# Sinica-SLAM/speechbrain

Measured on AMD Instinct MI355X. Metric: audio-sec/sec Fbank→Conformer fwd (16kHz, B=32×15s) at 1/2/4/8 GPU, higher is better.
Workload: dtype bf16; 1 GPU; Fbank(80)→ConvFrontEnd(64,32)→Conformer 12L d=256 H=4 ffn=1024 k=31 encode, B=32×15s per GPU; global_batch=32, seq_len=376, parallelism=replicas1, hip_graph=True

## Files before the change

include/sbk.h:

```cpp
#ifndef SBK_H
#define SBK_H

#include <stdint.h>

#ifdef __cplusplus
extern "C" {
#endif

#define SBK_ERR_ARG 1001


int sbk_fft_supported(int n_fft);

int sbk_spectrum(int mode, const float* wav, int Bo, int S, int C, int n_fft, int hop, int center, int pad_mode,
                 int T, const float* window, const float* twiddle_nc, const float* twiddle_nfft, int onesided,
                 float norm_scale, float power, float eps, int log_mag, const long long* out_strides,
                 const int* mel_start, const int* mel_len, const int* mel_off, const float* mel_w, int n_melw,
                 int M, int log_mel, float multiplier, float db_offset, float amin, float* out, float* slot_max,
                 void* stream);

int sbk_spectrum_slots(int n_fft, int hop, int T, int M, int n_melw);

int sbk_filterbank(const float* spec, int N, int T, int F, const int* mel_start, const int* mel_len,
                   const int* mel_off, const float* mel_w, const float* dense, int M, int log_mel, float multiplier,
                   float db_offset, float amin, float* out, float* slot_max, void* stream);

int sbk_filterbank_slots(int T, int F);

int sbk_topdb_clamp(float* x, const float* slot_max, int nslot, long long per_seq, int nseq, float top_db,
                    void* stream);

int sbk_filterbank_db_bwd(const float* x, const float* g, int N, long long per_seq, int log_mel, float multiplier,
                          float db_offset, float amin, float top_db, float* stats, float* dx, void* stream);

int sbk_filterbank_wgrad(const float* spec, const float* dx, long long rows, int F, int M, long long rows_per_chunk,
                         float* part, void* stream);

int sbk_magnitude(const float* x, float* y, long long n, int L, float power, float eps, int log_mag, void* stream);

int sbk_dct(const float* x, const float* D, float* y, long long rows, int n_in, int n_out, void* stream);

int sbk_deltas(const float* x, float* y, int N, int T, int F, int window_length, int concat, void* stream);
int sbk_deltas_floor(const float* x, float* y, int N, int T, int F, int window_length, const float* slot_max,
                     int nslot, float top_db, void* stream);

int sbk_context_window(const float* x, float* y, int N, int T, int F, int left, int right, void* stream);

int sbk_specaugment(float* x, int N, int T, int F, int c, int w, int warp_mode, float* tmp, const int* fmask,
                    int n_fmask, const int* tmask, int n_tmask, int use_mean, float* partial, long long n_fcells,
                    void* stream);
int sbk_specaugment_needs_scratch(int N, int T, int F, int c, int w, int n_fmask, int n_tmask, int x_aligned);


int sbk_rnnt_forward(const float* x, const int* labels, const int* Tl, const int* Ul, int B, int T, int U1, int V,
                     int blank, int is_logits, int loss_mode, int reduction, float* ws, float* out, void* stream);
long long sbk_rnnt_workspace_floats(int B, int T, int U1);

int sbk_rnnt_backward(const float* x, const int* labels, int B, int T, int U1, int V, int blank, int mode,
                      const float* ws, const float* scale, int scale_per_b, float* grad, void* stream);

int sbk_rnnt_lattice(const int* Tl, const int* Ul, int B, int T, int U1, int loss_mode, int reduction, float* ws,
                     float* out, void* stream);


int sbk_ctc_forward(const float* x, const int* targets, const int* in_len, const int* tg_len, int B, int T, int V,
                    int Lmax, int blank, int is_logits, float* ws, float* loss, void* stream);
long long sbk_ctc_workspace_floats(int B, int T, int Lmax);

int sbk_ctc_backward(const float* x, const int* targets, const int* in_len, const int* tg_len, int B, int T, int V,
                     int Lmax, int blank, int is_logits, const float* ws, const float* grad_out, float* grad,
                     void* stream);

int sbk_nll_rows_forward(const float* x, const int* targets, int B, int U, long long sb, int V, float* sel,
                         float* rsum, void* stream);
int sbk_nll_rows_backward(const int* targets, const float* a, const float* c, int B, int U, long long sb, int V,
                          float* grad, void* stream);


int sbk_thead_fwd(const float* tn, const float* pn, const void* w, const int* labels, int B, int T, int U1, int J,
                  int V, int blank, int act, float slope, float* lse, float* lpb, float* lpl, void* stream);
int sbk_thead_vpad(int V);
int sbk_thead_dlogits(const float* tn, const float* pn, const void* w, const int* labels, int B, int T, int U1,
                      int J, int V, int blank, int act, float slope, const float* lse, const float* gb,
                      const float* gl, const float* scale, int scale_per_b, void* ds, void* stream);
int sbk_thead_wgrad(const void* ds, const float* tn, const float* pn, const int* Tl, int B, int T, int U1, int J,
                    int V, int act, float slope, float* dw, void* stream);


int sbk_length_mask(const float* rel_len, int B, int T, uint8_t* out, void* stream);

int sbk_gemm_glu_group(int dtype_bf16);

int sbk_gemm(int dtype_bf16, const void* A, int lda, const void* W, int ldw, int M, int N, int K,
             const float* bias, int act, float slope, const float* res, int ldr, float alpha,
             const uint8_t* rowmask, void* out, int ldc, int out_bf16, int tile, void* stream);

int sbk_gemm_ln(int dtype_bf16, const void* A, int lda, const void* W, int ldw, int M, int N, int K,
                const float* bias, const float* res, int ldr, float alpha, const uint8_t* rowmask, float* out,
                int ldc, const float* ln_g, const float* ln_b, float ln_eps, void* u, int ldu, int u_bf16, int tile,
                void* stream);

int sbk_ffn_supported(int D, int H);

int sbk_gemm_batched(int dtype_bf16, const void* A, int lda, long long sA, const void* W, int ldw, long long sW, int M,
                     int N, int K, int batch, void* out, int ldc, long long sC, int zdiv, long long sCo, int out_bf16,
                     void* stream);

int sbk_gemm_tn(const void* A, long long lda, long long sA, const void* B, long long ldb, long long sB, int M, int N,
                int K, int batch, float* C, long long ldc, long long sC, void* stream);
int sbk_gemm_tn_cfg(const void* A, long long lda, long long sA, const void* B, long long ldb, long long sB, int M,
                    int N, int K, int batch, float* C, long long ldc, long long sC, int tile, int nsplit, void* stream);
int sbk_gemm_tn_f32(const float* A, long long lda, long long sA, const float* B, long long ldb, long long sB, int M,
                    int N, int K, int batch, float* C, long long ldc, long long sC, int nsplit, void* stream);

long long sbk_ffn_image_elems(int D, int H, int np, int chain);
int sbk_ffn_image(const void* w1, const void* w2, const void* w1b, const void* w2b, const void* wp, int D, int H,
                  int np, void* img, void* stream);

int sbk_ffn(const float* x, int M, int D, int d_eff, int H, const float* g0, const float* b0, float eps0, const void* img,
            long long img_elems, const float* b1, int act, float slope, const float* b2, float alpha, const float* gp, const float* bp,
            float epsp, float* out, const float* gn, const float* bn, float epsn, void* u, int u_bf16, void* stream);

int sbk_ffn_proj(const float* x, int M, int D, int d_eff, int H, const float* g0, const float* b0, float eps0, const void* img,
                 long long img_elems, const float* b1, int act, float slope, const float* b2, float alpha, const float* gp,
                 const float* bp, float epsp, float* out, const float* gn, const float* bn, float epsn, void* u,
                 int u_bf16, int np, void* yp, void* stream);

int sbk_ffn_chain(const float* x, int M, int D, int d_eff, int H, int act, float slope, const float* g0,
                  const float* b0,
                  float eps0, const float* b1, const float* b2, float alpha, const float* gp, const float* bp,
                  float epsp, const float* g0b, const float* b0b, float eps0b, const float* b1b, const float* b2b,
                  float alphab, float* out, const float* gn, const float* bn, float epsn, void* u, int u_bf16,
                  const void* img, long long img_elems, int np, void* yp, void* stream);

int sbk_layernorm(const float* x, int M, int D, const float* g1, const float* b1, float eps1, void* out1,
                  int out1_bf16, const float* g2, const float* b2, float eps2, void* out2, int out2_bf16,
                  void* stream);

int sbk_dwconv_ln_swish(int in_bf16, const void* x, int B, int T, int C, const float* w, const float* bias, int K,
                        int causal, const float* g, const float* beta, float eps, void* out, int out_bf16,
                        void* stream);

int sbk_conv_block_c1(const float* x, int B, int Tin, int Fin, int Cout, const float* w, const float* bias,
                      const float* g, const float* beta, float eps, float slope, void* out, int out_bf16, int* Tout,
                      int* Fout, void* stream);

int sbk_conv_block_mfma(int in_bf16, const void* x, int B, int Tin, int Fin, int Cin, int Cout, const void* wperm,
                        const float* bias, const float* g, const float* beta, float eps, float slope, void* out,
                        int out_bf16, int* Tout, int* Fout, void* stream);

int sbk_conv_frontend2(int dtype_bf16, const float* x, int B, int Tin, int Fin, const float* w1, const float* b1,
                       const float* g1, const float* be1, float eps1, float slope1, int C1, const void* wp2,
                       const float* b2, const float* g2, const float* be2, float eps2, float slope2, int C2, void* out,
                       int out_bf16, const float* slot_max, int nslot, float top_db, int* Tout, int* Fout,
                       void* stream);

int sbk_cast_bf16(const float* x, void* y, long long n, void* stream);

int sbk_swish(const float* x, float* y, long long n, float beta, void* stream);

int sbk_relpos_attention(int dtype_bf16, const void* qkv, const void* pk, const float* pbu, const float* pbv,
                         const uint8_t* kpm, int B, int T, int H, int dh, float scale, void* out, float* probs,
                         void* stream);

int sbk_relpos_attention_ld(int dtype_bf16, const void* qkv, const void* pk, int ldp, const float* pbu,
                            const float* pbv, const unsigned char* kpm, int B, int T, int H, int dh, float scale,
                            void* out, float* probs, void* stream);
int sbk_relpos_attention_mask(int dtype_bf16, const void* qkv, const void* pk, int ldp, const float* pbu,
                              const float* pbv, const unsigned char* kpm, const float* am, long long am_sb,
                              long long am_sh, int B, int T, int H, int dh, float scale, void* out, float* probs,
                              void* stream);
int sbk_mha_attention(const void* qkv, const unsigned char* kpm, int B, int T, int H, int dh, float scale, void* out,
                      void* stream);
long long sbk_relpos_attention_lds(int dtype_bf16, int T, int dh);

int sbk_relpos_xattn_fwd(int dtype_bf16, const void* q, int ldq, const void* k, int ldk, const void* v, int ldv,
                         const void* pk, int ldp, int P, const float* pbu, const float* pbv, const unsigned char* kpm,
                         const float* am, long long am_sb, long long am_sh, int B, int Lq, int Lk, int H, int dh,
                         float scale, int mask_pos_future, float p_drop, unsigned long long seed, void* out, int ldo,
                         float* probs, float* attn, void* stream);
int sbk_relpos_xattn_bwd(int dtype_bf16, const void* q, int ldq, const void* k, int ldk, const void* v, int ldv,
                         const void* pk, int ldp, int P, const float* pbu, const float* pbv, const float* probs,
                         const void* dO, int lddo, int B, int Lq, int Lk, int H, int dh, float scale,
                         int mask_pos_future, float p_drop, unsigned long long seed, float* G, float* dqu, float* dqv,
                         float* dq, float* dk, float* dv, float* dpk, void* stream);

int sbk_conv_module_supported(int D, int K);
int sbk_conv_module(const float* x, float* out, int B, int T, int D, int d_eff, const float* ln0_w, const float* ln0_b,
                    float eps0, const void* w1p, const float* b1p, const float* wc, const float* bc, int K, int causal,
                    const float* ln1_w, const float* ln1_b, float eps1, const void* w2, const float* b2,
                    const unsigned char* kpm, void* stream);
int sbk_conv_module_pre(const float* x, const void* o, const void* wo, const float* bo, float* out, int B, int T,
                        int D, int d_eff, const float* ln0_w, const float* ln0_b, float eps0, const void* w1p, const float* b1p,
                        const float* wc, const float* bc, int K, int causal, const float* ln1_w, const float* ln1_b,
                        float eps1, const void* w2, const float* b2, const unsigned char* kpm, void* stream);

int sbk_inorm_slices(int T);
int sbk_inorm_partials(const float* x, const float* len, int B, int T, int F, double* part, void* stream);
int sbk_inorm_stats(const double* part, int B, int T, int F, int mean_norm, int std_norm, float eps, float* mean,
                    float* std, float* cur_mean, float* cur_std, int upd, float keep, float wgt, float* glob_mean,
                    float* glob_std, void* stream);
int sbk_inorm_apply(const float* x, int B, int T, int F, const float* mean, const float* std, int per_utt, float* y,
                    void* stream);


int sbk_layernorm_bwd_blocks(int M);
int sbk_layernorm_bwd(const float* x, const void* dy, int dy_bf16, int M, int D, const float* g, float eps,
                      const float* dres, float* dx, float* part, void* stream);

int sbk_layernorm_wide(const float* x, int M, int D, const float* g, const float* b, float eps, void* y, int y_bf16,
                       void* stream);

int sbk_colsum(const float* part, int rows, int cols, float* out, int accumulate, void* stream);

int sbk_rowsum_chunks(long long rows);
int sbk_rowsum_batched(const void* x, int x_bf16, int batch, long long rows, int cols, float* part, float* out,
                       int accumulate, void* stream);
int sbk_rowsum(const void* x, int x_bf16, long long rows, int cols, float* part, float* out, int accumulate,
               void* stream);

int sbk_act_fwd(int mode, const void* x, int x_bf16, long long rows, int cols, void* y, int y_bf16, float slope,
                void* stream);
int sbk_act_bwd(int mode, const void* x, int x_bf16, const void* dy, int dy_bf16, long long rows, int cols, void* dx,
                int dx_bf16, float slope, void* stream);

int sbk_dwconv_fwd(const void* x, int x_bf16, int B, int T, int C, const float* w, const float* bias, int K,
                   int causal, void* y, int y_bf16, void* stream);
int sbk_dwconv_wgrad_chunks(int B, int T);
int sbk_dwconv_bwd(const void* x, int x_bf16, const float* dy, int B, int T, int C, const float* w, int K, int causal,
                   void* dx, int dx_bf16, float* part, void* stream);

int sbk_attn_prep(int dtype_bf16, const void* qkv, const void* dO, const void* pk, int ldp, const float* pbu,
                  const float* pbv, int B, int H, int T, int dh, int Tp, int dhp, int Wp, void* qu, void* qv, void* kT,
                  void* v, void* vT, void* doh, void* pkT, void* stream);
int sbk_attn_probs_pad(const float* P, int BH, int T, int Tp, float p, unsigned long long seed, float* attn, void* Pd,
                       int pd_bf16, void* stream);
int sbk_relpos_softmax_bwd_pad(int dtype_bf16, const float* P, const void* dP, int B, int H, int T, int Tp, int Wp,
                               float scale, float p, unsigned long long seed, void* dS, void* Pd, void* dBD,
                               void* stream);
int sbk_attn_dqkv(const float* dq_ac, const float* dq_bd, const float* dk, const float* dv, int B, int H, int T,
                  int dh, int Tp, int dhp, void* out, int out_bf16, void* stream);

int sbk_im2col(const void* x, int x_bf16, int B, int Ti, int Fi, int Ci, int kt, int kf, int st, int sf, int pt,
               int pf, int ldcol, void* col, int col_bf16, void* stream);
int sbk_col2im(const void* dcol, int dcol_bf16, int B, int Ti, int Fi, int Ci, int kt, int kf, int st, int sf, int pt,
               int pf, int ldcol, void* dx, int dx_bf16, void* stream);

int sbk_im2col_x(const void* x, int x_bf16, int B, int Ti, int Fi, int Ci, int kt, int kf, int st, int sf, int dt,
                 int df, int pt, int pf, int To, int Fo, int mode, int ldcol, void* col, int col_bf16, void* stream);
int sbk_col2im_x(const void* dcol, int dcol_bf16, int B, int Ti, int Fi, int Ci, int kt, int kf, int st, int sf,
                 int dt, int df, int pt, int pf, int To, int Fo, int mode, int ldcol, float* dxpad, void* dx,
                 int dx_bf16, void* stream);

long long sbk_joint_bwd_workspace_floats(int B, int T, int U1, int J);
int sbk_joint_fwd(const float* tn, const float* pn, int B, int T, int U1, int J, int act, float slope, void* z,
                  int z_bf16, void* stream);
int sbk_joint_bwd(const float* tn, const float* pn, const void* dz, int dz_bf16, int B, int T, int U1, int J, int act,
                  float slope, float* dtn, float* dpn, float* ws, void* stream);

int sbk_dropout_add(const void* x, int x_bf16, const float* res, long long rows, int cols,
                    const unsigned char* rowmask, float alpha, float p, unsigned long long seed, void* out,
                    int out_bf16, void* stream);

int sbk_logsoftmax_topk(const float* x, long long ldx, int R, int V, int k, float* vals, long long* idx,
                        void* stream);


int sbk_w2v_wav_stats(const float* wav, int B, long long S, float eps, float* stats, void* stream);

int sbk_w2v_conv0(const float* wav, const float* stats, int B, long long S, int T0, int C, int K, int stride,
                  const float* w, const float* g, const float* b, float eps, void* out, int out_mode,
                  uint8_t* scales, void* stream);

int sbk_ln_act(const void* x, int in_bf16, long long ldx, int M, int D, const float* g, const float* b, float eps,
               int act, void* out, long long ldo, int out_mode, uint8_t* scales, long long lds, void* stream);

int sbk_mx_gemm(const uint8_t* A, const uint8_t* SA, long long lda, long long ldsa, long long rpb, long long a_bs,
                long long s_bs, const uint8_t* W, const uint8_t* SW, long long ldw, long long ldsw, int M, int N,
                int K, const float* bias, int act, float alpha, const float* res, long long ldr, void* out,
                long long ldc, int out_mode, uint8_t* out_scales, long long ldso, void* stream);

long long sbk_mx_gemm_ws_floats(int M, int N, int K, int out_mode);
int sbk_mx_gemm_ws(const uint8_t* A, const uint8_t* SA, long long lda, long long ldsa, long long rpb, long long a_bs,
                   long long s_bs, const uint8_t* W, const uint8_t* SW, long long ldw, long long ldsw, int M, int N,
                   int K, const float* bias, int act, float alpha, const float* res, long long ldr, void* out,
                   long long ldc, int out_mode, uint8_t* out_scales, long long ldso, float* ws, long long ws_floats,
                   void* stream);

int sbk_mx_gemm256(const uint8_t* A, const uint8_t* SA, long long lda, long long ldsa, long long rpb, long long a_bs,
                   long long s_bs, const uint8_t* W, const uint8_t* SW, long long ldw, long long ldsw, int M, int N,
                   int K, const float* bias, int act, float alpha, const float* res, long long ldr, void* out,
                   long long ldc, int out_mode, uint8_t* out_scales, long long ldso, void* stream);

int sbk_add_rows_periodic(float* x, int M, int D, const float* pe, int T, void* stream);

int sbk_mx_quant(const void* x, int in_bf16, long long ldx, int M, int K, uint8_t* q, long long ldq,
                 uint8_t* scales, long long ldsq, void* stream);

int sbk_mx_dequant(const uint8_t* q, long long ldq, const uint8_t* scales, long long ldsq, int M, int K, float* out,
                   void* stream);

#ifdef __cplusplus
}
#endif

#endif
```

speechbrain_amd/_enc.py:

```python
import contextlib
import ctypes
import threading
import weakref
from typing import Optional

import torch

from ._lib import OPS, SbkError, check, custom_op, lib, ptr, require_device, stream_of

ACT = {None: 0, "none": 0, "swish": 1, "glu": 2, "leaky_relu": 3, "relu": 3, "gelu": 4}
_bf16 = torch.bfloat16
_f32 = torch.float32


def _is_bf16(t):
    return t.dtype == _bf16


@custom_op("sbk::gemm", mutates_args=())
def _gemm_op(a: torch.Tensor, w: torch.Tensor, bias: Optional[torch.Tensor], act: int, slope: float,
             res: Optional[torch.Tensor], alpha: float, rowmask: Optional[torch.Tensor], out_bf16: bool,
             tile: int) -> torch.Tensor:
    M, K = a.shape
    N = w.shape[0]
    n_out = N // 2 if act == 2 else N
    out = torch.empty(M, n_out, device=a.device, dtype=_bf16 if out_bf16 else _f32)
    rc = lib().sbk_gemm(int(_is_bf16(a)), ptr(a), a.stride(0), ptr(w), w.stride(0), M, N, K, ptr(bias), act,
                        float(slope), ptr(res), res.stride(0) if res is not None else 0, float(alpha),
                        ptr(rowmask), ptr(out), out.stride(0), int(out_bf16), int(tile), stream_of(a))
    check(rc, "sbk_gemm")
    return out


@_gemm_op.register_fake
def _(a, w, bias, act, slope, res, alpha, rowmask, out_bf16, tile):
    n = w.shape[0] // 2 if act == 2 else w.shape[0]
    return a.new_empty(a.shape[0], n, dtype=_bf16 if out_bf16 else _f32)


def gemm(a, w, bias=None, act=None, slope=0.0, res=None, alpha=1.0, rowmask=None, out=None,
         out_dtype=_f32, tile=0):
    require_device(a, w)
    if out is not None:
        raise ValueError("gemm allocates its output (out= is not supported)")
    if a.dtype != w.dtype:
        raise TypeError(f"gemm operand dtypes differ: {a.dtype} vs {w.dtype}")
    if (a.stride(-1) != 1 and a.shape[-1] > 1) or (w.stride(-1) != 1 and w.shape[-1] > 1):
        raise ValueError("gemm operands must be K-contiguous")
    if res is not None and (res.dtype != _f32 or res.stride(-1) != 1):
        raise ValueError("residual must be fp32, row-contiguous")
    vec = 8 if a.dtype == _bf16 else 4
    if (a.shape[1] % vec or a.stride(0) % vec or w.stride(0) % vec
            or (a.data_ptr() | w.data_ptr()) % 16):
        Kp = -(-a.shape[1] // vec) * vec
        a = torch.nn.functional.pad(a, (0, Kp - a.shape[1]))
        w = torch.nn.functional.pad(w, (0, Kp - w.shape[1]))
    return OPS.gemm(a, w, bias, ACT[act], float(slope), res, float(alpha), rowmask,
                              out_dtype == _bf16, int(tile))


@custom_op("sbk::gemm_tn", mutates_args=())
def _gemm_tn_op(a: torch.Tensor, b: torch.Tensor) -> torch.Tensor:
    K, M = a.shape[-2], a.shape[-1]
    N = b.shape[-1]
    batch = a.shape[0] if a.dim() == 3 else 1
    out = torch.zeros(*([batch] if a.dim() == 3 else []), M, N, device=a.device, dtype=_f32)
    sa = a.stride(0) if a.dim() == 3 else 0
    sb = b.stride(0) if b.dim() == 3 else 0
    _tn_call(a, a.stride(-2), sa, b, b.stride(-2), sb, M, N, K, batch, out, N, M * N if a.dim() == 3 else 0)
    return out


def _tn_call(a, lda, sa, b, ldb, sb, M, N, K, batch, out, ldc, sc):
    det = torch.are_deterministic_algorithms_enabled()
    L = lib()
    if a.dtype == _bf16:
        rc = (L.sbk_gemm_tn_cfg(ptr(a), lda, sa, ptr(b), ldb, sb, M, N, K, batch, ptr(out), ldc, sc, 0, 1, stream_of(a))
              if det else L.sbk_gemm_tn(ptr(a), lda, sa, ptr(b), ldb, sb, M, N, K, batch, ptr(out), ldc, sc, stream_of(a)))
    else:
        rc = L.sbk_gemm_tn_f32(ptr(a), lda, sa, ptr(b), ldb, sb, M, N, K, batch, ptr(out), ldc, sc, int(det),
                               stream_of(a))
    check(rc, "sbk_gemm_tn")


@_gemm_tn_op.register_fake
def _(a, b):
    return a.new_empty(*a.shape[:-2], a.shape[-1], b.shape[-1], dtype=_f32)


def gemm_tn(a, b):
    require_device(a, b)
    if a.dtype != b.dtype or a.dtype not in (_bf16, _f32):
        raise TypeError(f"gemm_tn takes two bf16 or two fp32 operands (got {a.dtype}, {b.dtype})")
    if a.stride(-1) != 1 or b.stride(-1) != 1:
        raise ValueError("gemm_tn operands must be column-contiguous")
    return OPS.gemm_tn(a, b)


def gemm_tn_into(a, b, out, ldc, sC):
    require_device(a, b, out)
    Bt, K, M = a.shape
    N = b.shape[-1]
    if a.dtype != b.dtype or out.dtype != _f32 or a.stride(-1) != 1 or b.stride(-1) != 1:
        raise ValueError("gemm_tn_into: same-dtype column-contiguous operands, fp32 out")
    if out.numel() < (Bt - 1) * sC + (M - 1) * ldc + N:
        raise ValueError("gemm_tn_into: output too small")
    _tn_call(a, a.stride(1), a.stride(0), b, b.stride(1), b.stride(0), M, N, K, Bt, out, ldc, sC)
    return out


@custom_op("sbk::gemm_batched", mutates_args=())
def _gemm_batched_op(a: torch.Tensor, w: torch.Tensor, out_bf16: bool, M: int, zdiv: int, ldc: int, sC: int,
                     sCo: int, rows: int) -> torch.Tensor:
    Bt, _, K = a.shape
    N = w.shape[1]
    if zdiv:
        out = torch.empty(rows, ldc, device=a.device, dtype=_bf16 if out_bf16 else _f32)
    else:
        out = torch.empty(Bt, M, N, device=a.device, dtype=_bf16 if out_bf16 else _f32)
        ldc, sC = N, M * N
    check(lib().sbk_gemm_batched(int(_is_bf16(a)), ptr(a), a.stride(1), a.stride(0), ptr(w), w.stride(1), w.stride(0),
                                 M, N, K, Bt, ptr(out), ldc, sC, zdiv, sCo, int(out_bf16), stream_of(a)),
          "sbk_gemm_batched")
    return out


@_gemm_batched_op.register_fake
def _(a, w, out_bf16, M, zdiv, ldc, sC, sCo, rows):
    dt = _bf16 if out_bf16 else _f32
    if zdiv:
        return a.new_empty(rows, ldc, dtype=dt)
    return a.new_empty(a.shape[0], M, w.shape[1], dtype=dt)


def gemm_batched(a, w, out_dtype=_f32, M=None, heads=None):
    require_device(a, w)
    if a.dtype != w.dtype or a.dtype not in (_bf16, _f32):
        raise TypeError(f"gemm_batched takes two bf16 or two fp32 operands (got {a.dtype}, {w.dtype})")
    if a.stride(-1) != 1 or w.stride(-1) != 1:
        raise ValueError("gemm_batched operands must be K-contiguous")
    Bt, Ma, _ = a.shape
    N = w.shape[1]
    M = Ma if M is None else int(M)
    if not 0 < M <= Ma:
        raise ValueError("gemm_batched: M out of range")
    if heads:
        H = int(heads)
        if Bt % H:
            raise ValueError("gemm_batched: batch not a multiple of heads")
        return OPS.gemm_batched(a, w, out_dtype == _bf16, M, H, H * N, N, M * H * N, Bt // H * M)
    return OPS.gemm_batched(a, w, out_dtype == _bf16, M, 0, 0, 0, 0, 0)


@custom_op("sbk::length_mask", mutates_args=())
def _length_mask_op(rel_len: torch.Tensor, T: int) -> torch.Tensor:
    B = rel_len.shape[0]
    out = torch.empty(B, T, device=rel_len.device, dtype=torch.uint8)
    check(lib().sbk_length_mask(ptr(rel_len), B, int(T), ptr(out), stream_of(rel_len)), "sbk_length_mask")
    return out


@_length_mask_op.register_fake
def _(rel_len, T):
    return rel_len.new_empty(rel_len.shape[0], T, dtype=torch.uint8)


def length_mask(rel_len, T):
    require_device(rel_len)
    rl = rel_len if (rel_len.dtype == _f32 and rel_len.is_contiguous()) else rel_len.float().contiguous()
    return OPS.length_mask(rl, int(T))


@custom_op("sbk::gemm_ln", mutates_args=())
def _gemm_ln_op(a: torch.Tensor, w: torch.Tensor, g: torch.Tensor, b: torch.Tensor, eps: float,
                bias: Optional[torch.Tensor], res: Optional[torch.Tensor], alpha: float,
                rowmask: Optional[torch.Tensor], u_bf16: bool, tile: int) -> tuple[torch.Tensor, torch.Tensor]:
    M, K = a.shape
    N = w.shape[0]
    out = torch.empty(M, N, device=a.device, dtype=_f32)
    u = torch.empty(M, N, device=a.device, dtype=_bf16 if u_bf16 else _f32)
    rc = lib().sbk_gemm_ln(int(_is_bf16(a)), ptr(a), a.stride(0), ptr(w), w.stride(0), M, N, K, ptr(bias), ptr(res),
                           res.stride(0) if res is not None else 0, float(alpha), ptr(rowmask), ptr(out),
                           out.stride(0), ptr(g), ptr(b), float(eps), ptr(u), u.stride(0), int(u_bf16),
                           int(tile), stream_of(a))
    check(rc, "sbk_gemm_ln")
    return out, u


@_gemm_ln_op.register_fake
def _(a, w, g, b, eps, bias, res, alpha, rowmask, u_bf16, tile):
    return (a.new_empty(a.shape[0], w.shape[0], dtype=_f32),
            a.new_empty(a.shape[0], w.shape[0], dtype=_bf16 if u_bf16 else _f32))


def gemm_ln(a, w, ln, bias=None, res=None, alpha=1.0, rowmask=None, out=None, u_dtype=_bf16, tile=0):
    require_device(a, w)
    if out is not None:
        raise ValueError("gemm_ln allocates its output (out= is not supported)")
    if a.dtype != w.dtype:
        raise TypeError(f"gemm operand dtypes differ: {a.dtype} vs {w.dtype}")
    if res is not None and (res.dtype != _f32 or res.stride(-1) != 1):
        raise ValueError("residual must be fp32, row-contiguous")
    g, b, eps = ln
    return OPS.gemm_ln(a, w, g, b, float(eps), bias, res, float(alpha), rowmask, u_dtype == _bf16,
                                 int(tile))


USE_GEMM_LN = False


def gemm_ln_supported(N):
    return int(N) == 256


@custom_op("sbk::layernorm", mutates_args=())
def _layernorm_op(x: torch.Tensor, w1: torch.Tensor, b1: torch.Tensor, eps1: float, out1_mode: int,
                  w2: Optional[torch.Tensor], b2: Optional[torch.Tensor], eps2: float,
                  out2_bf16: bool) -> tuple[torch.Tensor, torch.Tensor]:
    M, D = x.shape
    out1 = torch.empty(M, D, device=x.device, dtype=_bf16 if out1_mode == 2 else _f32) if out1_mode else None
    out2 = torch.empty(M, D, device=x.device, dtype=_bf16 if out2_bf16 else _f32) if w2 is not None else None
    rc = lib().sbk_layernorm(ptr(x), M, D, ptr(w1), ptr(b1), float(eps1), ptr(out1), int(out1_mode == 2),
                             ptr(w2), ptr(b2), float(eps2), ptr(out2), int(out2 is not None and out2_bf16),
                             stream_of(x))
    check(rc, "sbk_layernorm")
    e = x.new_empty(0)
    return (out1 if out1 is not None else e), (out2 if out2 is not None else e)


@_layernorm_op.register_fake
def _(x, w1, b1, eps1, out1_mode, w2, b2, eps2, out2_bf16):
    o1 = x.new_empty(x.shape, dtype=_bf16 if out1_mode == 2 else _f32) if out1_mode else x.new_empty(0)
    o2 = x.new_empty(x.shape, dtype=_bf16 if out2_bf16 else _f32) if w2 is not None else x.new_empty(0)
    return o1, o2


def layernorm(x, w1, b1, eps1, out1_dtype=_f32, w2=None, b2=None, eps2=1e-5, out2_dtype=_bf16, out1=None):
    require_device(x)
    if out1 is not None:
        raise ValueError("layernorm allocates its output (out1= is not supported)")
    mode = 0 if out1_dtype is None else (2 if out1_dtype == _bf16 else 1)
    y1, y2 = OPS.layernorm(x, w1, b1, float(eps1), mode, w2, b2, float(eps2), out2_dtype == _bf16)
    return (y1 if mode else None), (y2 if w2 is not None else None)


def ffn_supported(D, H):
    return bool(lib().sbk_ffn_supported(int(D), int(H)))


class _ImageCache:

    def __init__(self, cap=64):
        self.cap = cap
        self._d = {}

    def _drop(self, key):
        self._d.pop(key, None)

    def get(self, ws, np_, stream):
        key = tuple((w.data_ptr(), w._version) if w is not None else None for w in ws) + (np_,)
        hit = self._d.pop(key, None)
        if hit is None:
            w1, w2, w1b, w2b, wp = ws
            D, H = w1.shape[1], w1.shape[0]
            n = int(lib().sbk_ffn_image_elems(D, H, np_, int(w1b is not None)))
            if n <= 0:
                raise SbkError(f"sbk_ffn_image_elems: unsupported shape D={D} H={H} np={np_}")
            img = torch.empty(n, device=w1.device, dtype=_bf16)
            check(lib().sbk_ffn_image(ptr(w1), ptr(w2), ptr(w1b), ptr(w2b), ptr(wp), D, H, np_, ptr(img),
                                      ctypes.c_void_p(stream.cuda_stream)), "sbk_ffn_image")
            ev = torch.cuda.Event()
            ev.record(stream)
            refs = tuple(weakref.ref(w, lambda _r, k=key: self._drop(k)) for w in ws if w is not None)
            hit = (img, refs, ev, stream.cuda_stream)
            if len(self._d) >= self.cap:
                self._d.pop(next(iter(self._d)))
        elif hit[3] != stream.cuda_stream:
            stream.wait_event(hit[2])
        self._d[key] = hit
        return hit[0]


_FFN_IMAGES = _ImageCache()


def ffn_image(w1, w2, w1b=None, w2b=None, wp=None):
    for t in (w1, w2, w1b, w2b, wp):
        if t is not None and (t.dtype != _bf16 or not t.is_contiguous()):
            raise TypeError("ffn_image: contiguous bf16 weights")
    img = _FFN_IMAGES.get((w1, w2, w1b, w2b, wp), 0 if wp is None else wp.shape[0], torch.cuda.current_stream(w1.device))
    return img


@custom_op("sbk::ffn", mutates_args=())
def _ffn_op(x: torch.Tensor, g0: torch.Tensor, b0: torch.Tensor, e0: float, w1: torch.Tensor, b1: torch.Tensor,
            act: int, slope: float, w2: torch.Tensor, b2: torch.Tensor, alpha: float, gp: Optional[torch.Tensor],
            bp: Optional[torch.Tensor], ep: float, gn: Optional[torch.Tensor], bn: Optional[torch.Tensor], en: float,
            next_bf16: bool, deff: int) -> tuple[torch.Tensor, torch.Tensor]:
    M, D = x.shape
    H = w1.shape[0]
    img = ffn_image(w1, w2)
    out = torch.empty_like(x)
    u = torch.empty(M, D, device=x.device, dtype=_bf16 if next_bf16 else _f32) if gn is not None else None
    rc = lib().sbk_ffn(ptr(x), M, D, deff, H, ptr(g0), ptr(b0), float(e0), ptr(img), img.numel(), ptr(b1), act,
                       float(slope), ptr(b2), float(alpha), ptr(gp), ptr(bp), float(ep), ptr(out), ptr(gn), ptr(bn), float(en),
                       ptr(u), int(next_bf16), stream_of(x))
    check(rc, "sbk_ffn")
    return out, (u if u is not None else x.new_empty(0))


@_ffn_op.register_fake
def _(x, g0, b0, e0, w1, b1, act, slope, w2, b2, alpha, gp, bp, ep, gn, bn, en, next_bf16, deff):
    return (torch.empty_like(x),
            x.new_empty(x.shape, dtype=_bf16 if next_bf16 else _f32) if gn is not None else x.new_empty(0))


@custom_op("sbk::ffn_proj", mutates_args=())
def _ffn_proj_op(x: torch.Tensor, g0: torch.Tensor, b0: torch.Tensor, e0: float, w1: torch.Tensor,
                 b1: torch.Tensor, act: int, slope: float, w2: torch.Tensor, b2: torch.Tensor, alpha: float,
                 gp: Optional[torch.Tensor], bp: Optional[torch.Tensor], ep: float, gn: torch.Tensor,
                 bn: torch.Tensor, en: float, wp: torch.Tensor, deff: int) -> tuple[torch.Tensor, torch.Tensor]:
    M, D = x.shape
    H, NP = w1.shape[0], wp.shape[0]
    img = ffn_image(w1, w2, wp=wp)
    out = torch.empty_like(x)
    y = torch.empty(M, NP, device=x.device, dtype=_bf16)
    rc = lib().sbk_ffn_proj(ptr(x), M, D, deff, H, ptr(g0), ptr(b0), float(e0), ptr(img), img.numel(), ptr(b1), act,
                            float(slope), ptr(b2), float(alpha), ptr(gp), ptr(bp), float(ep), ptr(out), ptr(gn), ptr(bn),
                            float(en), None, 1, NP, ptr(y), stream_of(x))
    check(rc, "sbk_ffn_proj")
    return out, y


@_ffn_proj_op.register_fake
def _(x, g0, b0, e0, w1, b1, act, slope, w2, b2, alpha, gp, bp, ep, gn, bn, en, wp, deff):
    return torch.empty_like(x), x.new_empty((x.shape[0], wp.shape[0]), dtype=_bf16)


def ffn_proj_supported(D, H, NP):
    return ffn_supported(D, H) and NP > 0 and NP % 256 == 0


def ffn_proj(x, ln0, w1, b1, act, slope, w2, b2, alpha, next_ln, wp, post_ln=None, deff=None):
    require_device(x, w1, w2, wp)
    gp, bp, ep = post_ln if post_ln is not None else (None, None, 0.0)
    return OPS.ffn_proj(x, ln0[0], ln0[1], float(ln0[2]), w1, b1, ACT[act], float(slope), w2, b2,
                                  float(alpha), gp, bp, float(ep), next_ln[0], next_ln[1], float(next_ln[2]), wp,
                       int(deff or x.shape[1]))


@custom_op("sbk::ffn_chain", mutates_args=())
def _ffn_chain_op(x: torch.Tensor, act: int, slope: float, g0: torch.Tensor, b0: torch.Tensor, e0: float,
                  w1: torch.Tensor, b1: torch.Tensor, w2: torch.Tensor, b2: torch.Tensor, alpha: float,
                  gp: Optional[torch.Tensor], bp: Optional[torch.Tensor], ep: float, g0b: torch.Tensor,
                  b0b: torch.Tensor, e0b: float, w1b: torch.Tensor, b1b: torch.Tensor, w2b: torch.Tensor,
                  b2b: torch.Tensor, alphab: float, gn: torch.Tensor, bn: torch.Tensor, en: float,
                  wp: torch.Tensor, deff: int) -> tuple[torch.Tensor, torch.Tensor]:
    M, D = x.shape
    H, NP = w1.shape[0], wp.shape[0]
    img = ffn_image(w1, w2, w1b, w2b, wp)
    out = torch.empty_like(x)
    y = torch.empty(M, NP, device=x.device, dtype=_bf16)
    rc = lib().sbk_ffn_chain(ptr(x), M, D, deff, H, act, float(slope), ptr(g0), ptr(b0), float(e0), ptr(b1), ptr(b2),
                             float(alpha), ptr(gp), ptr(bp), float(ep), ptr(g0b), ptr(b0b), float(e0b), ptr(b1b),
                             ptr(b2b), float(alphab), ptr(out), ptr(gn), ptr(bn), float(en), None, 1, ptr(img), img.numel(), NP,
                             ptr(y), stream_of(x))
    check(rc, "sbk_ffn_chain")
    return out, y


@_ffn_chain_op.register_fake
def _(x, act, slope, g0, b0, e0, w1, b1, w2, b2, alpha, gp, bp, ep, g0b, b0b, e0b, w1b, b1b, w2b, b2b, alphab, gn,
      bn, en, wp, deff):
    return torch.empty_like(x), x.new_empty((x.shape[0], wp.shape[0]), dtype=_bf16)


def ffn_chain(x, a, b, act, slope, next_ln, wp, deff=None):
    require_device(x, a[1], b[1], wp)
    if b[1].shape != a[1].shape or b[3].shape != a[3].shape:
        raise ValueError(f"ffn_chain: block shapes differ ({tuple(a[1].shape)}/{tuple(a[3].shape)} vs "
                         f"{tuple(b[1].shape)}/{tuple(b[3].shape)})")
    gp, bp, ep = a[6] if a[6] is not None else (None, None, 0.0)
    return OPS.ffn_chain(x, ACT[act], float(slope), a[0][0], a[0][1], float(a[0][2]), a[1], a[2], a[3],
                                   a[4], float(a[5]), gp, bp, float(ep), b[0][0], b[0][1], float(b[0][2]), b[1], b[2],
                                   b[3], b[4], float(b[5]), next_ln[0], next_ln[1], float(next_ln[2]), wp,
                         int(deff or x.shape[1]))


def ffn(x, ln0, w1, b1, act, slope, w2, b2, alpha, post_ln=None, next_ln=None, next_dtype=_bf16, out=None, deff=None):
    require_device(x, w1, w2)
    gp, bp, ep = post_ln if post_ln is not None else (None, None, 0.0)
    gn, bn, en = next_ln if next_ln is not None else (None, None, 0.0)
    y, u = OPS.ffn(x, ln0[0], ln0[1], float(ln0[2]), w1, b1, ACT[act], float(slope), w2, b2, float(alpha),
                             gp, bp, float(ep), gn, bn, float(en), next_dtype == _bf16, int(deff or x.shape[1]))
    return y, (u if next_ln is not None else None)


@custom_op("sbk::dwconv_ln_swish", mutates_args=())
def _dwconv_op(x: torch.Tensor, B: int, T: int, w: torch.Tensor, bias: Optional[torch.Tensor], causal: bool,
               ln_w: torch.Tensor, ln_b: torch.Tensor, eps: float, out_bf16: bool) -> torch.Tensor:
    C = x.shape[-1]
    K = w.shape[-1]
    out = torch.empty(B * T, C, device=x.device, dtype=_bf16 if out_bf16 else _f32)
    rc = lib().sbk_dwconv_ln_swish(int(_is_bf16(x)), ptr(x), B, T, C, ptr(w), ptr(bias), K, int(causal), ptr(ln_w),
                                   ptr(ln_b), float(eps), ptr(out), int(out_bf16), stream_of(x))
    check(rc, "sbk_dwconv_ln_swish")
    return out


@_dwconv_op.register_fake
def _(x, B, T, w, bias, causal, ln_w, ln_b, eps, out_bf16):
    return x.new_empty(B * T, x.shape[-1], dtype=_bf16 if out_bf16 else _f32)


def dwconv_ln_swish(x, B, T, w, bias, causal, ln_w, ln_b, eps, out_dtype):
    return OPS.dwconv_ln_swish(x, int(B), int(T), w, bias, bool(causal), ln_w, ln_b, float(eps),
                                         out_dtype == _bf16)


def conv_module_supported(D, K):
    return bool(lib().sbk_conv_module_supported(int(D), int(K)))


@custom_op("sbk::conv_module", mutates_args=())
def _conv_module_op(x: torch.Tensor, B: int, T: int, g0: torch.Tensor, b0: torch.Tensor, e0: float,
                    w1p: torch.Tensor, b1p: torch.Tensor, wc: torch.Tensor, bc: Optional[torch.Tensor], causal: bool,
                    g1: torch.Tensor, b1: torch.Tensor, e1: float, w2: torch.Tensor, b2: Optional[torch.Tensor],
                    kpm: Optional[torch.Tensor], o: Optional[torch.Tensor], wo: Optional[torch.Tensor],
                    bo: Optional[torch.Tensor], deff: int) -> torch.Tensor:
    K = wc.shape[0]
    out = torch.empty_like(x)
    rc = lib().sbk_conv_module_pre(ptr(x), ptr(o), ptr(wo), ptr(bo), ptr(out), B, T, x.shape[1], deff, ptr(g0),
                                   ptr(b0),
                                   float(e0), ptr(w1p), ptr(b1p), ptr(wc), ptr(bc), K, int(causal), ptr(g1), ptr(b1),
                                   float(e1), ptr(w2), ptr(b2), ptr(kpm), stream_of(x))
    check(rc, "sbk_conv_module_pre")
    return out


@_conv_module_op.register_fake
def _(x, B, T, g0, b0, e0, w1p, b1p, wc, bc, causal, g1, b1, e1, w2, b2, kpm, o, wo, bo, deff):
    return torch.empty_like(x)


def conv_module(x, B, T, ln0, w1p, b1p, wc, bc, causal, ln1, w2, b2, kpm=None, pre=None, deff=None):
    require_device(x, w1p, w2)
    o, wo, bo = pre if pre is not None else (None, None, None)
    return OPS.conv_module(x, int(B), int(T), ln0[0], ln0[1], float(ln0[2]), w1p, b1p, wc, bc,
                                     bool(causal), ln1[0], ln1[1], float(ln1[2]), w2, b2, kpm, o, wo, bo,
                            int(deff or x.shape[1]))


@custom_op("sbk::conv_block_c1", mutates_args=())
def _conv_block_c1_op(x: torch.Tensor, w: torch.Tensor, bias: torch.Tensor, ln_w: torch.Tensor, ln_b: torch.Tensor,
                      eps: float, slope: float, out_bf16: bool) -> torch.Tensor:
    B, Tin, Fin = x.shape
    Cout = w.shape[0]
    Tout, Fout = (Tin - 1) // 2 + 1, (Fin - 1) // 2 + 1
    out = torch.empty(B, Tout, Fout, Cout, device=x.device, dtype=_bf16 if out_bf16 else _f32)
    rc = lib().sbk_conv_block_c1(ptr(x), B, Tin, Fin, Cout, ptr(w), ptr(bias), ptr(ln_w), ptr(ln_b), float(eps),
                                 float(slope), ptr(out), int(out_bf16), None, None, stream_of(x))
    check(rc, "sbk_conv_block_c1")
    return out


@_conv_block_c1_op.register_fake
def _(x, w, bias, ln_w, ln_b, eps, slope, out_bf16):
    B, Tin, Fin = x.shape
    return x.new_empty(B, (Tin - 1) // 2 + 1, (Fin - 1) // 2 + 1, w.shape[0], dtype=_bf16 if out_bf16 else _f32)


def conv_block_c1(x, w, bias, ln_w, ln_b, eps, slope, out_dtype):
    require_device(x)
    return OPS.conv_block_c1(x, w, bias, ln_w, ln_b, float(eps), float(slope), out_dtype == _bf16)


@custom_op("sbk::conv_block_mfma", mutates_args=())
def _conv_block_mfma_op(x: torch.Tensor, wperm: torch.Tensor, bias: torch.Tensor, ln_w: torch.Tensor,
                        ln_b: torch.Tensor, eps: float, slope: float, out_bf16: bool) -> torch.Tensor:
    B, Tin, Fin, Cin = x.shape
    Cout = wperm.shape[0]
    Tout, Fout = (Tin - 1) // 2 + 1, (Fin - 1) // 2 + 1
    out = torch.empty(B, Tout, Fout, Cout, device=x.device, dtype=_bf16 if out_bf16 else _f32)
    rc = lib().sbk_conv_block_mfma(int(_is_bf16(x)), ptr(x), B, Tin, Fin, Cin, Cout, ptr(wperm), ptr(bias),
                                   ptr(ln_w), ptr(ln_b), float(eps), float(slope), ptr(out), int(out_bf16), None,
                                   None, stream_of(x))
    check(rc, "sbk_conv_block_mfma")
    return out


@_conv_block_mfma_op.register_fake
def _(x, wperm, bias, ln_w, ln_b, eps, slope, out_bf16):
    B, Tin, Fin, _ = x.shape
    return x.new_empty(B, (Tin - 1) // 2 + 1, (Fin - 1) // 2 + 1, wperm.shape[0],
                       dtype=_bf16 if out_bf16 else _f32)


def conv_block_mfma(x, wperm, bias, ln_w, ln_b, eps, slope, out_dtype):
    require_device(x, wperm)
    return OPS.conv_block_mfma(x, wperm, bias, ln_w, ln_b, float(eps), float(slope), out_dtype == _bf16)


@custom_op("sbk::conv_frontend2", mutates_args=())
def _conv_frontend2_op(x: torch.Tensor, w1: torch.Tensor, b1: torch.Tensor, g1: torch.Tensor, be1: torch.Tensor,
                       e1: float, s1: float, wperm2: torch.Tensor, b2: torch.Tensor, g2: torch.Tensor,
                       be2: torch.Tensor, e2: float, s2: float, out_bf16: bool, slot_max: Optional[torch.Tensor],
                       top_db: float) -> torch.Tensor:
    B, Tin, Fin = x.shape
    C1, C2 = w1.shape[0], wperm2.shape[0]
    T1, F1 = (Tin - 1) // 2 + 1, (Fin - 1) // 2 + 1
    T2, F2 = (T1 - 1) // 2 + 1, (F1 - 1) // 2 + 1
    out = torch.empty(B, T2, F2, C2, device=x.device, dtype=_bf16 if out_bf16 else _f32)
    rc = lib().sbk_conv_frontend2(int(_is_bf16(wperm2)), ptr(x), B, Tin, Fin, ptr(w1), ptr(b1), ptr(g1), ptr(be1),
                                  float(e1), float(s1), C1, ptr(wperm2), ptr(b2), ptr(g2), ptr(be2), float(e2),
                                  float(s2), C2, ptr(out), int(out_bf16), ptr(slot_max),
                                  slot_max.shape[1] if slot_max is not None else 0, float(top_db), None, None,
                                  stream_of(x))
    check(rc, "sbk_conv_frontend2")
    return out


@_conv_frontend2_op.register_fake
def _(x, w1, b1, g1, be1, e1, s1, wperm2, b2, g2, be2, e2, s2, out_bf16, slot_max, top_db):
    B, Tin, Fin = x.shape
    T1, F1 = (Tin - 1) // 2 + 1, (Fin - 1) // 2 + 1
    return x.new_empty(B, (T1 - 1) // 2 + 1, (F1 - 1) // 2 + 1, wperm2.shape[0], dtype=_bf16 if out_bf16 else _f32)


def conv_frontend2(x, blk1, blk2, wperm2, out_dtype, topdb=None):
    require_device(x, wperm2)
    w1, b1, g1, be1, e1, s1 = blk1
    _, b2, g2, be2, e2, s2 = blk2
    sm, tdb = topdb if topdb is not None else (None, 0.0)
    return OPS.conv_frontend2(x, w1, b1, g1, be1, float(e1), float(s1), wperm2, b2, g2, be2, float(e2),
                                        float(s2), out_dtype == _bf16, sm, float(tdb))


@custom_op("sbk::relpos_attention", mutates_args=())
def _relpos_attention_op(qkv: torch.Tensor, pk: torch.Tensor, pbu: torch.Tensor, pbv: torch.Tensor,
                         kpm: Optional[torch.Tensor], B: int, T: int, H: int, dh: int, scale: float,
                         need_probs: bool, am: Optional[torch.Tensor], am_sb: int,
                         am_sh: int) -> tuple[torch.Tensor, torch.Tensor]:
    d = H * dh
    out = torch.empty(B * T, d, device=qkv.device, dtype=qkv.dtype)
    probs = torch.empty(B, H, T, T, device=qkv.device, dtype=_f32) if need_probs else qkv.new_empty(0, dtype=_f32)
    if am is None:
        rc = lib().sbk_relpos_attention_ld(int(_is_bf16(qkv)), ptr(qkv), ptr(pk), pk.stride(0), ptr(pbu), ptr(pbv),
                                           ptr(kpm), B, T, H, dh, float(scale), ptr(out),
                                           ptr(probs) if need_probs else None, stream_of(qkv))
    else:
        rc = lib().sbk_relpos_attention_mask(int(_is_bf16(qkv)), ptr(qkv), ptr(pk), pk.stride(0), ptr(pbu), ptr(pbv),
                                             ptr(kpm), ptr(am), am_sb, am_sh, B, T, H, dh, float(scale), ptr(out),
                                             ptr(probs) if need_probs else None, stream_of(qkv))
    check(rc, "sbk_relpos_attention")
    return out, probs


@_relpos_attention_op.register_fake
def _(qkv, pk, pbu, pbv, kpm, B, T, H, dh, scale, need_probs, am, am_sb, am_sh):
    return (qkv.new_empty(B * T, H * dh),
            qkv.new_empty(B, H, T, T, dtype=_f32) if need_probs else qkv.new_empty(0, dtype=_f32))


def attn_mask_arg(attn_mask, B, T, H, device, Lk=None):
    if attn_mask is None:
        return None
    Lk = T if Lk is None else Lk
    m = attn_mask.to(device)
    if m.dtype == torch.bool:
        m = torch.zeros(m.shape, device=device, dtype=_f32).masked_fill_(m, -float("inf"))
    else:
        m = m.to(_f32)
    if m.dim() == 2:
        if tuple(m.shape) != (T, Lk):
            raise ValueError(f"attn_mask {tuple(m.shape)} != ({T}, {Lk})")
        return m.contiguous(), 0, 0
    m = m.reshape(-1, H, T, Lk).contiguous()
    if m.shape[0] not in (1, B):
        raise ValueError(f"attn_mask batch {m.shape[0]} does not broadcast to {B}")
    return m, (H * T * Lk if m.shape[0] == B else 0), T * Lk


def relpos_attention(qkv, pk, pbu, pbv, kpm, B, T, H, dh, scale, need_probs=False, am=None):
    d = H * dh
    if pk.stride(-1) != 1 or pk.shape[-1] != d:
        raise ValueError("pk must be (2T-1, d) with unit column stride")
    m, sb, sh = am if am is not None else (None, 0, 0)
    out, probs = OPS.relpos_attention(qkv, pk, pbu, pbv, kpm, int(B), int(T), int(H), int(dh),
                                                float(scale), bool(need_probs), m, int(sb), int(sh))
    return out, (probs if need_probs else None)


@custom_op("sbk::relpos_xattn", mutates_args=())
def _relpos_xattn_op(q: torch.Tensor, k: torch.Tensor, v: torch.Tensor, pk: Optional[torch.Tensor],
                     pbu: Optional[torch.Tensor], pbv: Optional[torch.Tensor], kpm: Optional[torch.Tensor],
                     am: Optional[torch.Tensor], am_sb: int, am_sh: int, B: int, Lq: int, Lk: int, H: int, dh: int,
                     scale: float, mpf: bool, p: float, seed: int) -> tuple[torch.Tensor, torch.Tensor, torch.Tensor]:
    out = torch.empty(B * Lq, H * dh, device=q.device, dtype=q.dtype)
    probs = torch.empty(B, H, Lq, Lk, device=q.device, dtype=_f32)
    attn = torch.empty_like(probs) if p > 0 else probs.new_empty(0)
    P = pk.shape[0] if pk is not None else 2 * Lk - 1
    rc = lib().sbk_relpos_xattn_fwd(int(_is_bf16(q)), ptr(q), q.stride(0), ptr(k), k.stride(0), ptr(v), v.stride(0),
                                    ptr(pk), pk.stride(0) if pk is not None else 0, P, ptr(pbu), ptr(pbv), ptr(kpm),
                                    ptr(am), int(am_sb), int(am_sh), B, Lq, Lk, H, dh, float(scale), int(mpf),
                                    float(p), int(seed), ptr(out), out.stride(0), ptr(probs),
                                    ptr(attn) if p > 0 else None, stream_of(q))
    check(rc, "sbk_relpos_xattn_fwd")
    return out, probs, attn


@_relpos_xattn_op.register_fake
def _(q, k, v, pk, pbu, pbv, kpm, am, am_sb, am_sh, B, Lq, Lk, H, dh, scale, mpf, p, seed):
    probs = q.new_empty(B, H, Lq, Lk, dtype=_f32)
    return q.new_empty(B * Lq, H * dh), probs, (q.new_empty(B, H, Lq, Lk, dtype=_f32) if p > 0 else
                                                  q.new_empty(0, dtype=_f32))


def relpos_xattn(q, k, v, pk, pbu, pbv, kpm, B, Lq, Lk, H, dh, scale, mask_pos_future=False, am=None, p=0.0,
                 seed=0):
    for t in (q, k, v) + ((pk,) if pk is not None else ()):
        if t.stride(-1) != 1 or t.shape[-1] != H * dh or t.dtype != q.dtype:
            raise ValueError("relpos_xattn: q / k / v / pk must be (rows, H*dh), unit column stride, one dtype")
    if pk is not None and pk.shape[0] // 2 + 1 != Lk:
        raise ValueError(f"pos_embs has {pk.shape[0]} rows: rel_shift keeps {pk.shape[0] // 2 + 1} != k_len {Lk}")
    m, sb, sh = am if am is not None else (None, 0, 0)
    out, probs, attn = OPS.relpos_xattn(q, k, v, pk, pbu, pbv, kpm, m, int(sb), int(sh), int(B), int(Lq), int(Lk),
                                        int(H), int(dh), float(scale), bool(mask_pos_future), float(p), int(seed))
    return out, probs, (attn if p > 0 else probs)


@custom_op("sbk::mha_attention", mutates_args=())
def _mha_attention_op(qkv: torch.Tensor, kpm: Optional[torch.Tensor], B: int, T: int, H: int, dh: int,
                      scale: float) -> torch.Tensor:
    out = torch.empty(B * T, H * dh, device=qkv.device, dtype=qkv.dtype)
    check(lib().sbk_mha_attention(ptr(qkv), ptr(kpm), B, T, H, dh, float(scale), ptr(out), stream_of(qkv)),
          "sbk_mha_attention")
    return out


@_mha_attention_op.register_fake
def _(qkv, kpm, B, T, H, dh, scale):
    return qkv.new_empty(B * T, H * dh)


def mha_fast_ok(qkv, T, dh):
    return qkv.dtype == _bf16 and dh == 64 and T <= 4096 and qkv.is_contiguous() and qkv.data_ptr() % 16 == 0


def mha_attention(qkv, kpm, B, T, H, dh, scale):
    return OPS.mha_attention(qkv, kpm, int(B), int(T), int(H), int(dh), float(scale))


def glu_group():
    return int(lib().sbk_gemm_glu_group(1))


@custom_op("sbk::cast_bf16", mutates_args=())
def _cast_bf16_op(x: torch.Tensor) -> torch.Tensor:
    out = torch.empty(x.shape, device=x.device, dtype=_bf16)
    check(lib().sbk_cast_bf16(ptr(x), ptr(out), x.numel(), stream_of(x)), "sbk_cast_bf16")
    return out


@_cast_bf16_op.register_fake
def _(x):
    return x.new_empty(x.shape, dtype=_bf16)


def cast_bf16(x):
    return OPS.cast_bf16(x)


def to_compute(x, dtype):
    if dtype == _bf16:
        return x.contiguous() if x.dtype == _bf16 else cast_bf16(x.float().contiguous())
    if x.dtype in (torch.float16, _bf16):
        return x.float().contiguous()
    if x.dtype != _f32:
        raise TypeError(f"fp32 compute path got {x.dtype}")
    return x.contiguous()


def compute_dtype():
    if torch.is_autocast_enabled("cuda"):
        dt = torch.get_autocast_dtype("cuda")
        if dt == _bf16:
            return _bf16
        if dt != torch.float16:
            raise NotImplementedError(f"speechbrain_amd kernels compute in bf16 or fp32; torch.autocast(dtype={dt})")
    return _f32


_MX = threading.local()


@contextlib.contextmanager
def mxfp8(enabled=True):
    prev = getattr(_MX, "on", False)
    _MX.on = bool(enabled)
    try:
        yield
    finally:
        _MX.on = prev


def mx_enabled():
    return getattr(_MX, "on", False)


class WeightCache:

    def __init__(self):
        self._d = {}

    def get(self, key, params, make):
        sig = tuple((p.data_ptr(), p._version, p.device) for p in params)
        hit = self._d.get(key)
        if hit is not None and hit[0] == sig:
            return hit[1]
        v = make()
        self._d[key] = (sig, v)
        return v
```

speechbrain_amd/_lib.py:

```python
import ctypes
import os

import torch

_HERE = os.path.dirname(os.path.abspath(__file__))
LIB_PATH = os.path.join(_HERE, "libsbk.so")

_vp = ctypes.c_void_p
_i = ctypes.c_int
_ll = ctypes.c_longlong
_f = ctypes.c_float

SIGNATURES = {
    "sbk_fft_supported": [_i],
    "sbk_spectrum": [_i, _vp, _i, _i, _i, _i, _i, _i, _i, _i, _vp, _vp, _vp, _i, _f, _f, _f, _i, _vp,
                     _vp, _vp, _vp, _vp, _i, _i, _i, _f, _f, _f, _vp, _vp, _vp],
    "sbk_filterbank": [_vp, _i, _i, _i, _vp, _vp, _vp, _vp, _vp, _i, _i, _f, _f, _f, _vp, _vp, _vp],
    "sbk_spectrum_slots": [_i, _i, _i, _i, _i],
    "sbk_filterbank_slots": [_i, _i],
    "sbk_topdb_clamp": [_vp, _vp, _i, _ll, _i, _f, _vp],
    "sbk_filterbank_db_bwd": [_vp, _vp, _i, _ll, _i, _f, _f, _f, _f, _vp, _vp, _vp],
    "sbk_filterbank_wgrad": [_vp, _vp, _ll, _i, _i, _ll, _vp, _vp],
    "sbk_magnitude": [_vp, _vp, _ll, _i, _f, _f, _i, _vp],
    "sbk_dct": [_vp, _vp, _vp, _ll, _i, _i, _vp],
    "sbk_deltas": [_vp, _vp, _i, _i, _i, _i, _i, _vp],
    "sbk_deltas_floor": [_vp, _vp, _i, _i, _i, _i, _vp, _i, _f, _vp],
    "sbk_context_window": [_vp, _vp, _i, _i, _i, _i, _i, _vp],
    "sbk_gemm_glu_group": [_i],
    "sbk_length_mask": [_vp, _i, _i, _vp, _vp],
    "sbk_gemm": [_i, _vp, _i, _vp, _i, _i, _i, _i, _vp, _i, _f, _vp, _i, _f, _vp, _vp, _i, _i, _i, _vp],
    "sbk_gemm_ln": [_i, _vp, _i, _vp, _i, _i, _i, _i, _vp, _vp, _i, _f, _vp, _vp, _i, _vp, _vp, _f, _vp, _i, _i, _i,
                    _vp],
    "sbk_thead_vpad": [_i],
    "sbk_thead_fwd": [_vp, _vp, _vp, _vp, _i, _i, _i, _i, _i, _i, _i, _f, _vp, _vp, _vp, _vp],
    "sbk_thead_dlogits": [_vp, _vp, _vp, _vp, _i, _i, _i, _i, _i, _i, _i, _f, _vp, _vp, _vp, _vp, _i, _vp, _vp],
    "sbk_thead_wgrad": [_vp, _vp, _vp, _vp, _i, _i, _i, _i, _i, _i, _f, _vp, _vp],
    "sbk_rnnt_lattice": [_vp, _vp, _i, _i, _i, _i, _i, _vp, _vp, _vp],
    "sbk_gemm_tn": [_vp, _ll, _ll, _vp, _ll, _ll, _i, _i, _i, _i, _vp, _ll, _ll, _vp],
    "sbk_gemm_tn_cfg": [_vp, _ll, _ll, _vp, _ll, _ll, _i, _i, _i, _i, _vp, _ll, _ll, _i, _i, _vp],
    "sbk_gemm_tn_f32": [_vp, _ll, _ll, _vp, _ll, _ll, _i, _i, _i, _i, _vp, _ll, _ll, _i, _vp],
    "sbk_gemm_batched": [_i, _vp, _i, _ll, _vp, _i, _ll, _i, _i, _i, _i, _vp, _i, _ll, _i, _ll, _i, _vp],
    "sbk_attn_prep": [_i, _vp, _vp, _vp, _i, _vp, _vp, _i, _i, _i, _i, _i, _i, _i, _vp, _vp, _vp, _vp, _vp, _vp,
                      _vp, _vp],
    "sbk_attn_dqkv": [_vp, _vp, _vp, _vp, _i, _i, _i, _i, _i, _i, _vp, _i, _vp],
    "sbk_attn_probs_pad": [_vp, _i, _i, _i, _f, ctypes.c_ulonglong, _vp, _vp, _i, _vp],
    "sbk_relpos_softmax_bwd_pad": [_i, _vp, _vp, _i, _i, _i, _i, _i, _f, _f, ctypes.c_ulonglong, _vp, _vp, _vp,
                                   _vp],
    "sbk_ffn_supported": [_i, _i],
    "sbk_ffn": [_vp, _i, _i, _i, _i, _vp, _vp, _f, _vp, _ll, _vp, _i, _f, _vp, _f, _vp, _vp, _f, _vp, _vp, _vp, _f, _vp,
                _i, _vp],
    "sbk_ffn_chain": [_vp, _i, _i, _i, _i, _i, _f, _vp, _vp, _f, _vp, _vp, _f, _vp, _vp, _f, _vp, _vp, _f, _vp, _vp, _f,
                      _vp, _vp, _vp, _f, _vp, _i, _vp, _ll, _i, _vp, _vp],
    "sbk_ffn_proj": [_vp, _i, _i, _i, _i, _vp, _vp, _f, _vp, _ll, _vp, _i, _f, _vp, _f, _vp, _vp, _f, _vp, _vp, _vp, _f,
                     _vp, _i, _i, _vp, _vp],
    "sbk_ffn_image_elems": [_i, _i, _i, _i],
    "sbk_ffn_image": [_vp, _vp, _vp, _vp, _vp, _i, _i, _i, _vp, _vp],
    "sbk_layernorm": [_vp, _i, _i, _vp, _vp, _f, _vp, _i, _vp, _vp, _f, _vp, _i, _vp],
    "sbk_dwconv_ln_swish": [_i, _vp, _i, _i, _i, _vp, _vp, _i, _i, _vp, _vp, _f, _vp, _i, _vp],
    "sbk_conv_block_c1": [_vp, _i, _i, _i, _i, _vp, _vp, _vp, _vp, _f, _f, _vp, _i, _vp, _vp, _vp],
    "sbk_conv_block_mfma": [_i, _vp, _i, _i, _i, _i, _i, _vp, _vp, _vp, _vp, _f, _f, _vp, _i, _vp, _vp, _vp],
    "sbk_conv_frontend2": [_i, _vp, _i, _i, _i, _vp, _vp, _vp, _vp, _f, _f, _i, _vp, _vp, _vp, _vp, _f, _f, _i,
                           _vp, _i, _vp, _i, _f, _vp, _vp, _vp],
    "sbk_cast_bf16": [_vp, _vp, _ll, _vp],
    "sbk_swish": [_vp, _vp, _ll, _f, _vp],
    "sbk_w2v_wav_stats": [_vp, _i, _ll, _f, _vp, _vp],
    "sbk_w2v_conv0": [_vp, _vp, _i, _ll, _i, _i, _i, _i, _vp, _vp, _vp, _f, _vp, _i, _vp, _vp],
    "sbk_add_rows_periodic": [_vp, _i, _i, _vp, _i, _vp],
    "sbk_ln_act": [_vp, _i, _ll, _i, _i, _vp, _vp, _f, _i, _vp, _ll, _i, _vp, _ll, _vp],
    "sbk_mx_gemm": [_vp, _vp, _ll, _ll, _ll, _ll, _ll, _vp, _vp, _ll, _ll, _i, _i, _i, _vp, _i, _f, _vp, _ll, _vp,
                    _ll, _i, _vp, _ll, _vp],
    "sbk_mx_gemm_ws": [_vp, _vp, _ll, _ll, _ll, _ll, _ll, _vp, _vp, _ll, _ll, _i, _i, _i, _vp, _i, _f, _vp, _ll, _vp,
                       _ll, _i, _vp, _ll, _vp, _ll, _vp],
    "sbk_mx_gemm_ws_floats": [_i, _i, _i, _i],
    "sbk_mx_gemm256": [_vp, _vp, _ll, _ll, _ll, _ll, _ll, _vp, _vp, _ll, _ll, _i, _i, _i, _vp, _i, _f, _vp, _ll,
                       _vp, _ll, _i, _vp, _ll, _vp],
    "sbk_mx_quant": [_vp, _i, _ll, _i, _i, _vp, _ll, _vp, _ll, _vp],
    "sbk_mx_dequant": [_vp, _ll, _vp, _ll, _i, _i, _vp, _vp],
    "sbk_specaugment": [_vp, _i, _i, _i, _i, _i, _i, _vp, _vp, _i, _vp, _i, _i, _vp, _ll, _vp],
    "sbk_specaugment_needs_scratch": [_i, _i, _i, _i, _i, _i, _i, _i],
    "sbk_rnnt_forward": [_vp, _vp, _vp, _vp, _i, _i, _i, _i, _i, _i, _i, _i, _vp, _vp, _vp],
    "sbk_rnnt_workspace_floats": [_i, _i, _i],
    "sbk_logsoftmax_topk": [_vp, _ll, _i, _i, _i, _vp, _vp, _vp],
    "sbk_rnnt_backward": [_vp, _vp, _i, _i, _i, _i, _i, _i, _vp, _vp, _i, _vp, _vp],
    "sbk_ctc_forward": [_vp, _vp, _vp, _vp, _i, _i, _i, _i, _i, _i, _vp, _vp, _vp],
    "sbk_ctc_workspace_floats": [_i, _i, _i],
    "sbk_ctc_backward": [_vp, _vp, _vp, _vp, _i, _i, _i, _i, _i, _i, _vp, _vp, _vp, _vp],
    "sbk_nll_rows_forward": [_vp, _vp, _i, _i, _ll, _i, _vp, _vp, _vp],
    "sbk_nll_rows_backward": [_vp, _vp, _vp, _i, _i, _ll, _i, _vp, _vp],
    "sbk_relpos_attention": [_i, _vp, _vp, _vp, _vp, _vp, _i, _i, _i, _i, _f, _vp, _vp, _vp],
    "sbk_relpos_attention_lds": [_i, _i, _i],
    "sbk_relpos_attention_mask": [_i, _vp, _vp, _i, _vp, _vp, _vp, _vp, _ll, _ll, _i, _i, _i, _i, _f, _vp, _vp, _vp],
    "sbk_relpos_attention_ld": [_i, _vp, _vp, _i, _vp, _vp, _vp, _i, _i, _i, _i, _f, _vp, _vp, _vp],
    "sbk_mha_attention": [_vp, _vp, _i, _i, _i, _i, _f, _vp, _vp],
    "sbk_relpos_xattn_fwd": [_i, _vp, _i, _vp, _i, _vp, _i, _vp, _i, _i, _vp, _vp, _vp, _vp, _ll, _ll, _i, _i, _i, _i,
                             _i, _f, _i, _f, ctypes.c_ulonglong, _vp, _i, _vp, _vp, _vp],
    "sbk_relpos_xattn_bwd": [_i, _vp, _i, _vp, _i, _vp, _i, _vp, _i, _i, _vp, _vp, _vp, _vp, _i, _i, _i, _i, _i, _i,
                             _f, _i, _f, ctypes.c_ulonglong, _vp, _vp, _vp, _vp, _vp, _vp, _vp, _vp],
    "sbk_inorm_slices": [_i],
    "sbk_inorm_partials": [_vp, _vp, _i, _i, _i, _vp, _vp],
    "sbk_inorm_stats": [_vp, _i, _i, _i, _i, _i, _f, _vp, _vp, _vp, _vp, _i, _f, _f, _vp, _vp, _vp],
    "sbk_inorm_apply": [_vp, _i, _i, _i, _vp, _vp, _i, _vp, _vp],
    "sbk_conv_module_supported": [_i, _i],
    "sbk_conv_module_pre": [_vp, _vp, _vp, _vp, _vp, _i, _i, _i, _i, _vp, _vp, _f, _vp, _vp, _vp, _vp, _i, _i, _vp,
                            _vp, _f, _vp, _vp, _vp, _vp],
    "sbk_conv_module": [_vp, _vp, _i, _i, _i, _i, _vp, _vp, _f, _vp, _vp, _vp, _vp, _i, _i, _vp, _vp, _f, _vp, _vp, _vp,
                        _vp],
    "sbk_layernorm_bwd_blocks": [_i],
    "sbk_layernorm_bwd": [_vp, _vp, _i, _i, _i, _vp, _f, _vp, _vp, _vp, _vp],
    "sbk_layernorm_wide": [_vp, _i, _i, _vp, _vp, _f, _vp, _i, _vp],
    "sbk_colsum": [_vp, _i, _i, _vp, _i, _vp],
    "sbk_rowsum_chunks": [_ll],
    "sbk_rowsum": [_vp, _i, _ll, _i, _vp, _vp, _i, _vp],
    "sbk_rowsum_batched": [_vp, _i, _i, _ll, _i, _vp, _vp, _i, _vp],
    "sbk_act_fwd": [_i, _vp, _i, _ll, _i, _vp, _i, _f, _vp],
    "sbk_act_bwd": [_i, _vp, _i, _vp, _i, _ll, _i, _vp, _i, _f, _vp],
    "sbk_dwconv_fwd": [_vp, _i, _i, _i, _i, _vp, _vp, _i, _i, _vp, _i, _vp],
    "sbk_dwconv_wgrad_chunks": [_i, _i],
    "sbk_dwconv_bwd": [_vp, _i, _vp, _i, _i, _i, _vp, _i, _i, _vp, _i, _vp, _vp],
    "sbk_im2col": [_vp, _i, _i, _i, _i, _i, _i, _i, _i, _i, _i, _i, _i, _vp, _i, _vp],
    "sbk_col2im": [_vp, _i, _i, _i, _i, _i, _i, _i, _i, _i, _i, _i, _i, _vp, _i, _vp],
    "sbk_im2col_x": [_vp, _i, _i, _i, _i, _i, _i, _i, _i, _i, _i, _i, _i, _i, _i, _i, _i, _i, _vp, _i, _vp],
    "sbk_col2im_x": [_vp, _i, _i, _i, _i, _i, _i, _i, _i, _i, _i, _i, _i, _i, _i, _i, _i, _i, _vp, _vp, _i, _vp],
    "sbk_joint_fwd": [_vp, _vp, _i, _i, _i, _i, _i, _f, _vp, _i, _vp],
    "sbk_dropout_add": [_vp, _i, _vp, _ll, _i, _vp, _f, _f, ctypes.c_ulonglong, _vp, _i, _vp],
    "sbk_joint_bwd": [_vp, _vp, _vp, _i, _i, _i, _i, _i, _i, _f, _vp, _vp, _vp, _vp],
    "sbk_joint_bwd_workspace_floats": [_i, _i, _i, _i],
}
RESTYPES = {"sbk_relpos_attention_lds": ctypes.c_longlong, "sbk_mx_gemm_ws_floats": ctypes.c_longlong, "sbk_ffn_image_elems": ctypes.c_longlong, "sbk_joint_bwd_workspace_floats": ctypes.c_longlong, "sbk_rnnt_workspace_floats": ctypes.c_longlong, "sbk_ctc_workspace_floats": ctypes.c_longlong}

_lib = None
_load_error = None


class SbkError(RuntimeError):
    pass


def lib():
    global _lib, _load_error
    if _lib is not None:
        return _lib
    if not os.path.exists(LIB_PATH):
        raise SbkError(
            f"speechbrain_amd HIP library not found at {LIB_PATH}; build it with "
            "`python -c 'import __graft_entry__ as g; g.build()'` (hipcc --offload-arch=gfx950). "
            "There is no CPU fallback.")
    try:
        l = ctypes.CDLL(LIB_PATH)
    except OSError as e:
        _load_error = e
        raise SbkError(f"failed to load {LIB_PATH}: {e}") from e
    for name, argt in SIGNATURES.items():
        fn = getattr(l, name)
        fn.argtypes = argt
        fn.restype = RESTYPES.get(name, ctypes.c_int)
    _lib = l
    return l


def exported_symbols():
    return list(SIGNATURES)


def check(rc, what):
    if rc != 0:
        raise SbkError(f"{what} failed with code {rc}" + (" (invalid argument)" if rc == 1001 else ""))


def ptr(t):
    if t is None:
        return None
    return ctypes.c_void_p(t.data_ptr())


def stream_of(t):
    return ctypes.c_void_p(torch.cuda.current_stream(t.device).cuda_stream)


def require_device(*tensors):
    for t in tensors:
        if t is not None and (not isinstance(t, torch.Tensor) or t.device.type != "cuda"):
            raise SbkError("speechbrain_amd kernels need ROCm device tensors (got "
                           f"{getattr(t, 'device', type(t))}); there is no CPU fallback")


class _FastOp:

    def __init__(self, opdef, mutates_args=()):
        import inspect
        self._def = opdef
        self._body = opdef._init_fn
        self._op = None
        names = list(inspect.signature(opdef._init_fn).parameters)
        self._mut = tuple((names.index(m), m) for m in mutates_args)

    def __call__(self, *args, **kw):
        diff = (torch.is_grad_enabled()
                and any(isinstance(t, torch.Tensor) and t.requires_grad for t in (*args, *kw.values())))
        if diff and self._def._backward_fn is None and not torch.jit.is_tracing():
            raise RuntimeError(f"sbk::{self._def._name} has no backward; an input requires grad — call it under "
                               "torch.no_grad() or on detached tensors (the differentiable path is _autograd)")
        if (torch.compiler.is_compiling() or torch.jit.is_tracing()
                or torch._C._get_dispatch_mode(torch._C._TorchDispatchModeKey.FAKE) is not None
                or torch._C._len_torch_dispatch_stack() > 0 or torch._C._are_functorch_transforms_active()
                or diff):
            if self._op is None:
                self._op = getattr(torch.ops.sbk, self._def._name)
            return self._op(*args, **kw)
        out = self._body(*args, **kw)
        for i, m in self._mut:
            t = args[i] if i < len(args) else kw.get(m)
            if isinstance(t, torch.Tensor):
                torch.autograd.graph.increment_version(t)
        return out

    def __getattr__(self, name):
        return getattr(self._def, name)


_OPS = {}


def custom_op(qualname, mutates_args):
    def deco(fn):
        op = _FastOp(torch.library.custom_op(qualname, mutates_args=mutates_args)(fn), mutates_args)
        _OPS[qualname.split("::", 1)[1]] = op
        return op
    return deco


class _Ops:

    def __getattr__(self, name):
        return _OPS[name]


OPS = _Ops()
```

speechbrain_amd/csrc/ffn.hip:

```cpp
#include "mfma.h"

using namespace sbk;

namespace {

enum Act { ACT_NONE = 0, ACT_SWISH = 1, ACT_GLU = 2, ACT_LRELU = 3, ACT_GELU = 4 };

struct FfnArgs {
  const float* x;
  int M, H;
  const float *g0, *b0;
  float eps0;
  const bf16_t* img;
  const float* b1;
  int act;
  float slope;
  const float* b2;
  float alpha;
  const float *gp, *bp;
  float epsp;
  float* out;
  const float *gn, *bn;
  float epsn;
  void* u;
  int u_bf16;
  int np;
  bf16_t* yp;
  const float *g0b, *b0b;
  float eps0b;
  const float *b1b, *b2b;
  float alphab;
  float inv_n, npad;
};

__device__ __forceinline__ bf16x8 ld8(const bf16_t* p) { return *reinterpret_cast<const bf16x8*>(p); }

template <int V>
struct IntC {
  static constexpr int value = V;
};

constexpr int FFN_BM = 48;
constexpr int FFN_PAD = 16;
constexpr int FFN_NW = 8, FFN_NT = FFN_NW * 64;
__device__ __forceinline__ constexpr int ffn_sw(int row) { return ((row >> 2) & 1) << 3; }
static_assert(FFN_NW % 8 == 0, "rows w + FFN_NW * i share bit 2 with w (their swizzle is ffn_sw(w))");
constexpr int FFN_RS = 12;

#define FFN_MFMA(A, B, C) __builtin_amdgcn_mfma_f32_16x16x32_bf16((A), (B), (C), 0, 0, 0)

template <int ACT>
__device__ __forceinline__ float act_fn(float v, float slope) {
  if (ACT == ACT_SWISH) return v * __builtin_amdgcn_rcpf(1.0f + __expf(-v));
  if (ACT == ACT_LRELU) return v >= 0.f ? v : v * slope;
  if (ACT == ACT_GELU) return 0.5f * v * (1.0f + erff(v * 0.70710678118654752f));
  return v;
}

__device__ __forceinline__ f32x4 lds_f4(const float* p) {
  f32x4 v;
  const uint32_t la = (uint32_t)(uintptr_t)((const __attribute__((address_space(3))) float*)p);
  asm volatile("ds_read_b128 %0, %1" : "=v"(v) : "v"(la) : "memory");
  return v;
}

__device__ __forceinline__ uint32_t lds_addr(const void* p) {
  return (uint32_t)(uintptr_t)((const __attribute__((address_space(3))) char*)p);
}
__device__ __forceinline__ float lds_f1(const float* p) {
  float v;
  asm volatile("ds_read_b32 %0, %1" : "=v"(v) : "v"(lds_addr(p)) : "memory");
  return v;
}
__device__ __forceinline__ void lds_st1(float* p, float v) {
  asm volatile("ds_write_b32 %0, %1" ::"v"(lds_addr(p)), "v"(v) : "memory");
}
__device__ __forceinline__ void lds_st4(float* p, f32x4 v) {
  asm volatile("ds_write_b128 %0, %1" ::"v"(lds_addr(p)), "v"(v) : "memory");
}
__device__ __forceinline__ void lds_st2(void* p, uint2 v) {
  const unsigned long long u = (unsigned long long)v.x | ((unsigned long long)v.y << 32);
  asm volatile("ds_write_b64 %0, %1" ::"v"(lds_addr(p)), "v"(u) : "memory");
}
template <typename V>
__device__ __forceinline__ void tie(V& v) {
  asm volatile("s_waitcnt lgkmcnt(0)" : "+v"(v));
}
__device__ __forceinline__ void lds_barrier() {
  asm volatile("s_waitcnt lgkmcnt(0)" ::: "memory");
  __builtin_amdgcn_s_barrier();
}

__device__ __forceinline__ f32x4 gld4(const float* p) {
  f32x4 v;
  asm volatile("global_load_dwordx4 %0, %1, off" : "=v"(v) : "v"(p) : "memory");
  return v;
}
__device__ __forceinline__ void vtie(f32x4& v) { asm volatile("" : "+v"(v)); }

__device__ __forceinline__ void vm_wait(int n) {
  switch (n) {
    case 0: asm volatile("s_waitcnt vmcnt(0)" ::: "memory"); break;
    case 1: asm volatile("s_waitcnt vmcnt(1)" ::: "memory"); break;
    case 2: asm volatile("s_waitcnt vmcnt(2)" ::: "memory"); break;
    case 3: asm volatile("s_waitcnt vmcnt(3)" ::: "memory"); break;
    case 4: asm volatile("s_waitcnt vmcnt(4)" ::: "memory"); break;
    case 5: asm volatile("s_waitcnt vmcnt(5)" ::: "memory"); break;
    case 6: asm volatile("s_waitcnt vmcnt(6)" ::: "memory"); break;
    case 7: asm volatile("s_waitcnt vmcnt(7)" ::: "memory"); break;
    default: asm volatile("s_waitcnt vmcnt(8)" ::: "memory"); break;
  }
}

template <int D, int T2, int MT, int NW>
__device__ __forceinline__ void row_ln(float (&z)[T2][MT][4], float* red, const float* gam, const float* bet, float eps,
                                       int w, int g, int fr, float inv_n, float npad) {
  static_assert(NW == 8, "two b128 reads per row");
  float mean[MT], rstd[MT];
#pragma unroll
  for (int pass = 0; pass < 2; ++pass) {
    float part[MT];
#pragma unroll
    for (int mt = 0; mt < MT; ++mt) {
      float s = 0.f;
#pragma unroll
      for (int j = 0; j < T2; ++j)
#pragma unroll
        for (int e = 0; e < 4; ++e) {
          const float dv = pass ? z[j][mt][e] - mean[mt] : z[j][mt][e];
          s += pass ? dv * dv : dv;
        }
      part[mt] = col4_sum(s);
    }
    lds_barrier();
    if (g == 0) {
#pragma unroll
      for (int mt = 0; mt < MT; ++mt) lds_st1(red + (mt * 16 + fr) * FFN_RS + w, part[mt]);
    }
    lds_barrier();
    f32x4 rv[MT][2];
#pragma unroll
    for (int mt = 0; mt < MT; ++mt) {
      rv[mt][0] = lds_f4(red + (mt * 16 + fr) * FFN_RS);
      rv[mt][1] = lds_f4(red + (mt * 16 + fr) * FFN_RS + 4);
    }
#pragma unroll
    for (int mt = 0; mt < MT; ++mt) {
      tie(rv[mt][0]);
      tie(rv[mt][1]);
      const float t = (rv[mt][0][0] + rv[mt][0][1]) + (rv[mt][0][2] + rv[mt][0][3]) + (rv[mt][1][0] + rv[mt][1][1]) +
                      (rv[mt][1][2] + rv[mt][1][3]);
      if (pass)
        rstd[mt] = 1.0f / sqrtf((t - npad * mean[mt] * mean[mt]) * inv_n + eps);
      else
        mean[mt] = t * inv_n;
    }
  }
  f32x4 gv[T2], bv[T2];
#pragma unroll
  for (int j = 0; j < T2; ++j) {
    const int d = (w * T2 + j) * 16 + 4 * g;
    gv[j] = lds_f4(gam + d);
    bv[j] = lds_f4(bet + d);
  }
#pragma unroll
  for (int j = 0; j < T2; ++j) {
    tie(gv[j]);
    tie(bv[j]);
#pragma unroll
    for (int e = 0; e < 4; ++e)
#pragma unroll
      for (int mt = 0; mt < MT; ++mt) z[j][mt][e] = (z[j][mt][e] - mean[mt]) * rstd[mt] * gv[j][e] + bv[j][e];
  }
}

template <int K1, int KS, int MT, int XS, int BK>
__device__ __forceinline__ void load_frags(bf16x8 (&xa)[K1][KS][MT], const bf16_t* Xn, int fr, int fk) {
#pragma unroll
  for (int r = 0; r < K1; ++r)
#pragma unroll
    for (int ks = 0; ks < KS; ++ks)
#pragma unroll
      for (int mt = 0; mt < MT; ++mt)
        asm volatile("ds_read_b128 %0, %1"
                     : "=v"(xa[r][ks][mt])
                     : "v"(lds_addr(Xn + (mt * 16 + fr) * XS + r * BK + ks * 32 + fk))
                     : "memory");
#pragma unroll
  for (int r = 0; r < K1; ++r)
#pragma unroll
    for (int ks = 0; ks < KS; ++ks)
#pragma unroll
      for (int mt = 0; mt < MT; ++mt) tie(xa[r][ks][mt]);
}


SBK_PROBE_BUFFER(g_ffn_tl, 16, 256)
#define FFN_TL(i) SBK_PROBE(if (tl_rec >= 0 && lane == 0) g_ffn_tl[tl_rec][i] = __builtin_amdgcn_s_memtime();)

template <int D, int ACT, bool PROJ, bool CHAIN>
__global__ void __launch_bounds__(FFN_NT) ffn_kernel(FfnArgs a) {
  constexpr int BM = FFN_BM, HC = 256, NW = FFN_NW, NT = FFN_NT;
  constexpr int XS = D + FFN_PAD, HS = HC + FFN_PAD;
  constexpr int MT = BM / 16;
  constexpr int T = 256 / 16 / FFN_NW;
  constexpr int BK = 64;
  constexpr int K1 = D / BK, K2 = HC / BK, SPC = K1 + K2;
  constexpr int NB = 2;
  constexpr int TROWS = 256;
  constexpr int GL = TROWS * BK * 2 / 16 / NT;
  static_assert(GL * 8 == T * 16, "each wave stages exactly the weight rows it multiplies");
  constexpr int PER = D / 64;
  static_assert(PER == 4 && D == 256 && HC / 16 / NW == T && D / 16 / NW == T, "shape");

  extern __shared__ __attribute__((aligned(16))) unsigned char smem[];
  bf16_t* ring = reinterpret_cast<bf16_t*>(smem);
  bf16_t* Xn = ring + NB * TROWS * BK;
  bf16_t* Hs = Xn + BM * XS;
  float* b1s = reinterpret_cast<float*>(Hs + 2 * BM * HS);
  float* red = b1s + (CHAIN ? 2 : 1) * a.H;
  float* prm = red + BM * FFN_RS;
  enum { P_B2 = 0, P_GP, P_BP, P_G0B, P_B0B, P_B2B, P_GN, P_BN, P_N };
  static_assert(P_N == NW, "one parameter row per wave");

  const int tid = threadIdx.x, lane = tid & 63, w = tid >> 6;
  const int fr = lane & 15, g = lane >> 4, fk = (8 * g) ^ ffn_sw(fr);
  const int m0 = blockIdx.x * BM;
  const int NCH = a.H / HC;
  const int S = NCH * SPC;
  const int SF = CHAIN ? 2 * S : S;
  const int SP = PROJ ? (a.np / TROWS) * K1 : 0;
  const int ST = SF + SP;
  SBK_PROBE(const int tl_rec = blockIdx.x == 128 ? w : -1;)
  FFN_TL(0);

  auto issue = [&](int s, int slot) __attribute__((always_inline)) {
    const bf16_t* src = a.img + (long long)s * (TROWS * BK) + w * (GL * 512) + lane * 8;
    bf16_t* dst = ring + slot * (TROWS * BK) + w * (GL * 512);
    const auto gs = (const __attribute__((address_space(1))) void*)src;
    const auto ls = (__attribute__((address_space(3))) void*)dst;
    static_assert(GL == 4, "four 1-KB pieces per wave and tile");
    __builtin_amdgcn_global_load_lds(gs, ls, 16, 0, 0);
    __builtin_amdgcn_global_load_lds(gs, ls, 16, 1024, 0);
    __builtin_amdgcn_global_load_lds(gs, ls, 16, 2048, 0);
    __builtin_amdgcn_global_load_lds(gs, ls, 16, 3072, 0);
  };
  constexpr int NRW = (BM + NW - 1) / NW;
  f32x4 xres[T][MT];
#pragma unroll
  for (int j = 0; j < T; ++j)
#pragma unroll
    for (int mt = 0; mt < MT; ++mt) {
      const int row = min(m0 + mt * 16 + fr, a.M - 1);
      xres[j][mt] = gld4(a.x + (long long)row * D + (w * T + j) * 16 + 4 * g);
    }
  f32x4 xv[NRW];
#pragma unroll
  for (int i = 0; i < NRW; ++i) {
    const int rr = w + i * NW, row = min(m0 + rr, a.M - 1);
    xv[i] = gld4(a.x + (long long)row * D + lane * PER);
  }
  f32x4 g04 = gld4(a.g0 + lane * PER), b04 = gld4(a.b0 + lane * PER);
  const float* psrc = w == P_B2 ? a.b2 : w == P_GP ? a.gp : w == P_BP ? a.bp : w == P_G0B ? a.g0b
                    : w == P_B0B ? a.b0b : w == P_B2B ? a.b2b : w == P_GN ? a.gn : a.bn;
  f32x4 pv = f32x4{0.f, 0.f, 0.f, 0.f}, b1v = pv, b1bv = pv;
  if (psrc) pv = gld4(psrc + lane * PER);
  const bool b1t = tid * 4 < a.H;
  if (b1t) b1v = gld4(a.b1 + tid * 4);
  if (CHAIN && b1t) b1bv = gld4(a.b1b + tid * 4);
  issue(0, 0);
  issue(1, 1);
  asm volatile("s_waitcnt vmcnt(%0)" ::"n"(NB * GL) : "memory");
#pragma unroll
  for (int j = 0; j < T; ++j)
#pragma unroll
    for (int mt = 0; mt < MT; ++mt) vtie(xres[j][mt]);
#pragma unroll
  for (int i = 0; i < NRW; ++i) vtie(xv[i]);
  vtie(g04);
  vtie(b04);
  vtie(pv);
  vtie(b1v);
  vtie(b1bv);

#pragma unroll
  for (int i = 0; i < NRW; ++i) {
    const int rr = w + i * NW;
    if (rr >= BM) break;
    const bool live = m0 + rr < a.M;
    const float v[4] = {live ? xv[i][0] : 0.f, live ? xv[i][1] : 0.f, live ? xv[i][2] : 0.f, live ? xv[i][3] : 0.f};
    const float mean = wave_sum_v(v[0] + v[1] + v[2] + v[3]) * a.inv_n;
    float q = 0.f;
#pragma unroll
    for (int e = 0; e < 4; ++e) q += (v[e] - mean) * (v[e] - mean);
    const float rstd = 1.0f / sqrtf((wave_sum_v(q) - a.npad * mean * mean) * a.inv_n + a.eps0);
    uint2 pk;
    pk.x = pack_bf16x2((v[0] - mean) * rstd * g04[0] + b04[0], (v[1] - mean) * rstd * g04[1] + b04[1]);
    pk.y = pack_bf16x2((v[2] - mean) * rstd * g04[2] + b04[2], (v[3] - mean) * rstd * g04[3] + b04[3]);
    lds_st2(Xn + rr * XS + ((lane * PER) ^ ffn_sw(w)), pk);
  }
  static_assert(2048 <= NT * 4, "b1 in one float4 per thread");
  if (psrc) lds_st4(prm + w * D + lane * PER, pv);
  if (b1t) lds_st4(b1s + tid * 4, b1v);
  if (CHAIN && b1t) lds_st4(b1s + a.H + tid * 4, b1bv);

  f32x4 acc1[T][MT], acc2[T][MT];
#pragma unroll
  for (int t = 0; t < T; ++t)
#pragma unroll
    for (int mt = 0; mt < MT; ++mt) {
      acc1[t][mt] = f32x4{0.f, 0.f, 0.f, 0.f};
      acc2[t][mt] = f32x4{0.f, 0.f, 0.f, 0.f};
    }

  FFN_TL(1);
  lds_barrier();
  bf16x8 xa[K1][BK / 32][MT];
  load_frags<K1, BK / 32, MT, XS, BK>(xa, Xn, fr, fk);
  auto step = [&](int s, int r, bool ph2, const bf16_t* Hc, bool bar, auto&& post) __attribute__((always_inline)) {
    asm volatile("s_waitcnt vmcnt(%0)" ::"n"(GL * (NB - 1)) : "memory");
    asm volatile("s_waitcnt lgkmcnt(0)" ::: "memory");
    if (bar) __builtin_amdgcn_s_barrier();
    if (s < 96) FFN_TL(2 + 2 * s);
    const bf16_t* tile = ring + (s % NB) * TROWS * BK;
    bf16x8 fw[BK / 32][T], fa[BK / 32][MT];
#pragma unroll
    for (int ks = 0; ks < BK / 32; ++ks) {
#pragma unroll
      for (int t = 0; t < T; ++t) {
        const int row = w * (T * 16) + t * 16 + fr;
        fw[ks][t] = ld8(tile + row * BK + (((ks * 4 + g) ^ ((row >> 1) & 7)) << 3));
      }
#pragma unroll
      for (int mt = 0; mt < MT; ++mt)
        fa[ks][mt] = ph2 ? ld8(Hc + (mt * 16 + fr) * HS + r * BK + ks * 32 + fk) : xa[ph2 ? 0 : r][ks][mt];
    }
    asm volatile("s_waitcnt lgkmcnt(0)" ::: "memory");
    issue(min(s + NB, ST - 1), s % NB);
#pragma unroll
    for (int ks = 0; ks < BK / 32; ++ks)
#pragma unroll
      for (int t = 0; t < T; ++t)
#pragma unroll
        for (int mt = 0; mt < MT; ++mt) {
          if (ph2)
            acc2[t][mt] = FFN_MFMA(fw[ks][t], fa[ks][mt], acc2[t][mt]);
          else
            acc1[t][mt] = FFN_MFMA(fw[ks][t], fa[ks][mt], acc1[t][mt]);
        }
    post();
    if (s < 96) FFN_TL(3 + 2 * s);
  };
  auto none = []() __attribute__((always_inline)) {};
  auto act_tiles = [&](int i0, int i1, const float* b1c, bf16_t* Hn) __attribute__((always_inline)) {
#pragma unroll
    for (int t = 0; t < T; ++t) {
      if ((t + 1) * MT <= i0 || t * MT >= i1) continue;
      const int n = w * (T * 16) + t * 16 + 4 * g;
      f32x4 bb;
      asm volatile("ds_read_b128 %0, %1\n\ts_waitcnt lgkmcnt(0)" : "=v"(bb) : "v"(lds_addr(b1c + n)) : "memory");
#pragma unroll
      for (int mt = 0; mt < MT; ++mt) {
        const int i = t * MT + mt;
        if (i < i0 || i >= i1) continue;
        const f32x4 v = acc1[t][mt];
        uint2 pk;
        pk.x = pack_bf16x2(act_fn<ACT>(v[0] + bb[0], a.slope), act_fn<ACT>(v[1] + bb[1], a.slope));
        pk.y = pack_bf16x2(act_fn<ACT>(v[2] + bb[2], a.slope), act_fn<ACT>(v[3] + bb[3], a.slope));
        const unsigned long long pv = (unsigned long long)pk.x | ((unsigned long long)pk.y << 32);
        asm volatile("ds_write_b64 %0, %1" ::"v"(lds_addr(Hn + (mt * 16 + fr) * HS + (n ^ ffn_sw(fr)))), "v"(pv) : "memory");
        acc1[t][mt] = f32x4{0.f, 0.f, 0.f, 0.f};
      }
    }
  };
  for (int stage = 0; stage < (CHAIN ? 2 : 1); ++stage) {
  if (CHAIN && stage == 1) {
    FFN_TL(197);
    float z[T][MT][4];
#pragma unroll
    for (int j = 0; j < T; ++j) {
      const int d = (w * T + j) * 16 + 4 * g;
      f32x4 bb = lds_f4(prm + P_B2 * D + d);
      tie(bb);
#pragma unroll
      for (int mt = 0; mt < MT; ++mt) {
        const f32x4 xr = xres[j][mt];
        z[j][mt][0] = xr[0] + a.alpha * (acc2[j][mt][0] + bb[0]);
        z[j][mt][1] = xr[1] + a.alpha * (acc2[j][mt][1] + bb[1]);
        z[j][mt][2] = xr[2] + a.alpha * (acc2[j][mt][2] + bb[2]);
        z[j][mt][3] = xr[3] + a.alpha * (acc2[j][mt][3] + bb[3]);
        acc1[j][mt] = f32x4{0.f, 0.f, 0.f, 0.f};
        acc2[j][mt] = f32x4{0.f, 0.f, 0.f, 0.f};
      }
    }
    FFN_TL(200);
    if (a.gp) row_ln<D, T, MT, NW>(z, red, prm + P_GP * D, prm + P_BP * D, a.epsp, w, g, fr, a.inv_n, a.npad);
    FFN_TL(201);
#pragma unroll
    for (int j = 0; j < T; ++j)
#pragma unroll
      for (int mt = 0; mt < MT; ++mt) xres[j][mt] = f32x4{z[j][mt][0], z[j][mt][1], z[j][mt][2], z[j][mt][3]};
    row_ln<D, T, MT, NW>(z, red, prm + P_G0B * D, prm + P_B0B * D, a.eps0b, w, g, fr, a.inv_n, a.npad);
    FFN_TL(202);
#pragma unroll
    for (int j = 0; j < T; ++j) {
      const int d = (w * T + j) * 16 + 4 * g;
#pragma unroll
      for (int mt = 0; mt < MT; ++mt) {
        uint2 pk;
        pk.x = pack_bf16x2(z[j][mt][0], z[j][mt][1]);
        pk.y = pack_bf16x2(z[j][mt][2], z[j][mt][3]);
        lds_st2(Xn + (mt * 16 + fr) * XS + (d ^ ffn_sw(fr)), pk);
      }
    }
    lds_barrier();
    FFN_TL(203);
    load_frags<K1, BK / 32, MT, XS, BK>(xa, Xn, fr, fk);
    FFN_TL(198);
  }
  const float* b1st = b1s + stage * a.H;
  for (int c = 0; c < NCH; ++c) {
    const int s0 = stage * S + c * SPC;
#pragma unroll
    for (int r = 0; r < K1; ++r) step(s0 + r, r, false, nullptr, false, none);
    bf16_t* Hc = Hs + (c & 1) * BM * HS;
    act_tiles(0, T * MT, b1st + c * HC, Hc);
#pragma unroll
    for (int p = 0; p < K2; ++p) step(s0 + K1 + p, p, true, Hc, p == 0, none);
  }
  }
  if (!PROJ) asm volatile("s_waitcnt vmcnt(0)" ::: "memory");
  FFN_TL(194);

  const float* b2f = prm + (CHAIN ? P_B2B : P_B2) * D;
  const float alphaf = CHAIN ? a.alphab : a.alpha;
  const bool postln = !CHAIN && a.gp;
  float z[T][MT][4];
#pragma unroll
  for (int j = 0; j < T; ++j) {
    const int d = (w * T + j) * 16 + 4 * g;
    f32x4 bb = lds_f4(b2f + d);
    tie(bb);
#pragma unroll
    for (int mt = 0; mt < MT; ++mt) {
      const f32x4 xr = xres[j][mt];
      z[j][mt][0] = xr[0] + alphaf * (acc2[j][mt][0] + bb[0]);
      z[j][mt][1] = xr[1] + alphaf * (acc2[j][mt][1] + bb[1]);
      z[j][mt][2] = xr[2] + alphaf * (acc2[j][mt][2] + bb[2]);
      z[j][mt][3] = xr[3] + alphaf * (acc2[j][mt][3] + bb[3]);
    }
  }
  FFN_TL(195);
  if (postln) row_ln<D, T, MT, NW>(z, red, prm + P_GP * D, prm + P_BP * D, a.epsp, w, g, fr, a.inv_n, a.npad);
  if (PROJ) {
    float* Zo = reinterpret_cast<float*>(Hs);
    constexpr int ZS = D + 4;
    static_assert(BM * ZS * 4 <= 2 * BM * HS * 2, "out rows fit over Hs");
#pragma unroll
    for (int j = 0; j < T; ++j)
#pragma unroll
      for (int mt = 0; mt < MT; ++mt) xres[j][mt] = f32x4{z[j][mt][0], z[j][mt][1], z[j][mt][2], z[j][mt][3]};
    row_ln<D, T, MT, NW>(z, red, prm + P_GN * D, prm + P_BN * D, a.epsn, w, g, fr, a.inv_n, a.npad);
    FFN_TL(204);
#pragma unroll
    for (int j = 0; j < T; ++j) {
      const int d = (w * T + j) * 16 + 4 * g;
#pragma unroll
      for (int mt = 0; mt < MT; ++mt) {
        lds_st4(Zo + (mt * 16 + fr) * ZS + d, xres[j][mt]);
        uint2 pk;
        pk.x = pack_bf16x2(z[j][mt][0], z[j][mt][1]);
        pk.y = pack_bf16x2(z[j][mt][2], z[j][mt][3]);
        lds_st2(Xn + (mt * 16 + fr) * XS + (d ^ ffn_sw(fr)), pk);
      }
    }
    lds_barrier();
    FFN_TL(205);
    static_assert(MT <= K1, "stores of a column block fit in its steps");
    const int ncp = a.np / TROWS;
    const bool full = m0 + BM <= a.M;
    uint2 yq[T][MT];
    for (int nc = 0; nc < ncp; ++nc) {
#pragma unroll
      for (int r = 0; r < K1; ++r) {
        const int s = SF + nc * K1 + r;
        const int kprev1 = (r >= 1 ? (r - 1 < MT) : (K1 - 1 < MT)) ? T : 0;
        const int kprev2 = (r >= 2 ? (r - 2 < MT) : (K1 + r - 2 < MT)) ? T : 0;
        const int k1 = (r >= 1 || nc > 0) ? kprev1 : 0, k2 = (r >= 2 || nc > 0) ? kprev2 : 0;
        vm_wait((s + 1 < ST ? GL : 0) + (full ? k1 + k2 : 0));
        const bf16_t* tile = ring + (s % NB) * TROWS * BK;
        int ln;
        asm volatile("v_mbcnt_lo_u32_b32 %0, -1, 0\n\tv_mbcnt_hi_u32_b32 %0, -1, %0" : "=v"(ln));
        const int lfr = ln & 15, lg = ln >> 4;
        bf16x8 fw[BK / 32][T];
#pragma unroll
        for (int ks = 0; ks < BK / 32; ++ks)
#pragma unroll
          for (int t = 0; t < T; ++t) {
            const int row = w * (T * 16) + t * 16 + lfr;
            fw[ks][t] = ld8(tile + row * BK + (((ks * 4 + lg) ^ ((row >> 1) & 7)) << 3));
          }
        bf16x8 fx[BK / 32][MT];
#pragma unroll
        for (int ks = 0; ks < BK / 32; ++ks)
#pragma unroll
          for (int mt = 0; mt < MT; ++mt) {
            const uint32_t la = (uint32_t)(uintptr_t)((const __attribute__((address_space(3))) bf16_t*)(
                Xn + (mt * 16 + fr) * XS + r * BK + ks * 32 + fk));
            asm volatile("ds_read_b128 %0, %1" : "=v"(fx[ks][mt]) : "v"(la) : "memory");
          }
        f32x4 ov[T];
        if (r < MT && full && nc == 0) {
#pragma unroll
          for (int j = 0; j < T; ++j) ov[j] = lds_f4(Zo + (r * 16 + lfr) * ZS + (w * T + j) * 16 + 4 * lg);
        }
        asm volatile("s_waitcnt lgkmcnt(0)" ::: "memory");
        if (s + NB < ST) issue(s + NB, s % NB);
        asm volatile("" ::: "memory");
        if (r < MT && full) {
          const long long row = m0 + r * 16 + lfr;
          if (nc == 0) {
#pragma unroll
            for (int j = 0; j < T; ++j)
              *reinterpret_cast<f32x4*>(a.out + row * D + (w * T + j) * 16 + 4 * lg) = ov[j];
          } else {
#pragma unroll
            for (int t = 0; t < T; ++t)
              *reinterpret_cast<uint2*>(a.yp + row * a.np + (nc - 1) * TROWS + w * (T * 16) + t * 16 + 4 * lg) = yq[t][r];
          }
        }
#pragma unroll
        for (int ks = 0; ks < BK / 32; ++ks)
#pragma unroll
          for (int t = 0; t < T; ++t)
#pragma unroll
            for (int mt = 0; mt < MT; ++mt)
              acc1[t][mt] = __builtin_amdgcn_mfma_f32_16x16x32_bf16(fw[ks][t], fx[ks][mt], acc1[t][mt], 0, 0, 0);
      }
      int ln;
      asm volatile("v_mbcnt_lo_u32_b32 %0, -1, 0\n\tv_mbcnt_hi_u32_b32 %0, -1, %0" : "=v"(ln));
#pragma unroll
      for (int t = 0; t < T; ++t)
#pragma unroll
        for (int mt = 0; mt < MT; ++mt) {
          const f32x4 v = acc1[t][mt];
          yq[t][mt].x = pack_bf16x2(v[0], v[1]);
          yq[t][mt].y = pack_bf16x2(v[2], v[3]);
          acc1[t][mt] = f32x4{0.f, 0.f, 0.f, 0.f};
          const int row = m0 + mt * 16 + (ln & 15);
          if ((!full || nc == ncp - 1) && row < a.M)
            *reinterpret_cast<uint2*>(a.yp + (long long)row * a.np + nc * TROWS + w * (T * 16) + t * 16 + 4 * (ln >> 4)) =
                yq[t][mt];
        }
    }
    FFN_TL(206);
    if (!full) {
      f32x4 ov[T][MT];
#pragma unroll
      for (int j = 0; j < T; ++j)
#pragma unroll
        for (int mt = 0; mt < MT; ++mt) ov[j][mt] = lds_f4(Zo + (mt * 16 + fr) * ZS + (w * T + j) * 16 + 4 * g);
      asm volatile("s_waitcnt lgkmcnt(0)" ::: "memory");
#pragma unroll
      for (int j = 0; j < T; ++j)
#pragma unroll
        for (int mt = 0; mt < MT; ++mt) {
          const int row = m0 + mt * 16 + fr;
          if (row < a.M) *reinterpret_cast<f32x4*>(a.out + (long long)row * D + (w * T + j) * 16 + 4 * g) = ov[j][mt];
        }
    }
    SBK_PROBE(asm volatile("s_waitcnt vmcnt(0)" ::: "memory");)
    FFN_TL(196);
    return;
  }
#pragma unroll
  for (int j = 0; j < T; ++j) {
    const int d = (w * T + j) * 16 + 4 * g;
#pragma unroll
    for (int mt = 0; mt < MT; ++mt) {
      const int row = m0 + mt * 16 + fr;
      if (row < a.M)
        *reinterpret_cast<float4*>(a.out + (long long)row * D + d) =
            make_float4(z[j][mt][0], z[j][mt][1], z[j][mt][2], z[j][mt][3]);
    }
  }
  if (a.gn) {
    row_ln<D, T, MT, NW>(z, red, prm + P_GN * D, prm + P_BN * D, a.epsn, w, g, fr, a.inv_n, a.npad);
#pragma unroll
    for (int j = 0; j < T; ++j) {
      const int d = (w * T + j) * 16 + 4 * g;
#pragma unroll
      for (int mt = 0; mt < MT; ++mt) {
        const int row = m0 + mt * 16 + fr;
        if (row >= a.M) continue;
        if (a.u_bf16) {
          uint2 pk;
          pk.x = pack_bf16x2(z[j][mt][0], z[j][mt][1]);
          pk.y = pack_bf16x2(z[j][mt][2], z[j][mt][3]);
          *reinterpret_cast<uint2*>(reinterpret_cast<bf16_t*>(a.u) + (long long)row * D + d) = pk;
        } else {
          *reinterpret_cast<float4*>(reinterpret_cast<float*>(a.u) + (long long)row * D + d) =
              make_float4(z[j][mt][0], z[j][mt][1], z[j][mt][2], z[j][mt][3]);
        }
      }
    }
  }
  FFN_TL(196);
}

template <int D>
size_t ffn_lds(int H, bool chain) {
  return ((size_t)2 * 256 * 64 + (size_t)FFN_BM * (D + FFN_PAD) + (size_t)2 * FFN_BM * (256 + FFN_PAD)) *
             sizeof(bf16_t) +
         (size_t)(chain ? 2 : 1) * H * 4 + (size_t)FFN_RS * FFN_BM * 4 + (size_t)FFN_NW * D * 4;
}

template <int D, int ACT, bool PROJ, bool CHAIN>
int launch_ffn_act(const FfnArgs& a, size_t lds, hipStream_t s) {
  if (hipError_t e = sbk::lds_optin(reinterpret_cast<const void*>(&ffn_kernel<D, ACT, PROJ, CHAIN>), lds))
    return (int)e;
  hipLaunchKernelGGL((ffn_kernel<D, ACT, PROJ, CHAIN>), dim3((a.M + FFN_BM - 1) / FFN_BM), dim3(FFN_NT), lds, s, a);
  return 0;
}

template <int D, bool PROJ, bool CHAIN>
int launch_ffn(const FfnArgs& a, hipStream_t s) {
  const size_t lds = ffn_lds<D>(a.H, CHAIN);
  if (lds > 160 * 1024) return SBK_ERR_ARG;
  switch (a.act) {
    case ACT_SWISH: return launch_ffn_act<D, ACT_SWISH, PROJ, CHAIN>(a, lds, s);
    case ACT_LRELU: return launch_ffn_act<D, ACT_LRELU, PROJ, CHAIN>(a, lds, s);
    case ACT_GELU: return launch_ffn_act<D, ACT_GELU, PROJ, CHAIN>(a, lds, s);
    case ACT_NONE: return launch_ffn_act<D, ACT_NONE, PROJ, CHAIN>(a, lds, s);
    default: return SBK_ERR_ARG;
  }
}

int ffn_dispatch(const FfnArgs& a, hipStream_t s) {
  const bool proj = a.np > 0, chain = a.g0b != nullptr;
  if (chain) return proj ? launch_ffn<256, true, true>(a, s) : launch_ffn<256, false, true>(a, s);
  return proj ? launch_ffn<256, true, false>(a, s) : launch_ffn<256, false, false>(a, s);
}

struct ImgSrc {
  const bf16_t *w1, *w2, *w1b, *w2b, *wp;
  int D, H, ntile_blk, ntile_ffn, chain;
};

__device__ __forceinline__ void img_tile_src(const ImgSrc& q, int s, const bf16_t** mat, int* ld, int* row0,
                                             int* k0) {
  const int K1 = q.D / 64, SPC = K1 + 4;
  if (s >= q.ntile_ffn) {
    const int pj = s - q.ntile_ffn, nc = pj / K1, r = pj - nc * K1;
    *mat = q.wp; *ld = q.D; *row0 = nc * 256; *k0 = r * 64;
    return;
  }
  const bool sb = s >= q.ntile_blk;
  const int sl = sb ? s - q.ntile_blk : s, c = sl / SPC, r = sl - c * SPC;
  if (r < K1) {
    *mat = sb ? q.w1b : q.w1; *ld = q.D; *row0 = c * 256; *k0 = r * 64;
  } else {
    *mat = sb ? q.w2b : q.w2; *ld = q.H; *row0 = 0; *k0 = c * 256 + (r - K1) * 64;
  }
}

__global__ void __launch_bounds__(256) ffn_image_kernel(ImgSrc q, int ntile, bf16_t* __restrict__ img) {
  const long long n = (long long)ntile * 256 * 8;
  for (long long i = (long long)blockIdx.x * blockDim.x + threadIdx.x; i < n; i += (long long)gridDim.x * blockDim.x) {
    const int s = (int)(i >> 11), rem = (int)(i & 2047), r = rem >> 3, jp = rem & 7;
    const bf16_t* mat;
    int ld, row0, k0;
    img_tile_src(q, s, &mat, &ld, &row0, &k0);
    const int j = jp ^ ((r >> 1) & 7);
    *reinterpret_cast<uint4*>(img + i * 8) =
        *reinterpret_cast<const uint4*>(mat + (long long)(row0 + r) * ld + k0 + 8 * j);
  }
}

int ffn_tiles(int D, int H, int np, int chain) {
  const int per_blk = (H / 256) * (D / 64 + 4);
  return (chain ? 2 : 1) * per_blk + (np / 256) * (D / 64);
}

}

SBK_PROBE_EXPORT(sbk_probe_ffn_tl, g_ffn_tl)

SBK_API int sbk_ffn_supported(int D, int H) { return D == 256 && H > 0 && H % 256 == 0 && H <= 2048; }

SBK_API long long sbk_ffn_image_elems(int D, int H, int np, int chain) {
  if (!sbk_ffn_supported(D, H) || np < 0 || np % 256) return -1;
  return (long long)ffn_tiles(D, H, np, chain) * 256 * 64;
}

SBK_API int sbk_ffn_image(const void* w1, const void* w2, const void* w1b, const void* w2b, const void* wp, int D,
                          int H, int np, void* img, void* stream) {
  const int chain = w1b != nullptr;
  if (!sbk_ffn_supported(D, H) || !w1 || !w2 || !img || (chain && !w2b) || np < 0 || np % 256 || (np > 0) != (wp != nullptr))
    return SBK_ERR_ARG;
  if ((reinterpret_cast<uintptr_t>(w1) | reinterpret_cast<uintptr_t>(w2) | reinterpret_cast<uintptr_t>(w1b) |
       reinterpret_cast<uintptr_t>(w2b) | reinterpret_cast<uintptr_t>(wp) | reinterpret_cast<uintptr_t>(img)) & 15)
    return SBK_ERR_ARG;
  ImgSrc q;
  q.w1 = reinterpret_cast<const bf16_t*>(w1); q.w2 = reinterpret_cast<const bf16_t*>(w2);
  q.w1b = reinterpret_cast<const bf16_t*>(w1b); q.w2b = reinterpret_cast<const bf16_t*>(w2b);
  q.wp = reinterpret_cast<const bf16_t*>(wp);
  q.D = D; q.H = H; q.chain = chain;
  q.ntile_blk = (H / 256) * (D / 64 + 4);
  q.ntile_ffn = (chain ? 2 : 1) * q.ntile_blk;
  const int nt = ffn_tiles(D, H, np, chain);
  const long long chunks = (long long)nt * 2048;
  hipLaunchKernelGGL(ffn_image_kernel, dim3((unsigned)std::min<long long>((chunks + 255) / 256, 4096)), dim3(256), 0,
                     (hipStream_t)stream, q, nt, reinterpret_cast<bf16_t*>(img));
  SBK_CHECK_LAUNCH();
  return 0;
}

namespace {
int ffn_check(const float* x, int M, int D, int H, const float* g0, const float* b0, const void* img,
              long long img_elems, int chain, const float* b1, int act, const float* b2, const float* gp,
              const float* bp, float* out, const float* gn, const float* bn, void* u, int np, void* yp) {
  if (M <= 0 || !sbk_ffn_supported(D, H) || !g0 || !b0 || !img || !b1 || !b2 || !out) return SBK_ERR_ARG;
  if (np < 0 || np % 256 || img_elems != sbk_ffn_image_elems(D, H, np, chain)) return SBK_ERR_ARG;
  if (act == ACT_GLU || act < 0 || act > ACT_GELU || (gn && !u && np == 0)) return SBK_ERR_ARG;
  if (np < 0 || np % 256 || (np > 0 && (!gn || !bn || u || !yp))) return SBK_ERR_ARG;
  const uintptr_t al = reinterpret_cast<uintptr_t>(x) | reinterpret_cast<uintptr_t>(g0) |
                       reinterpret_cast<uintptr_t>(b0) | reinterpret_cast<uintptr_t>(b1) |
                       reinterpret_cast<uintptr_t>(b2) | reinterpret_cast<uintptr_t>(gp) |
                       reinterpret_cast<uintptr_t>(bp) | reinterpret_cast<uintptr_t>(out) |
                       reinterpret_cast<uintptr_t>(gn) | reinterpret_cast<uintptr_t>(bn) |
                       reinterpret_cast<uintptr_t>(u) | reinterpret_cast<uintptr_t>(img) | reinterpret_cast<uintptr_t>(yp);
  return (al & 15) ? SBK_ERR_ARG : 0;
}
}

SBK_API int sbk_ffn_proj(const float* x, int M, int D, int d_eff, int H, const float* g0, const float* b0, float eps0,
                         const void* img, long long img_elems, const float* b1, int act, float slope, const float* b2,
                         float alpha, const float* gp, const float* bp, float epsp, float* out, const float* gn,
                         const float* bn, float epsn, void* u, int u_bf16, int np, void* yp, void* stream) {
  if (ffn_check(x, M, D, H, g0, b0, img, img_elems, 0, b1, act, b2, gp, bp, out, gn, bn, u, np, yp) || d_eff <= 0 ||
      d_eff > D)
    return SBK_ERR_ARG;
  FfnArgs a;
  a.inv_n = 1.0f / (float)d_eff; a.npad = (float)(D - d_eff);
  a.x = x; a.M = M; a.H = H;
  a.g0 = g0; a.b0 = b0; a.eps0 = eps0;
  a.img = reinterpret_cast<const bf16_t*>(img); a.b1 = b1; a.act = act; a.slope = slope;
  a.b2 = b2; a.alpha = alpha;
  a.gp = gp; a.bp = bp; a.epsp = epsp;
  a.out = out;
  a.gn = gn; a.bn = bn; a.epsn = epsn; a.u = u; a.u_bf16 = u_bf16;
  a.np = np; a.yp = reinterpret_cast<bf16_t*>(yp);
  a.g0b = nullptr; a.b0b = nullptr; a.eps0b = 0.f; a.b1b = nullptr; a.b2b = nullptr; a.alphab = 0.f;
  const int rc = ffn_dispatch(a, (hipStream_t)stream);
  if (rc) return rc;
  SBK_CHECK_LAUNCH();
  return 0;
}

SBK_API int sbk_ffn_chain(const float* x, int M, int D, int d_eff, int H, int act, float slope, const float* g0,
                          const float* b0,
                          float eps0, const float* b1, const float* b2, float alpha, const float* gp, const float* bp,
                          float epsp, const float* g0b, const float* b0b, float eps0b, const float* b1b,
                          const float* b2b, float alphab, float* out, const float* gn, const float* bn, float epsn,
                          void* u, int u_bf16, const void* img, long long img_elems, int np, void* yp,
                          void* stream) {
  if (!g0b || !b0b || !b1b || !b2b) return SBK_ERR_ARG;
  if ((reinterpret_cast<uintptr_t>(g0b) | reinterpret_cast<uintptr_t>(b0b) | reinterpret_cast<uintptr_t>(b1b) |
       reinterpret_cast<uintptr_t>(b2b)) & 15)
    return SBK_ERR_ARG;
  if (ffn_check(x, M, D, H, g0, b0, img, img_elems, 1, b1, act, b2, gp, bp, out, gn, bn, u, np, yp) || d_eff <= 0 ||
      d_eff > D)
    return SBK_ERR_ARG;
  FfnArgs a;
  a.inv_n = 1.0f / (float)d_eff; a.npad = (float)(D - d_eff);
  a.x = x; a.M = M; a.H = H;
  a.g0 = g0; a.b0 = b0; a.eps0 = eps0;
  a.img = reinterpret_cast<const bf16_t*>(img); a.b1 = b1; a.act = act; a.slope = slope;
  a.b2 = b2; a.alpha = alpha;
  a.gp = gp; a.bp = bp; a.epsp = epsp;
  a.out = out;
  a.gn = gn; a.bn = bn; a.epsn = epsn; a.u = u; a.u_bf16 = u_bf16;
  a.np = np; a.yp = reinterpret_cast<bf16_t*>(yp);
  a.g0b = g0b; a.b0b = b0b; a.eps0b = eps0b;
  a.b1b = b1b; a.b2b = b2b; a.alphab = alphab;
  const int rc = ffn_dispatch(a, (hipStream_t)stream);
  if (rc) return rc;
  SBK_CHECK_LAUNCH();
  return 0;
}

SBK_API int sbk_ffn(const float* x, int M, int D, int d_eff, int H, const float* g0, const float* b0, float eps0,
                    const void* img, long long img_elems, const float* b1, int act, float slope, const float* b2,
                    float alpha, const float* gp, const float* bp, float epsp, float* out, const float* gn,
                    const float* bn, float epsn, void* u, int u_bf16, void* stream) {
  return sbk_ffn_proj(x, M, D, d_eff, H, g0, b0, eps0, img, img_elems, b1, act, slope, b2, alpha, gp, bp, epsp, out, gn, bn,
                      epsn, u, u_bf16, 0, nullptr, stream);
}
```

speechbrain_amd/lobes/models/transformer/Conformer.py:

```python
from typing import Optional

import torch
import torch.nn as nn

from .... import _autograd as A
from .... import _enc
from ....nnet.activations import Swish
from ....nnet.attention import FUSED_DH_MAX, MultiheadAttention, PositionalwiseFeedForward, RelPosMHAXL
from ....nnet.normalization import LayerNorm

__all__ = ["ConvolutionModule", "ConformerEncoderLayer", "ConformerEncoder"]

_f32 = torch.float32
_bf16 = torch.bfloat16

USE_CONV_MODULE_KERNEL = True
USE_LAYER_CHAIN = True
USE_PADDED_SHADOW = True
PAD_D = 256


def _check_swish(act_module):
    if not (isinstance(act_module, Swish) or type(act_module).__name__ == "Swish"):
        raise NotImplementedError("fused conv module supports the Swish activation only")
    if getattr(act_module, "beta", 1) != 1:
        raise NotImplementedError("Swish(beta != 1) is not fused")


class ConvolutionModule(nn.Module):

    _deff = None

    def __init__(self, input_size, kernel_size=31, bias=True, activation=Swish, dropout=0.0, causal=False,
                 dilation=1):
        super().__init__()
        self.causal = causal
        if dilation != 1:
            raise NotImplementedError("dilated depthwise conv is not on the hot path")
        if self.causal:
            self.padding = (kernel_size - 1) * 2 ** (dilation - 1)
        else:
            self.padding = (kernel_size - 1) * 2 ** (dilation - 1) // 2
        self.layer_norm = nn.LayerNorm(input_size)
        self.bottleneck = nn.Sequential(
            nn.Conv1d(input_size, 2 * input_size, kernel_size=1, stride=1, bias=bias), nn.GLU(dim=1))
        self.conv = nn.Conv1d(input_size, input_size, kernel_size=kernel_size, stride=1, padding=self.padding,
                              dilation=dilation, groups=input_size, bias=bias)
        self.after_conv = nn.Sequential(nn.LayerNorm(input_size), activation(), nn.Linear(input_size, input_size,
                                                                                          bias=bias),
                                        nn.Dropout(dropout))
        self._wc = _enc.WeightCache()

    def kernel_weights(self, dtype):
        w1 = self.bottleneck[0].weight
        b1 = self.bottleneck[0].bias
        w2 = self.after_conv[2].weight

        def make():
            d = w2.shape[0]
            grp = _enc.glu_group()
            perm = []
            for q in range(d // grp):
                perm += list(range(q * grp, (q + 1) * grp))
                perm += list(range(d + q * grp, d + (q + 1) * grp))
            idx = torch.tensor(perm, device=w1.device)
            w1p = w1.detach().reshape(2 * d, d).index_select(0, idx).contiguous()
            b1p = b1.detach().index_select(0, idx).contiguous() if b1 is not None else None
            w2d = w2.detach().contiguous()
            if dtype == _bf16:
                w1p, w2d = _enc.cast_bf16(w1p), _enc.cast_bf16(w2d)
            return w1p, b1p, w2d
        ps = [w1, w2] + ([b1] if b1 is not None else [])
        return self._wc.get(str(dtype), ps, make)

    def ln_params(self):
        return (self.layer_norm.weight.detach(), self.layer_norm.bias.detach(), self.layer_norm.eps)

    def run(self, x2d, B, T, dtype, pad_mask_u8=None, residual=None, u=None):
        d = x2d.shape[1]
        if d % _enc.glu_group():
            raise NotImplementedError("fused GLU needs d_model % 16 == 0")
        _check_swish(self.after_conv[1])
        w1p, b1p, w2 = self.kernel_weights(dtype)
        if u is None:
            u, _ = _enc.layernorm(x2d, *self.ln_params(), out1_dtype=dtype)
        g = _enc.gemm(u, w1p, bias=b1p, act="glu", out_dtype=dtype)
        ln = self.after_conv[0]
        v = _enc.dwconv_ln_swish(g, B, T, self.conv.weight.detach(), self.conv.bias.detach() if self.conv.bias is not None
                                 else None, self.causal, ln.weight.detach(), ln.bias.detach(), ln.eps, dtype)
        lin = self.after_conv[2]
        return _enc.gemm(v, w2, bias=lin.bias.detach() if lin.bias is not None else None, rowmask=pad_mask_u8,
                         res=residual, out_dtype=_f32)

    def fusable(self, dtype, d):
        return (dtype == _bf16 and _enc.conv_module_supported(d, self.conv.weight.shape[-1])
                and self.bottleneck[0].bias is not None and isinstance(self.after_conv[1], Swish)
                and getattr(self.after_conv[1], "beta", 1) == 1)

    def run_fused(self, x2d, B, T, pad_mask_u8=None, pre=None):
        w1p, b1p, w2 = self.kernel_weights(_bf16)
        ln = self.after_conv[0]
        lin = self.after_conv[2]
        wc = self._wc.get("taps", [self.conv.weight], lambda: self.conv.weight.detach().reshape(
            self.conv.weight.shape[0], -1).t().contiguous())
        return _enc.conv_module(x2d, B, T, self.ln_params(), w1p, b1p, wc,
                                self.conv.bias.detach() if self.conv.bias is not None else None, self.causal,
                                (ln.weight.detach(), ln.bias.detach(), ln.eps), w2,
                                lin.bias.detach() if lin.bias is not None else None, pad_mask_u8, pre=pre,
                                deff=self._deff)

    def train_run(self, x2d, B, T, dtype, pad_mask_u8=None, residual=None):
        _check_swish(self.after_conv[1])
        d = x2d.shape[1]
        u = A.layer_norm(x2d, self.layer_norm, out_dtype=dtype)
        pw = self.bottleneck[0]
        h = A.linear(u, pw.weight, pw.bias, dtype, self._wc, "t_pw", out_dtype=dtype)
        g = A.act(h, "glu")
        c = A.DwConvFn.apply(g, self.conv.weight, self.conv.bias, B, T, self.causal)
        n = A.layer_norm(c, self.after_conv[0], out_dtype=_f32)
        s = A.act(n, "swish", out_dtype=dtype)
        lin = self.after_conv[2]
        p = self.after_conv[3].p if self.training else 0.0
        if p == 0:
            return A.linear(s, lin.weight, lin.bias, dtype, self._wc, "t_lin", res=residual, rowmask=pad_mask_u8)
        y = A.linear(s, lin.weight, lin.bias, dtype, self._wc, "t_lin")
        return A.DropAddFn.apply(y, residual, 1.0, pad_mask_u8, float(p), _f32)

    def forward(self, x, mask=None):
        B, T, d = x.shape
        m = mask.reshape(B * T).to(torch.uint8).contiguous() if mask is not None else None
        x2d = x.float().reshape(B * T, d).contiguous()
        if A.needs_grad(self, x) or (self.training and self.after_conv[3].p > 0):
            return self.train_run(x2d, B, T, _enc.compute_dtype(), m).view(B, T, d)
        return self.run(x2d, B, T, _enc.compute_dtype(), m).view(B, T, d)


class ConformerEncoderLayer(nn.Module):

    def __init__(self, d_model, d_ffn, nhead, kernel_size=31, kdim=None, vdim=None, activation=Swish, bias=True,
                 dropout=0.0, causal=False, attention_type="RelPosMHAXL"):
        super().__init__()
        if attention_type == "regularMHA":
            self.mha_layer = MultiheadAttention(nhead=nhead, d_model=d_model, dropout=dropout, kdim=kdim, vdim=vdim)
        elif attention_type == "RelPosMHAXL":
            self.mha_layer = RelPosMHAXL(num_heads=nhead, embed_dim=d_model, dropout=dropout,
                                         mask_pos_future=causal)
        else:
            raise ValueError(f"attention_type {attention_type!r}: 'regularMHA' or 'RelPosMHAXL'")
        self.attention_type = attention_type
        self.module_layer = attention_type == "regularMHA" or d_model // nhead > FUSED_DH_MAX
        self.convolution_module = ConvolutionModule(d_model, kernel_size, bias, activation, dropout, causal=causal)
        self.ffn_module1 = nn.Sequential(
            nn.LayerNorm(d_model),
            PositionalwiseFeedForward(d_ffn=d_ffn, input_size=d_model, dropout=dropout, activation=activation),
            nn.Dropout(dropout))
        self.ffn_module2 = nn.Sequential(
            nn.LayerNorm(d_model),
            PositionalwiseFeedForward(d_ffn=d_ffn, input_size=d_model, dropout=dropout, activation=activation),
            nn.Dropout(dropout))
        self.norm1 = LayerNorm(d_model)
        self.norm2 = LayerNorm(d_model)
        self.drop = nn.Dropout(dropout)

    def _ln(self, mod):
        return mod.weight.detach(), mod.bias.detach(), mod.eps

    def chainable(self, dtype, d):
        if self.training and self.drop.p > 0 or self.module_layer:
            return False
        f1, f2 = self.ffn_module1, self.ffn_module2
        mha = self.mha_layer
        return (f1[1].fusable(dtype) and f2[1].fusable(dtype) and f1[1].act_name() == f2[1].act_name()
                and f1[1].ffn[0].out_features == f2[1].ffn[0].out_features
                and hasattr(mha, "fused_in_proj") and mha.fused_in_proj(dtype) is not None
                and self.convolution_module.fusable(dtype, d))

    def fused(self, x, B, T, pos, kpm_u8, dtype, need_attn, u_in=None, next_ln=None, final_ln=None, pk=None,
              am=None):
        if self.training and self.drop.p > 0:
            raise NotImplementedError("dropout in training mode is not implemented in HIP yet")
        f1, f2 = self.ffn_module1, self.ffn_module2
        if f1[1].fusable(dtype) and f2[1].fusable(dtype):
            wq = self.mha_layer.fused_in_proj(dtype) if hasattr(self.mha_layer, "fused_in_proj") else None
            qkv = None
            if wq is not None:
                x, qkv = f1[1].run_fused_proj(x, self._ln(f1[0]), 0.5, self._ln(self.norm1.norm), wq)
                u = None
            else:
                x, u = f1[1].run_fused(x, self._ln(f1[0]), 0.5, next_ln=self._ln(self.norm1.norm),
                                       next_dtype=dtype)
            cm = self.convolution_module
            if USE_CONV_MODULE_KERNEL and cm.fusable(dtype, x.shape[1]):
                if hasattr(self.mha_layer, "attend_heads"):
                    o, attn, pre = self.mha_layer.attend_heads(u, B, T, pos, kpm_u8, dtype, need_attn, pk=pk,
                                                               qkv=qkv, am=am)
                    x = cm.run_fused(x, B, T, kpm_u8, pre=pre)
                else:
                    x, attn = self.mha_layer.attend(u, B, T, pos, kpm_u8, dtype, need_attn, residual=x, pk=pk,
                                                    qkv=qkv, am=am)
                    x = cm.run_fused(x, B, T, kpm_u8)
            else:
                x, attn, uc = self.mha_layer.attend(u, B, T, pos, kpm_u8, dtype, need_attn, residual=x,
                                                    post_ln=cm.ln_params(), pk=pk, qkv=qkv, am=am)
                x = cm.run(x, B, T, dtype, kpm_u8, residual=x, u=uc)
            x, y = f2[1].run_fused(x, self._ln(f2[0]), 0.5, post_ln=self._ln(self.norm2.norm), out=x,
                                   next_ln=final_ln, next_dtype=_f32)
            return (y, None, attn, True) if final_ln is not None else (x, None, attn, False)
        if u_in is None:
            u_in, _ = _enc.layernorm(x, *self._ln(f1[0]), out1_dtype=dtype)
        x = f1[1].run(u_in, dtype, residual=x, alpha=0.5)
        u, _ = _enc.layernorm(x, *self._ln(self.norm1.norm), out1_dtype=dtype)
        x, attn, uc = self.mha_layer.attend(u, B, T, pos, kpm_u8, dtype, need_attn, residual=x,
                                            post_ln=self.convolution_module.ln_params(), pk=pk, am=am)
        x = self.convolution_module.run(x, B, T, dtype, kpm_u8, residual=x, u=uc)
        u, _ = _enc.layernorm(x, *self._ln(f2[0]), out1_dtype=dtype)
        z = f2[1].run(u, dtype, residual=x, alpha=0.5)
        w2, b2, e2 = self._ln(self.norm2.norm)
        if next_ln is not None:
            x, u_next = _enc.layernorm(z, w2, b2, e2, out1_dtype=_f32, w2=next_ln[0], b2=next_ln[1],
                                       eps2=next_ln[2], out2_dtype=dtype)
            return x, u_next, attn, False
        x, _ = _enc.layernorm(z, w2, b2, e2, out1_dtype=_f32)
        return x, None, attn, False

    def train_layer(self, x, B, T, pos, kpm_u8, dtype, am=None):
        f1, f2 = self.ffn_module1, self.ffn_module2
        tr = self.training
        u = A.layer_norm(x, f1[0], out_dtype=dtype)
        x = f1[1].train_run(u, dtype, residual=x, alpha=0.5, out_p=f1[2].p if tr else 0.0)
        u = A.layer_norm(x, self.norm1.norm, out_dtype=dtype)
        x, attn = self.mha_layer.train_attend(u, B, T, pos, kpm_u8, dtype, residual=x, am=am)
        x = self.convolution_module.train_run(x, B, T, dtype, kpm_u8, residual=x)
        u = A.layer_norm(x, f2[0], out_dtype=dtype)
        z = f2[1].train_run(u, dtype, residual=x, alpha=0.5, out_p=f2[2].p if tr else 0.0)
        return A.layer_norm(z, self.norm2.norm, out_dtype=_f32), attn

    def mha_layer_forward(self, x, B, T, kpm_u8, src_mask, pos_embs, dtype):
        f1, f2 = self.ffn_module1, self.ffn_module2
        tr = self.training
        d = x.shape[1]
        u = A.layer_norm(x, f1[0], out_dtype=dtype)
        x = f1[1].train_run(u, dtype, residual=x, alpha=0.5, out_p=f1[2].p if tr else 0.0)
        u = A.layer_norm(x, self.norm1.norm, out_dtype=_f32).view(B, T, d)
        o, attn = self.mha_layer(u, u, u, attn_mask=src_mask, key_padding_mask=kpm_u8, pos_embs=pos_embs)
        x = A.DropAddFn.apply(o.reshape(B * T, d).float(), x, 1.0, None, 0.0, _f32)
        x = self.convolution_module.train_run(x, B, T, dtype, kpm_u8, residual=x)
        u = A.layer_norm(x, f2[0], out_dtype=dtype)
        z = f2[1].train_run(u, dtype, residual=x, alpha=0.5, out_p=f2[2].p if tr else 0.0)
        return A.layer_norm(z, self.norm2.norm, out_dtype=_f32), attn

    def wants_train_path(self, x):
        return A.needs_grad(self, x) or (self.training and self.ffn_module1[2].p > 0)

    def forward(self, x, src_mask: Optional[torch.Tensor] = None,
                src_key_padding_mask: Optional[torch.Tensor] = None, pos_embs: Optional[torch.Tensor] = None):
        B, T, d = x.shape
        dtype = _enc.compute_dtype()
        kpm = src_key_padding_mask.to(torch.uint8).contiguous() if src_key_padding_mask is not None else None
        if self.module_layer:
            y, attn = self.mha_layer_forward(x.float().reshape(B * T, d).contiguous(), B, T, kpm, src_mask,
                                             pos_embs, dtype)
            return y.view(B, T, d), attn
        am = _enc.attn_mask_arg(src_mask, B, T, self.mha_layer.num_heads, x.device)
        x2d = x.float().reshape(B * T, d).contiguous()
        if self.wants_train_path(x):
            y, attn = self.train_layer(x2d, B, T, pos_embs.reshape(-1, d).float(), kpm, dtype, am=am)
            return y.view(B, T, d), attn
        pos = _enc.to_compute(pos_embs.reshape(-1, d), dtype)
        y, _, attn, _ = self.fused(x2d, B, T, pos, kpm, dtype, True, am=am)
        return y.view(B, T, d), attn


class ConformerEncoder(nn.Module):

    def __init__(self, num_layers, d_model, d_ffn, nhead, kernel_size=31, kdim=None, vdim=None, activation=Swish,
                 bias=True, dropout=0.0, causal=False, attention_type="RelPosMHAXL"):
        super().__init__()
        self.layers = torch.nn.ModuleList([
            ConformerEncoderLayer(d_ffn=d_ffn, nhead=nhead, d_model=d_model, kdim=kdim, vdim=vdim, dropout=dropout,
                                  activation=activation, kernel_size=kernel_size, bias=bias, causal=causal,
                                  attention_type=attention_type) for i in range(num_layers)])
        self.norm = LayerNorm(d_model, eps=1e-6)
        self.attention_type = attention_type
        self._wc = _enc.WeightCache()

    def stacked_pos_weight(self, dtype):
        ws = [layer.mha_layer.linear_pos.weight for layer in self.layers]

        def make():
            w = torch.cat([p.detach() for p in ws], dim=0).contiguous()
            return _enc.cast_bf16(w) if dtype == _bf16 else w
        return self._wc.get(("pos", dtype), ws, make)

    def train_run(self, src2d, B, T, pos_embs, kpm_u8, dtype, am=None):
        d = src2d.shape[1]
        pos = pos_embs.reshape(-1, d).float()
        x = src2d
        attns = []
        for layer in self.layers:
            x, a = layer.train_layer(x, B, T, pos, kpm_u8, dtype, am=am)
            attns.append(a)
        return A.layer_norm(x, self.norm.norm, out_dtype=_f32), attns

    def wants_train_path(self, x):
        return any(layer.wants_train_path(x) for layer in self.layers) or A.needs_grad(self.norm, x)

    def _shadow(self, d, dtype, am=None):
        if USE_PADDED_SHADOW and am is None and dtype == _bf16 and d < PAD_D:
            return _PaddedEncoder.of(self)
        return None

    def run(self, src2d, B, T, pos_embs, kpm_u8, dtype, need_attn, am=None):
        if self.wants_train_path(src2d):
            return self.train_run(src2d, B, T, pos_embs, kpm_u8, dtype, am=am)
        d = src2d.shape[1]
        sh = self._shadow(d, dtype, am)
        if sh is not None:
            return sh.run(src2d, B, T, pos_embs, kpm_u8, dtype, need_attn)
        pos = _enc.to_compute(pos_embs.reshape(-1, d), dtype)
        pk_all = _enc.gemm(pos, self.stacked_pos_weight(dtype), out_dtype=dtype)
        x = src2d
        u = None
        attns = []
        n = len(self.layers)
        if (USE_LAYER_CHAIN and am is None and all(layer.chainable(dtype, d) for layer in self.layers)
                and self._uniform_ffns()):
            return self._run_chain(x, B, T, pos, kpm_u8, dtype, need_attn, pk_all)
        for i, layer in enumerate(self.layers):
            nxt = self.layers[i + 1].ffn_module1[0] if i + 1 < n else None
            next_ln = (nxt.weight.detach(), nxt.bias.detach(), nxt.eps) if nxt is not None else None
            fn = self.norm.norm
            final_ln = (fn.weight.detach(), fn.bias.detach(), fn.eps) if nxt is None else None
            x, u, a, done = layer.fused(x, B, T, pos, kpm_u8, dtype, need_attn, u_in=u, next_ln=next_ln,
                                        final_ln=final_ln, pk=pk_all[:, i * d:(i + 1) * d], am=am)
            attns.append(a)
            if done:
                return x, attns
        fn = self.norm.norm
        y, _ = _enc.layernorm(x, fn.weight.detach(), fn.bias.detach(), fn.eps, out1_dtype=_f32)
        return y, attns

    def _uniform_ffns(self):
        f = [m[1] for layer in self.layers for m in (layer.ffn_module1, layer.ffn_module2)]
        return all(x.act_name() == f[0].act_name() and x.ffn[0].out_features == f[0].ffn[0].out_features for x in f)

    def _run_chain(self, x, B, T, pos, kpm_u8, dtype, need_attn, pk_all):
        d = x.shape[1]
        ln = ConformerEncoderLayer._ln
        L = self.layers
        l0 = L[0]
        f1 = l0.ffn_module1
        x, qkv = f1[1].run_fused_proj(x, ln(l0, f1[0]), 0.5, ln(l0, l0.norm1.norm), l0.mha_layer.fused_in_proj(dtype))
        attns = []
        for i, layer in enumerate(L):
            _, attn, pre = layer.mha_layer.attend_heads(None, B, T, pos, kpm_u8, dtype, need_attn,
                                                        pk=pk_all[:, i * d:(i + 1) * d], qkv=qkv)
            attns.append(attn)
            x = layer.convolution_module.run_fused(x, B, T, kpm_u8, pre=pre)
            f2 = layer.ffn_module2
            if i + 1 < len(L):
                nl = L[i + 1]
                a = f2[1].chain_block(ln(layer, f2[0]), 0.5, post_ln=ln(layer, layer.norm2.norm))
                b = nl.ffn_module1[1].chain_block(ln(nl, nl.ffn_module1[0]), 0.5)
                act, slope = f2[1].act_name()
                x, qkv = _enc.ffn_chain(x, a, b, act, slope, ln(nl, nl.norm1.norm), nl.mha_layer.fused_in_proj(dtype),
                                        deff=f2[1]._deff)
            else:
                fn = self.norm.norm
                _, y = f2[1].run_fused(x, ln(layer, f2[0]), 0.5, post_ln=ln(layer, layer.norm2.norm),
                                       next_ln=(fn.weight.detach(), fn.bias.detach(), fn.eps), next_dtype=_f32)
                return y, attns

    def forward(self, src, src_mask: Optional[torch.Tensor] = None,
                src_key_padding_mask: Optional[torch.Tensor] = None, pos_embs: Optional[torch.Tensor] = None):
        if self.attention_type == "RelPosMHAXL" and pos_embs is None:
            raise ValueError("The chosen attention type for the Conformer is RelPosMHAXL. For this attention type, "
                             "the positional embeddings are mandatory")
        B, T, d = src.shape
        kpm = src_key_padding_mask.to(torch.uint8).contiguous() if src_key_padding_mask is not None else None
        if self.layers[0].module_layer:
            x = src.float().reshape(B * T, d).contiguous()
            attns = []
            for layer in self.layers:
                x, a = layer.mha_layer_forward(x, B, T, kpm, src_mask, pos_embs, _enc.compute_dtype())
                attns.append(a)
            return A.layer_norm(x, self.norm.norm, out_dtype=_f32).view(B, T, d), attns
        am = _enc.attn_mask_arg(src_mask, B, T, self.layers[0].mha_layer.num_heads, src.device)
        y, attns = self.run(src.float().reshape(B * T, d).contiguous(), B, T, pos_embs, kpm,
                            _enc.compute_dtype(), True, am=am)
        return y.view(B, T, d), attns


class _PaddedEncoder:

    def __init__(self, enc, dev):
        d = enc.norm.norm.weight.shape[0]
        l0 = enc.layers[0]
        H = l0.mha_layer.num_heads
        K = l0.convolution_module.conv.weight.shape[-1]
        F = l0.ffn_module1[1].ffn[0].out_features
        act = type(l0.ffn_module1[1].ffn[1])
        self.d = d
        with torch.random.fork_rng(devices=[]):
            sh = ConformerEncoder(len(enc.layers), PAD_D, F, H, kernel_size=K, activation=act,
                                  bias=l0.convolution_module.conv.bias is not None,
                                  causal=l0.convolution_module.causal)
        sh = sh.to(dev).eval()
        dh, dp = d // H, PAD_D // H
        hmap = torch.tensor([h * dp + i for h in range(H) for i in range(dh)], device=dev)
        qmap = torch.tensor([h * 3 * dp + p * dp + i for h in range(H) for p in range(3) for i in range(dh)],
                            device=dev)
        gmap = torch.cat([torch.arange(d, device=dev), PAD_D + torch.arange(d, device=dev)])

        def put(dst, src, rows=None, cols=None):
            src = src.detach().to(dev, torch.float32)
            dst.zero_()
            r = rows if rows is not None else torch.arange(src.shape[0], device=dev)
            if dst.dim() == 1:
                dst[r] = src
                return
            tmp = torch.zeros(src.shape[0], *dst.shape[1:], device=dev)
            if cols is None:
                tmp[:, :src.shape[1]] = src
            else:
                tmp[:, cols] = src
            dst[r] = tmp

        with torch.no_grad():
            for lr, ls in zip(enc.layers, sh.layers):
                for fr_, fs in ((lr.ffn_module1, ls.ffn_module1), (lr.ffn_module2, ls.ffn_module2)):
                    put(fs[0].weight, fr_[0].weight)
                    put(fs[0].bias, fr_[0].bias)
                    put(fs[1].ffn[0].weight, fr_[1].ffn[0].weight, rows=torch.arange(F, device=dev))
                    put(fs[1].ffn[0].bias, fr_[1].ffn[0].bias, rows=torch.arange(F, device=dev))
                    put(fs[1].ffn[3].weight, fr_[1].ffn[3].weight)
                    put(fs[1].ffn[3].bias, fr_[1].ffn[3].bias)
                    fs[1]._deff = d
                mr, ms = lr.mha_layer, ls.mha_layer
                put(ms.in_proj_weight, mr.in_proj_weight, rows=qmap)
                put(ms.pos_bias_u.view(-1), mr.pos_bias_u.reshape(-1), rows=hmap)
                put(ms.pos_bias_v.view(-1), mr.pos_bias_v.reshape(-1), rows=hmap)
                put(ms.linear_pos.weight, mr.linear_pos.weight, rows=hmap)
                put(ms.out_proj.weight, mr.out_proj.weight, cols=hmap)
                put(ms.out_proj.bias, mr.out_proj.bias)
                ms.scale = mr.scale
                cr, cs = lr.convolution_module, ls.convolution_module
                put(cs.layer_norm.weight, cr.layer_norm.weight)
                put(cs.layer_norm.bias, cr.layer_norm.bias)
                put(cs.bottleneck[0].weight.view(2 * PAD_D, PAD_D), cr.bottleneck[0].weight.view(2 * d, d), rows=gmap)
                if cr.bottleneck[0].bias is not None:
                    put(cs.bottleneck[0].bias, cr.bottleneck[0].bias, rows=gmap)
                put(cs.conv.weight.view(PAD_D, K), cr.conv.weight.view(d, K))
                if cr.conv.bias is not None:
                    put(cs.conv.bias, cr.conv.bias)
                put(cs.after_conv[0].weight, cr.after_conv[0].weight)
                put(cs.after_conv[0].bias, cr.after_conv[0].bias)
                put(cs.after_conv[2].weight, cr.after_conv[2].weight)
                if cr.after_conv[2].bias is not None:
                    put(cs.after_conv[2].bias, cr.after_conv[2].bias)
                cs._deff = d
                for nr, ns in ((lr.norm1.norm, ls.norm1.norm), (lr.norm2.norm, ls.norm2.norm)):
                    put(ns.weight, nr.weight)
                    put(ns.bias, nr.bias)
                    ns.eps = nr.eps
                for a, b in ((lr.ffn_module1[0], ls.ffn_module1[0]), (lr.ffn_module2[0], ls.ffn_module2[0]),
                             (cr.layer_norm, cs.layer_norm), (cr.after_conv[0], cs.after_conv[0])):
                    b.eps = a.eps
            put(sh.norm.norm.weight, enc.norm.norm.weight)
            put(sh.norm.norm.bias, enc.norm.norm.bias)
            sh.norm.norm.eps = enc.norm.norm.eps
        self.sh = sh
        self._pos = {}

    @staticmethod
    def of(enc):
        ps = list(enc.parameters())
        dev = ps[0].device
        sig = (str(dev),) + tuple((p.data_ptr(), p._version) for p in ps)
        hit = getattr(enc, "_padded_shadow", None)
        if hit is not None and hit[0] == sig:
            return hit[1]
        l0 = enc.layers[0]
        d = enc.norm.norm.weight.shape[0]
        ok = (l0.attention_type == "RelPosMHAXL" and not l0.module_layer and d % l0.mha_layer.num_heads == 0
              and PAD_D % l0.mha_layer.num_heads == 0 and l0.mha_layer.vbias is None
              and l0.mha_layer._qkv_same_embed_dim and enc._uniform_ffns())
        shadow = None
        if ok:
            shadow = _PaddedEncoder(enc, dev)
            if not (all(layer.chainable(_bf16, PAD_D) for layer in shadow.sh.layers) and shadow.sh._uniform_ffns()):
                shadow = None
        enc._padded_shadow = (sig, shadow)
        return shadow

    def padded_pos(self, pos_embs, dtype):
        d = self.d
        key = (pos_embs.data_ptr(), tuple(pos_embs.shape), dtype)
        pos = self._pos.get(key)
        if pos is None:
            p = pos_embs.reshape(-1, d)
            pos = torch.zeros(p.shape[0], PAD_D, device=p.device, dtype=dtype)
            pos[:, :d] = p.to(dtype)
            self._pos = {key: pos}
        return pos

    def run(self, src2d, B, T, pos_embs, kpm_u8, dtype, need_attn):
        d = self.d
        if src2d.shape[1] == PAD_D:
            x = src2d
        else:
            x = torch.zeros(src2d.shape[0], PAD_D, device=src2d.device, dtype=torch.float32)
            x[:, :d] = src2d
        y, attns = self.sh.run(x, B, T, self.padded_pos(pos_embs, dtype), kpm_u8, dtype, need_attn)
        return y[:, :d].contiguous(), attns
```

Measured before the change: 384,100 audio-sec/sec.

## Fuse conformer conv module into the FFN chain kernel per layer

Adds a conv_ffn_chain kernel that runs the attention output projection, the conv module (LN, pointwise GLU, depthwise conv, LN-swish, pointwise) and the following FFN chain with next-layer QKV projection in one launch. The conv weights are pre-packed into a swizzled bf16 image and cached. This removes a kernel launch and the global-memory round trip of the conv module output between stages. In exchange it recomputes halo rows for the depthwise conv, and LDS pressure is high, which may lower occupancy.

```diff
diff --git a/include/sbk.h b/include/sbk.h
--- a/include/sbk.h
+++ b/include/sbk.h
@@ -132,6 +132,19 @@
                   float epsp, const float* g0b, const float* b0b, float eps0b, const float* b1b, const float* b2b,
                   float alphab, float* out, const float* gn, const float* bn, float epsn, void* u, int u_bf16,
                   const void* img, long long img_elems, int np, void* yp, void* stream);
+
+long long sbk_conv_image_elems(int D);
+int sbk_conv_image(const void* w1p, const void* w2, int D, void* img, void* stream);
+
+int sbk_conv_ffn_chain(const float* x, const void* o, const void* wo, const float* bo, int B, int T, int D, int d_eff,
+                       const float* cln0_w, const float* cln0_b, float ceps0, const void* cimg, long long cimg_elems,
+                       const float* cb1p, const float* wc, const float* bc, int K, int causal, const float* cln1_w,
+                       const float* cln1_b, float ceps1, const float* cb2, const unsigned char* kpm, int H, int act,
+                       float slope, const float* g0, const float* b0, float eps0, const float* b1, const float* b2,
+                       float alpha, const float* gp, const float* bp, float epsp, const float* g0b, const float* b0b,
+                       float eps0b, const float* b1b, const float* b2b, float alphab, float* out, const float* gn,
+                       const float* bn, float epsn, const void* img, long long img_elems, int np, void* yp,
+                       void* stream);
 
 int sbk_layernorm(const float* x, int M, int D, const float* g1, const float* b1, float eps1, void* out1,
                   int out1_bf16, const float* g2, const float* b2, float eps2, void* out2, int out2_bf16,
diff --git a/speechbrain_amd/_enc.py b/speechbrain_amd/_enc.py
--- a/speechbrain_amd/_enc.py
+++ b/speechbrain_amd/_enc.py
@@ -257,18 +257,23 @@
     def _drop(self, key):
         self._d.pop(key, None)
 
-    def get(self, ws, np_, stream):
+    @staticmethod
+    def _build_ffn(ws, np_, stream):
+        w1, w2, w1b, w2b, wp = ws
+        D, H = w1.shape[1], w1.shape[0]
+        n = int(lib().sbk_ffn_image_elems(D, H, np_, int(w1b is not None)))
+        if n <= 0:
+            raise SbkError(f"sbk_ffn_image_elems: unsupported shape D={D} H={H} np={np_}")
+        img = torch.empty(n, device=w1.device, dtype=_bf16)
+        check(lib().sbk_ffn_image(ptr(w1), ptr(w2), ptr(w1b), ptr(w2b), ptr(wp), D, H, np_, ptr(img),
+                                  ctypes.c_void_p(stream.cuda_stream)), "sbk_ffn_image")
+        return img
+
+    def get(self, ws, np_, stream, build=None):
         key = tuple((w.data_ptr(), w._version) if w is not None else None for w in ws) + (np_,)
         hit = self._d.pop(key, None)
         if hit is None:
-            w1, w2, w1b, w2b, wp = ws
-            D, H = w1.shape[1], w1.shape[0]
-            n = int(lib().sbk_ffn_image_elems(D, H, np_, int(w1b is not None)))
-            if n <= 0:
-                raise SbkError(f"sbk_ffn_image_elems: unsupported shape D={D} H={H} np={np_}")
-            img = torch.empty(n, device=w1.device, dtype=_bf16)
-            check(lib().sbk_ffn_image(ptr(w1), ptr(w2), ptr(w1b), ptr(w2b), ptr(wp), D, H, np_, ptr(img),
-                                      ctypes.c_void_p(stream.cuda_stream)), "sbk_ffn_image")
+            img = (build or self._build_ffn)(ws, np_, stream)
             ev = torch.cuda.Event()
             ev.record(stream)
             refs = tuple(weakref.ref(w, lambda _r, k=key: self._drop(k)) for w in ws if w is not None)
@@ -290,6 +295,27 @@
             raise TypeError("ffn_image: contiguous bf16 weights")
     img = _FFN_IMAGES.get((w1, w2, w1b, w2b, wp), 0 if wp is None else wp.shape[0], torch.cuda.current_stream(w1.device))
     return img
+
+
+_CONV_IMAGES = _ImageCache()
+
+
+def _build_conv_image(ws, np_, stream):
+    w1p, w2 = ws
+    D = w2.shape[0]
+    n = int(lib().sbk_conv_image_elems(D))
+    if n <= 0 or tuple(w1p.shape) != (2 * D, D) or tuple(w2.shape) != (D, D):
+        raise SbkError(f"sbk_conv_image: unsupported shapes {tuple(w1p.shape)}, {tuple(w2.shape)}")
+    img = torch.empty(n, device=w1p.device, dtype=_bf16)
+    check(lib().sbk_conv_image(ptr(w1p), ptr(w2), D, ptr(img), ctypes.c_void_p(stream.cuda_stream)), "sbk_conv_image")
+    return img
+
+
+def conv_image(w1p, w2):
+    for t in (w1p, w2):
+        if t.dtype != _bf16 or not t.is_contiguous():
+            raise TypeError("conv_image: contiguous bf16 weights")
+    return _CONV_IMAGES.get((w1p, w2), 0, torch.cuda.current_stream(w1p.device), build=_build_conv_image)
 
 
 @custom_op("sbk::ffn", mutates_args=())
@@ -387,6 +413,69 @@
                          int(deff or x.shape[1]))
 
 
+@custom_op("sbk::conv_ffn_chain", mutates_args=())
+def _conv_ffn_chain_op(x: torch.Tensor, B: int, T: int, o: torch.Tensor, wo: torch.Tensor, bo: Optional[torch.Tensor],
+                       cg0: torch.Tensor, cb0: torch.Tensor, ce0: float, w1p: torch.Tensor, b1p: torch.Tensor,
+                       wc: torch.Tensor, bc: Optional[torch.Tensor], causal: bool, cg1: torch.Tensor,
+                       cb1: torch.Tensor, ce1: float, cw2: torch.Tensor, cb2: Optional[torch.Tensor],
+                       kpm: Optional[torch.Tensor], act: int, slope: float, g0: torch.Tensor, b0: torch.Tensor,
+                       e0: float, w1: torch.Tensor, b1: torch.Tensor, w2: torch.Tensor, b2: torch.Tensor, alpha: float,
+                       gp: Optional[torch.Tensor], bp: Optional[torch.Tensor], ep: float, g0b: torch.Tensor,
+                       b0b: torch.Tensor, e0b: float, w1b: torch.Tensor, b1b: torch.Tensor, w2b: torch.Tensor,
+                       b2b: torch.Tensor, alphab: float, gn: torch.Tensor, bn: torch.Tensor, en: float,
+                       wp: torch.Tensor, deff: int) -> tuple[torch.Tensor, torch.Tensor]:
+    M, NP = x.shape[0], wp.shape[0]
+    if M != B * T:
+        raise ValueError(f"conv_ffn_chain: x has {M} rows, B * T = {B * T}")
+    out = torch.empty_like(x)
+    y = torch.empty(M, NP, device=x.device, dtype=_bf16)
+    _conv_ffn_chain_into(out, y, x, B, T, o, wo, bo, cg0, cb0, ce0, w1p, b1p, wc, bc, causal, cg1, cb1, ce1, cw2, cb2,
+                         kpm, act, slope, g0, b0, e0, w1, b1, w2, b2, alpha, gp, bp, ep, g0b, b0b, e0b, w1b, b1b, w2b,
+                         b2b, alphab, gn, bn, en, wp, deff)
+    return out, y
+
+
+def _conv_ffn_chain_into(out, y, x, B, T, o, wo, bo, cg0, cb0, ce0, w1p, b1p, wc, bc, causal, cg1, cb1, ce1, cw2, cb2,
+                         kpm, act, slope, g0, b0, e0, w1, b1, w2, b2, alpha, gp, bp, ep, g0b, b0b, e0b, w1b, b1b, w2b,
+                         b2b, alphab, gn, bn, en, wp, deff):
+    D = x.shape[1]
+    H, NP = w1.shape[0], wp.shape[0]
+    cimg = conv_image(w1p, cw2)
+    img = ffn_image(w1, w2, w1b, w2b, wp)
+    rc = lib().sbk_conv_ffn_chain(ptr(x), ptr(o), ptr(wo), ptr(bo), B, T, D, deff, ptr(cg0), ptr(cb0), float(ce0),
+                                  ptr(cimg), cimg.numel(), ptr(b1p), ptr(wc), ptr(bc), wc.shape[0], int(causal),
+                                  ptr(cg1), ptr(cb1), float(ce1), ptr(cb2), ptr(kpm), H, act, float(slope), ptr(g0),
+                                  ptr(b0), float(e0), ptr(b1), ptr(b2), float(alpha), ptr(gp), ptr(bp), float(ep),
+                                  ptr(g0b), ptr(b0b), float(e0b), ptr(b1b), ptr(b2b), float(alphab), ptr(out), ptr(gn),
+                                  ptr(bn), float(en), ptr(img), img.numel(), NP, ptr(y), stream_of(x))
+    check(rc, "sbk_conv_ffn_chain")
+
+
+@_conv_ffn_chain_op.register_fake
+def _(x, B, T, o, wo, bo, cg0, cb0, ce0, w1p, b1p, wc, bc, causal, cg1, cb1, ce1, cw2, cb2, kpm, act, slope, g0, b0,
+      e0, w1, b1, w2, b2, alpha, gp, bp, ep, g0b, b0b, e0b, w1b, b1b, w2b, b2b, alphab, gn, bn, en, wp, deff):
+    return torch.empty_like(x), x.new_empty((x.shape[0], wp.shape[0]), dtype=_bf16)
+
+
+def conv_ffn_chain_supported(D, K, H, NP):
+    return conv_module_supported(D, K) and ffn_proj_supported(D, H, NP) and H <= 1024
+
+
+def conv_ffn_chain(x, B, T, pre, conv, kpm, a, b, act, slope, next_ln, wp, deff=None):
+    o, wo, bo = pre
+    cln0, w1p, b1p, wc, bc, causal, cln1, cw2, cb2 = conv
+    require_device(x, o, wo, w1p, cw2, a[1], b[1], wp)
+    if b[1].shape != a[1].shape or b[3].shape != a[3].shape:
+        raise ValueError(f"conv_ffn_chain: block shapes differ ({tuple(a[1].shape)}/{tuple(a[3].shape)} vs "
+                         f"{tuple(b[1].shape)}/{tuple(b[3].shape)})")
+    gp, bp, ep = a[6] if a[6] is not None else (None, None, 0.0)
+    return OPS.conv_ffn_chain(x, int(B), int(T), o, wo, bo, cln0[0], cln0[1], float(cln0[2]), w1p, b1p, wc, bc,
+                              bool(causal), cln1[0], cln1[1], float(cln1[2]), cw2, cb2, kpm, ACT[act], float(slope),
+                              a[0][0], a[0][1], float(a[0][2]), a[1], a[2], a[3], a[4], float(a[5]), gp, bp, float(ep),
+                              b[0][0], b[0][1], float(b[0][2]), b[1], b[2], b[3], b[4], float(b[5]), next_ln[0],
+                              next_ln[1], float(next_ln[2]), wp, int(deff or x.shape[1]))
+
+
 def ffn(x, ln0, w1, b1, act, slope, w2, b2, alpha, post_ln=None, next_ln=None, next_dtype=_bf16, out=None, deff=None):
     require_device(x, w1, w2)
     gp, bp, ep = post_ln if post_ln is not None else (None, None, 0.0)
diff --git a/speechbrain_amd/_lib.py b/speechbrain_amd/_lib.py
--- a/speechbrain_amd/_lib.py
+++ b/speechbrain_amd/_lib.py
@@ -55,6 +55,11 @@
                      _vp, _i, _i, _vp, _vp],
     "sbk_ffn_image_elems": [_i, _i, _i, _i],
     "sbk_ffn_image": [_vp, _vp, _vp, _vp, _vp, _i, _i, _i, _vp, _vp],
+    "sbk_conv_image_elems": [_i],
+    "sbk_conv_image": [_vp, _vp, _i, _vp, _vp],
+    "sbk_conv_ffn_chain": [_vp, _vp, _vp, _vp, _i, _i, _i, _i, _vp, _vp, _f, _vp, _ll, _vp, _vp, _vp, _i, _i, _vp, _vp,
+                           _f, _vp, _vp, _i, _i, _f, _vp, _vp, _f, _vp, _vp, _f, _vp, _vp, _f, _vp, _vp, _f, _vp, _vp,
+                           _f, _vp, _vp, _vp, _f, _vp, _ll, _i, _vp, _vp],
     "sbk_layernorm": [_vp, _i, _i, _vp, _vp, _f, _vp, _i, _vp, _vp, _f, _vp, _i, _vp],
     "sbk_dwconv_ln_swish": [_i, _vp, _i, _i, _i, _vp, _vp, _i, _i, _vp, _vp, _f, _vp, _i, _vp],
     "sbk_conv_block_c1": [_vp, _i, _i, _i, _i, _vp, _vp, _vp, _vp, _f, _f, _vp, _i, _vp, _vp, _vp],
@@ -126,7 +131,7 @@
     "sbk_joint_bwd": [_vp, _vp, _vp, _i, _i, _i, _i, _i, _i, _f, _vp, _vp, _vp, _vp],
     "sbk_joint_bwd_workspace_floats": [_i, _i, _i, _i],
 }
-RESTYPES = {"sbk_relpos_attention_lds": ctypes.c_longlong, "sbk_mx_gemm_ws_floats": ctypes.c_longlong, "sbk_ffn_image_elems": ctypes.c_longlong, "sbk_joint_bwd_workspace_floats": ctypes.c_longlong, "sbk_rnnt_workspace_floats": ctypes.c_longlong, "sbk_ctc_workspace_floats": ctypes.c_longlong}
+RESTYPES = {"sbk_relpos_attention_lds": ctypes.c_longlong, "sbk_mx_gemm_ws_floats": ctypes.c_longlong, "sbk_ffn_image_elems": ctypes.c_longlong, "sbk_conv_image_elems": ctypes.c_longlong, "sbk_joint_bwd_workspace_floats": ctypes.c_longlong, "sbk_rnnt_workspace_floats": ctypes.c_longlong, "sbk_ctc_workspace_floats": ctypes.c_longlong}
 
 _lib = None
 _load_error = None
diff --git a/speechbrain_amd/csrc/convstage.h b/speechbrain_amd/csrc/convstage.h
--- /dev/null
+++ b/speechbrain_amd/csrc/convstage.h
@@ -0,0 +1,427 @@
+#pragma once
+
+struct ConvStageArgs {
+  const float* x;
+  int B, T, K, padL;
+  const float *g0, *b0;
+  float eps0;
+  const bf16_t* img;
+  const float* b1;
+  const float* wc;
+  const float* bc;
+  const float *g1, *b1n;
+  float eps1;
+  const float* b2;
+  const uint8_t* kpm;
+  const bf16_t* o;
+  const bf16_t* wo;
+  const float* bo;
+};
+
+constexpr int CS_D = 256, CS_BM = FFN_BM, CS_KMAX = 31;
+constexpr int CS_ROWS = 80;
+constexpr int CS_MT1 = CS_ROWS / 16, CS_MT3 = CS_BM / 16;
+constexpr int CS_NW = FFN_NW, CS_NT = FFN_NT;
+constexpr int CS_S = CS_D + FFN_PAD;
+constexpr int CS_TILE = 256 * 64;
+constexpr int CS_P1T = 8, CS_P3T = 4;
+constexpr int CS_OFF_G = CS_ROWS * CS_S * 2, CS_OFF_CV = 2 * CS_OFF_G;
+constexpr int CS_LDS = CS_OFF_CV + CS_BM * CS_D * 4;
+static_assert(CS_TILE * 2 <= CS_OFF_G && CS_TILE * 2 <= CS_BM * CS_D * 4, "ring slots fit");
+
+#pragma clang diagnostic push
+#pragma clang diagnostic ignored "-Winline-asm"
+__device__ __forceinline__ void cs_issue(const bf16_t* img, int tile, bf16_t* slot, int w, int lane) {
+  const bf16_t* src = img + (long long)tile * CS_TILE + w * 2048 + lane * 8;
+  const uint32_t la = __builtin_amdgcn_readfirstlane(lds_addr(slot + w * 2048));
+  asm volatile(
+      "s_mov_b32 m0, %1\n\ts_nop 0\n\t"
+      "global_load_lds_dwordx4 %0, off\n\t"
+      "global_load_lds_dwordx4 %0, off offset:1024\n\t"
+      "global_load_lds_dwordx4 %0, off offset:2048\n\t"
+      "global_load_lds_dwordx4 %0, off offset:3072" ::"v"(src),
+      "s"(la)
+      : "memory", "m0");
+}
+#pragma clang diagnostic pop
+__device__ __forceinline__ bf16x8 cs_frag(const bf16_t* slot, int row, int c) {
+  return *reinterpret_cast<const bf16x8*>(slot + row * 64 + ((c ^ ((row >> 1) & 7)) << 3));
+}
+__device__ __forceinline__ int cs_gldu8(const uint8_t* p) {
+  int v;
+  asm volatile("global_load_ubyte %0, %1, off" : "=v"(v) : "v"(p) : "memory");
+  return v;
+}
+__device__ __forceinline__ void cs_barrier() {
+  asm volatile("s_waitcnt lgkmcnt(0)" ::: "memory");
+  __builtin_amdgcn_s_barrier();
+  asm volatile("" ::: "memory");
+}
+
+template <typename F>
+__device__ __forceinline__ void conv_stage(const ConvStageArgs& a, float inv_n, float npad, unsigned char* smem, int b,
+                                           int t0, f32x4 (&zres)[2][CS_MT3], F&& stage) {
+  bf16_t* Us = reinterpret_cast<bf16_t*>(smem);
+  bf16_t* Gs = reinterpret_cast<bf16_t*>(smem + CS_OFF_G);
+  float* Cv = reinterpret_cast<float*>(smem + CS_OFF_CV);
+  bf16_t* slot[2] = {Gs, reinterpret_cast<bf16_t*>(Cv)};
+
+  const int tid = threadIdx.x, lane = tid & 63, w = tid >> 6;
+  const int fr = lane & 15, g = lane >> 4, fk = 8 * g;
+  const int fks = fk ^ ffn_sw(fr);
+  const int f0 = t0 - a.padL;
+  const int nrows = CS_BM + a.K - 1;
+  const long long ubase = (long long)b * a.T;
+
+  float4 xres[2][CS_MT3];
+  {
+    constexpr int OC = CS_ROWS * (CS_D / 8) / CS_NT;
+    static_assert(OC * CS_NT == CS_ROWS * (CS_D / 8), "whole chunks");
+    uint4 ov[OC];
+#pragma unroll
+    for (int i = 0; i < OC; ++i) {
+      const int c = tid + i * CS_NT;
+      const int r = c / (CS_D / 8), ch = c - r * (CS_D / 8);
+      const int fc = min(max(f0 + r, 0), a.T - 1);
+      ov[i] = *reinterpret_cast<const uint4*>(a.o + (ubase + fc) * CS_D + ch * 8);
+    }
+    float* lnscr = Cv + CS_TILE / 2;
+    constexpr int RS = CS_NW + 4;
+    static_assert(CS_TILE / 2 + 2 * CS_ROWS * RS + 2 * CS_ROWS + 2 * CS_D <= CS_BM * CS_D, "LN0 scratch fits");
+    float* gb0s = lnscr + 2 * CS_ROWS * RS + 2 * CS_ROWS;
+    const float4 gbv = tid < CS_D / 2 ? *reinterpret_cast<const float4*>((tid < CS_D / 4 ? a.g0 : a.b0) +
+                                                                         4 * (tid % (CS_D / 4)))
+                                      : make_float4(0.f, 0.f, 0.f, 0.f);
+    float4 xv[2][CS_MT1], bo4[2];
+    bf16x8 fwo[2][CS_D / 32];
+#pragma unroll
+    for (int j = 0; j < 2; ++j) {
+      const int u0 = (w * 2 + j) * 16 + 4 * g;
+#pragma unroll
+      for (int mt = 0; mt < CS_MT1; ++mt) {
+        const int f = min(max(f0 + mt * 16 + fr, 0), a.T - 1);
+        xv[j][mt] = *reinterpret_cast<const float4*>(a.x + (ubase + f) * CS_D + u0);
+      }
+      bo4[j] = a.bo ? *reinterpret_cast<const float4*>(a.bo + u0) : make_float4(0.f, 0.f, 0.f, 0.f);
+      const bf16_t* wrowo = a.wo + (long long)((w * 2 + j) * 16 + fr) * CS_D + fk;
+#pragma unroll
+      for (int kk = 0; kk < CS_D / 32; ++kk) fwo[j][kk] = ld8(wrowo + kk * 32);
+    }
+#pragma unroll
+    for (int i = 0; i < OC; ++i) {
+      const int c = tid + i * CS_NT;
+      const int r = c / (CS_D / 8), ch = c - r * (CS_D / 8), f = f0 + r;
+      const bool live = r < nrows && f >= 0 && f < a.T;
+      *reinterpret_cast<uint4*>(Gs + r * CS_S + ((ch * 8) ^ ffn_sw(r))) = live ? ov[i] : uint4{0u, 0u, 0u, 0u};
+    }
+    if (tid < CS_D / 2) *reinterpret_cast<float4*>(gb0s + 4 * tid) = gbv;
+    stage();
+    cs_barrier();
+    f32x4 acc[2][CS_MT1];
+#pragma unroll
+    for (int j = 0; j < 2; ++j)
+#pragma unroll
+      for (int mt = 0; mt < CS_MT1; ++mt) acc[j][mt] = f32x4{0.f, 0.f, 0.f, 0.f};
+#pragma unroll
+    for (int kk = 0; kk < CS_D / 32; ++kk)
+#pragma unroll
+      for (int mt = 0; mt < CS_MT1; ++mt) {
+        const bf16x8 fo = *reinterpret_cast<const bf16x8*>(Gs + (mt * 16 + fr) * CS_S + kk * 32 + fks);
+#pragma unroll
+        for (int j = 0; j < 2; ++j) acc[j][mt] = FFN_MFMA(fwo[j][kk], fo, acc[j][mt]);
+      }
+    float xa[2][CS_MT1][4];
+#pragma unroll
+    for (int j = 0; j < 2; ++j)
+#pragma unroll
+      for (int mt = 0; mt < CS_MT1; ++mt) {
+        xa[j][mt][0] = xv[j][mt].x + (acc[j][mt][0] + bo4[j].x);
+        xa[j][mt][1] = xv[j][mt].y + (acc[j][mt][1] + bo4[j].y);
+        xa[j][mt][2] = xv[j][mt].z + (acc[j][mt][2] + bo4[j].z);
+        xa[j][mt][3] = xv[j][mt].w + (acc[j][mt][3] + bo4[j].w);
+      }
+    {
+      const int q = a.padL >> 4, rr = a.padL & 15;
+      const int src = ((lane & 0x30) + ((fr + rr) & 15)) << 2;
+      const bool hi = fr + rr >= 16;
+#pragma unroll
+      for (int j = 0; j < 2; ++j)
+#pragma unroll
+        for (int mt = 0; mt < CS_MT3; ++mt) {
+          float v[4];
+#pragma unroll
+          for (int e = 0; e < 4; ++e) {
+            const float lo_v = q == 0 ? xa[j][mt][e] : xa[j][mt + 1][e];
+            const float hi_v = q == 0 ? xa[j][mt + 1][e] : xa[j][mt + 2][e];
+            const float lo = __int_as_float(__builtin_amdgcn_ds_bpermute(src, __float_as_int(lo_v)));
+            const float hv = __int_as_float(__builtin_amdgcn_ds_bpermute(src, __float_as_int(hi_v)));
+            v[e] = hi ? hv : lo;
+          }
+          xres[j][mt] = make_float4(v[0], v[1], v[2], v[3]);
+        }
+    }
+    float* red = lnscr;
+#pragma unroll
+    for (int mt = 0; mt < CS_MT1; ++mt) {
+      float s = 0.f, q2 = 0.f;
+#pragma unroll
+      for (int j = 0; j < 2; ++j) {
+        s += (xa[j][mt][0] + xa[j][mt][1]) + (xa[j][mt][2] + xa[j][mt][3]);
+        q2 += (xa[j][mt][0] * xa[j][mt][0] + xa[j][mt][1] * xa[j][mt][1]) +
+              (xa[j][mt][2] * xa[j][mt][2] + xa[j][mt][3] * xa[j][mt][3]);
+      }
+      const float ps = col4_sum(s), pq = col4_sum(q2);
+      if (g == 0) {
+        red[(mt * 16 + fr) * RS + w] = ps;
+        red[CS_ROWS * RS + (mt * 16 + fr) * RS + w] = pq;
+      }
+    }
+    cs_barrier();
+    cs_issue(a.img, 0, slot[0], w, lane);
+    cs_issue(a.img, 1, slot[1], w, lane);
+    float* stat = red + 2 * CS_ROWS * RS;
+    if (w < (CS_ROWS + 63) / 64 && w * 64 + lane < CS_ROWS) {
+      const int row = w * 64 + lane;
+      float t = 0.f, t2 = 0.f;
+#pragma unroll
+      for (int k4 = 0; k4 < CS_NW / 4; ++k4) {
+        const float4 a4 = *reinterpret_cast<const float4*>(red + row * RS + 4 * k4);
+        const float4 q4 = *reinterpret_cast<const float4*>(red + CS_ROWS * RS + row * RS + 4 * k4);
+        t += a4.x; t += a4.y; t += a4.z; t += a4.w;
+        t2 += q4.x; t2 += q4.y; t2 += q4.z; t2 += q4.w;
+      }
+      const float mu = t * inv_n;
+      stat[row] = mu;
+      stat[CS_ROWS + row] = 1.0f / sqrtf(fmaxf(t2 * inv_n - mu * mu, 0.f) + a.eps0);
+    }
+    cs_barrier();
+#pragma unroll
+    for (int j = 0; j < 2; ++j) {
+      const int u0 = (w * 2 + j) * 16 + 4 * g;
+      const float4 g04 = *reinterpret_cast<const float4*>(gb0s + u0);
+      const float4 b04 = *reinterpret_cast<const float4*>(gb0s + CS_D + u0);
+#pragma unroll
+      for (int mt = 0; mt < CS_MT1; ++mt) {
+        const float mean = stat[mt * 16 + fr], rstd = stat[CS_ROWS + mt * 16 + fr];
+        const int r = mt * 16 + fr, f = f0 + r;
+        const bool live = r < nrows && f >= 0 && f < a.T;
+        uint2 pk = make_uint2(0u, 0u);
+        if (live) {
+          pk.x = pack_bf16x2((xa[j][mt][0] - mean) * rstd * g04.x + b04.x, (xa[j][mt][1] - mean) * rstd * g04.y + b04.y);
+          pk.y = pack_bf16x2((xa[j][mt][2] - mean) * rstd * g04.z + b04.z, (xa[j][mt][3] - mean) * rstd * g04.w + b04.w);
+        }
+        *reinterpret_cast<uint2*>(Us + r * CS_S + (u0 ^ ffn_sw(fr))) = pk;
+      }
+    }
+  }
+  cs_barrier();
+
+  {
+    f32x4 acc[2][2][CS_MT1];
+#pragma unroll
+    for (int h = 0; h < 2; ++h)
+#pragma unroll
+      for (int t = 0; t < 2; ++t)
+#pragma unroll
+        for (int mt = 0; mt < CS_MT1; ++mt) acc[h][t][mt] = f32x4{0.f, 0.f, 0.f, 0.f};
+    bf16x8 fa[2][CS_MT1];
+#pragma unroll
+    for (int q = 0; q < CS_P1T; ++q) {
+      const int kt = q >> 1, h = q & 1;
+      if (q + 1 < CS_P1T)
+        asm volatile("s_waitcnt vmcnt(4)" ::: "memory");
+      else
+        asm volatile("s_waitcnt vmcnt(0)" ::: "memory");
+      bf16x8 fw[2][2];
+#pragma unroll
+      for (int ks = 0; ks < 2; ++ks)
+#pragma unroll
+        for (int t = 0; t < 2; ++t) fw[ks][t] = cs_frag(slot[q & 1], w * 32 + t * 16 + fr, ks * 4 + g);
+      if (h == 0) {
+#pragma unroll
+        for (int ks = 0; ks < 2; ++ks)
+#pragma unroll
+          for (int mt = 0; mt < CS_MT1; ++mt)
+            fa[ks][mt] = *reinterpret_cast<const bf16x8*>(Us + (mt * 16 + fr) * CS_S + kt * 64 + ks * 32 + fks);
+      }
+      asm volatile("s_waitcnt lgkmcnt(0)" ::: "memory");
+      if (q + 2 < CS_P1T) cs_issue(a.img, q + 2, slot[q & 1], w, lane);
+#pragma unroll
+      for (int ks = 0; ks < 2; ++ks)
+#pragma unroll
+        for (int t = 0; t < 2; ++t)
+#pragma unroll
+          for (int mt = 0; mt < CS_MT1; ++mt) acc[h][t][mt] = FFN_MFMA(fw[ks][t], fa[ks][mt], acc[h][t][mt]);
+    }
+    cs_barrier();
+#pragma unroll
+    for (int h = 0; h < 2; ++h) {
+      const int ch = (w * 2 + h) * 16 + 4 * g;
+      const int pa = (w * 2 + h) * 32 + 4 * g, pg = pa + 16;
+      const float4 ba = *reinterpret_cast<const float4*>(a.b1 + pa);
+      const float4 bg = *reinterpret_cast<const float4*>(a.b1 + pg);
+      const float bav[4] = {ba.x, ba.y, ba.z, ba.w}, bgv[4] = {bg.x, bg.y, bg.z, bg.w};
+#pragma unroll
+      for (int mt = 0; mt < CS_MT1; ++mt) {
+        const int r = mt * 16 + fr, f = f0 + r;
+        const bool live = r < nrows && f >= 0 && f < a.T;
+        float o[4];
+#pragma unroll
+        for (int e = 0; e < 4; ++e) {
+          const float va = acc[h][0][mt][e] + bav[e], vg = acc[h][1][mt][e] + bgv[e];
+          const float sg = va * __builtin_amdgcn_rcpf(1.0f + __expf(-vg));
+          o[e] = live ? sg : 0.f;
+        }
+        uint2 pk;
+        pk.x = pack_bf16x2(o[0], o[1]);
+        pk.y = pack_bf16x2(o[2], o[3]);
+        *reinterpret_cast<uint2*>(Gs + r * CS_S + (ch ^ ffn_sw(fr))) = pk;
+      }
+    }
+  }
+  cs_barrier();
+
+  {
+    const int c = tid & (CS_D - 1), h = tid >> 8;
+    constexpr int NF = CS_BM / (CS_NT / CS_D);
+    constexpr int NP = (CS_KMAX + 1) / 2;
+    float wk[2 * NP];
+#pragma unroll
+    for (int k = 0; k < 2 * NP; ++k) {
+      const float v = a.wc[min(k, a.K - 1) * CS_D + c];
+      wk[k] = k < a.K ? v : 0.f;
+    }
+    const float bias = a.bc ? a.bc[c] : 0.f;
+    static_assert((CS_NT / CS_D - 1) * NF + NF + 2 * NP - 1 <= CS_ROWS, "every window row is staged");
+    static_assert(NF % 4 == 0, "h * NF keeps bits 0-1 of the row; frame pairs");
+    typedef __bf16 bf2 __attribute__((ext_vector_type(2)));
+    bf2 tp[NP], ev[NF / 2 + NP - 1], od[NF / 2 + NP - 1];
+#pragma unroll
+    for (int j = 0; j < NP; ++j) {
+      tp[j] = __builtin_bit_cast(bf2, pack_bf16x2(wk[2 * j], wk[2 * j + 1]));
+      asm volatile("" : "+v"(tp[j]));
+    }
+    const int cx = c ^ ffn_sw(h * NF);
+    const unsigned short* Gu0 = reinterpret_cast<const unsigned short*>(Gs) + h * NF * CS_S + cx;
+    const unsigned short* Gu1 = reinterpret_cast<const unsigned short*>(Gs) + h * NF * CS_S + (cx ^ 8);
+    auto gu = [&](int k) __attribute__((always_inline)) { return (uint32_t)(ffn_sw(k) ? Gu1 : Gu0)[k * CS_S]; };
+    uint32_t g0 = gu(0);
+#pragma unroll
+    for (int r = 0; r < NF / 2 + NP - 1; ++r) {
+      const uint32_t g1 = gu(2 * r + 1), g2 = gu(2 * r + 2);
+      ev[r] = __builtin_bit_cast(bf2, g0 | (g1 << 16));
+      od[r] = __builtin_bit_cast(bf2, g1 | (g2 << 16));
+      g0 = g2;
+    }
+#pragma unroll
+    for (int i = 0; i < NF; ++i) {
+      float s = bias;
+#pragma unroll
+      for (int j = 0; j < NP; ++j) s = __builtin_amdgcn_fdot2_f32_bf16(tp[j], (i & 1) ? od[i / 2 + j] : ev[i / 2 + j], s, false);
+      Cv[(h * NF + i) * CS_D + c] = s;
+    }
+  }
+  cs_barrier();
+
+  f32x4 bb2[2] = {f32x4{0.f, 0.f, 0.f, 0.f}, f32x4{0.f, 0.f, 0.f, 0.f}};
+  int km[CS_MT3] = {};
+  {
+    f32x4 g14 = gld4(a.g1 + lane * 4), b14 = gld4(a.b1n + lane * 4);
+    const float* b2p = a.b2 ? a.b2 : a.g1;
+#pragma unroll
+    for (int j = 0; j < 2; ++j) bb2[j] = gld4(b2p + (w * 2 + j) * 16 + 4 * g);
+#pragma unroll
+    for (int mt = 0; mt < CS_MT3; ++mt)
+      km[mt] = cs_gldu8(a.kpm ? a.kpm + ubase + min(t0 + mt * 16 + fr, a.T - 1) : reinterpret_cast<const uint8_t*>(a.g1));
+    cs_issue(a.img, CS_P1T, slot[0], w, lane);
+    asm volatile("s_waitcnt vmcnt(4)" ::: "memory");
+    vtie(g14);
+    vtie(b14);
+    vtie(bb2[0]);
+    vtie(bb2[1]);
+#pragma unroll
+    for (int mt = 0; mt < CS_MT3; ++mt) asm volatile("" : "+v"(km[mt]));
+    if (!a.b2) bb2[0] = bb2[1] = f32x4{0.f, 0.f, 0.f, 0.f};
+    if (!a.kpm) km[0] = km[1] = km[2] = 0;
+    const float gm[4] = {g14[0], g14[1], g14[2], g14[3]}, bt[4] = {b14[0], b14[1], b14[2], b14[3]};
+    constexpr int FPW = CS_BM / CS_NW;
+    float v[FPW][4], mean[FPW], rstd[FPW];
+#pragma unroll
+    for (int u = 0; u < FPW; ++u) {
+      const float4 v4 = *reinterpret_cast<const float4*>(Cv + (w + u * CS_NW) * CS_D + lane * 4);
+      v[u][0] = v4.x; v[u][1] = v4.y; v[u][2] = v4.z; v[u][3] = v4.w;
+    }
+#pragma unroll
+    for (int u = 0; u < FPW; ++u) mean[u] = wave_sum_v((v[u][0] + v[u][1]) + (v[u][2] + v[u][3])) * inv_n;
+#pragma unroll
+    for (int u = 0; u < FPW; ++u) {
+      float q = 0.f;
+#pragma unroll
+      for (int e = 0; e < 4; ++e) q += (v[u][e] - mean[u]) * (v[u][e] - mean[u]);
+      rstd[u] = q;
+    }
+#pragma unroll
+    for (int u = 0; u < FPW; ++u)
+      rstd[u] = 1.0f / sqrtf((wave_sum_v(rstd[u]) - npad * mean[u] * mean[u]) * inv_n + a.eps1);
+#pragma unroll
+    for (int u = 0; u < FPW; ++u) {
+#pragma unroll
+      for (int e = 0; e < 4; ++e) {
+        const float z = (v[u][e] - mean[u]) * rstd[u] * gm[e] + bt[e];
+        v[u][e] = z * __builtin_amdgcn_rcpf(1.0f + __expf(-z));
+      }
+      uint2 pk;
+      pk.x = pack_bf16x2(v[u][0], v[u][1]);
+      pk.y = pack_bf16x2(v[u][2], v[u][3]);
+      *reinterpret_cast<uint2*>(Us + (w + u * CS_NW) * CS_S + ((lane * 4) ^ ffn_sw(w))) = pk;
+    }
+  }
+  cs_barrier();
+
+  {
+    f32x4 acc[2][CS_MT3];
+#pragma unroll
+    for (int j = 0; j < 2; ++j)
+#pragma unroll
+      for (int mt = 0; mt < CS_MT3; ++mt) acc[j][mt] = f32x4{0.f, 0.f, 0.f, 0.f};
+    cs_issue(a.img, CS_P1T + 1, slot[1], w, lane);
+#pragma unroll
+    for (int kt = 0; kt < CS_P3T; ++kt) {
+      if (kt + 1 < CS_P3T)
+        asm volatile("s_waitcnt vmcnt(4)" ::: "memory");
+      else
+        asm volatile("s_waitcnt vmcnt(0)" ::: "memory");
+      bf16x8 fw[2][2], fa[2][CS_MT3];
+#pragma unroll
+      for (int ks = 0; ks < 2; ++ks) {
+#pragma unroll
+        for (int j = 0; j < 2; ++j) fw[ks][j] = cs_frag(slot[kt & 1], w * 32 + j * 16 + fr, ks * 4 + g);
+#pragma unroll
+        for (int mt = 0; mt < CS_MT3; ++mt)
+          fa[ks][mt] = *reinterpret_cast<const bf16x8*>(Us + (mt * 16 + fr) * CS_S + kt * 64 + ks * 32 + fks);
+      }
+      asm volatile("s_waitcnt lgkmcnt(0)" ::: "memory");
+      if (kt + 2 < CS_P3T) cs_issue(a.img, CS_P1T + kt + 2, slot[kt & 1], w, lane);
+#pragma unroll
+      for (int ks = 0; ks < 2; ++ks)
+#pragma unroll
+        for (int j = 0; j < 2; ++j)
+#pragma unroll
+          for (int mt = 0; mt < CS_MT3; ++mt) acc[j][mt] = FFN_MFMA(fw[ks][j], fa[ks][mt], acc[j][mt]);
+    }
+#pragma unroll
+    for (int j = 0; j < 2; ++j)
+#pragma unroll
+      for (int mt = 0; mt < CS_MT3; ++mt) {
+        const bool live = t0 + mt * 16 + fr < a.T;
+        const bool m = km[mt] != 0;
+        const float4 xv = xres[j][mt];
+        f32x4 o;
+        o[0] = xv.x + (m ? 0.f : acc[j][mt][0] + bb2[j][0]);
+        o[1] = xv.y + (m ? 0.f : acc[j][mt][1] + bb2[j][1]);
+        o[2] = xv.z + (m ? 0.f : acc[j][mt][2] + bb2[j][2]);
+        o[3] = xv.w + (m ? 0.f : acc[j][mt][3] + bb2[j][3]);
+        zres[j][mt] = live ? o : f32x4{0.f, 0.f, 0.f, 0.f};
+      }
+  }
+}
diff --git a/speechbrain_amd/csrc/ffn.hip b/speechbrain_amd/csrc/ffn.hip
--- a/speechbrain_amd/csrc/ffn.hip
+++ b/speechbrain_amd/csrc/ffn.hip
@@ -194,12 +194,13 @@
       for (int mt = 0; mt < MT; ++mt) tie(xa[r][ks][mt]);
 }
 
+#include "convstage.h"
 
 SBK_PROBE_BUFFER(g_ffn_tl, 16, 256)
 #define FFN_TL(i) SBK_PROBE(if (tl_rec >= 0 && lane == 0) g_ffn_tl[tl_rec][i] = __builtin_amdgcn_s_memtime();)
 
-template <int D, int ACT, bool PROJ, bool CHAIN>
-__global__ void __launch_bounds__(FFN_NT) ffn_kernel(FfnArgs a) {
+template <int D, int ACT, bool PROJ, bool CHAIN, bool CONV>
+__device__ __forceinline__ void ffn_body(const FfnArgs& a, const ConvStageArgs* cs) {
   constexpr int BM = FFN_BM, HC = 256, NW = FFN_NW, NT = FFN_NT;
   constexpr int XS = D + FFN_PAD, HS = HC + FFN_PAD;
   constexpr int MT = BM / 16;
@@ -225,7 +226,12 @@
 
   const int tid = threadIdx.x, lane = tid & 63, w = tid >> 6;
   const int fr = lane & 15, g = lane >> 4, fk = (8 * g) ^ ffn_sw(fr);
-  const int m0 = blockIdx.x * BM;
+  int m0 = blockIdx.x * BM, mlim = a.M;
+  if constexpr (CONV) {
+    const int nblk = (cs->T + BM - 1) / BM, b = blockIdx.x / nblk;
+    m0 = b * cs->T + (blockIdx.x - b * nblk) * BM;
+    mlim = (b + 1) * cs->T;
+  }
   const int NCH = a.H / HC;
   const int S = NCH * SPC;
   const int SF = CHAIN ? 2 * S : S;
@@ -247,17 +253,65 @@
   };
   constexpr int NRW = (BM + NW - 1) / NW;
   f32x4 xres[T][MT];
+  if constexpr (CONV) {
+    static_assert(T == 2 && MT == CS_MT3 && CHAIN && PROJ, "conv_stage hands over the chain's residual layout");
+    float* ga0 = reinterpret_cast<float*>(smem + CS_LDS);
+    static_assert(CS_LDS + 2 * D * 4 <= (NB * TROWS * BK + BM * XS + 2 * BM * HS) * 2, "LN0 affine below b1");
+    static_assert(CS_LDS >= (NB * TROWS * BK + BM * XS + BM * HS) * 2, "LN0 affine in the second hidden buffer");
+    const float* psrc = w == P_B2 ? a.b2 : w == P_GP ? a.gp : w == P_BP ? a.bp : w == P_G0B ? a.g0b
+                      : w == P_B0B ? a.b0b : w == P_B2B ? a.b2b : w == P_GN ? a.gn : a.bn;
+    const bool b1t = tid * 4 < a.H;
+    const float4 z4 = make_float4(0.f, 0.f, 0.f, 0.f);
+    float4 pv = z4, b1v = z4, b1bv = z4, gav = z4;
+    if (psrc) pv = *reinterpret_cast<const float4*>(psrc + lane * PER);
+    if (b1t) {
+      b1v = *reinterpret_cast<const float4*>(a.b1 + tid * 4);
+      b1bv = *reinterpret_cast<const float4*>(a.b1b + tid * 4);
+    }
+    if (tid < D / 2) gav = *reinterpret_cast<const float4*>((tid < D / 4 ? a.g0 : a.b0) + 4 * (tid % (D / 4)));
+    const int nblk = (cs->T + BM - 1) / BM, ub = blockIdx.x / nblk;
+    conv_stage(*cs, a.inv_n, a.npad, smem, ub, (blockIdx.x - ub * nblk) * BM, xres, [&]() __attribute__((always_inline)) {
+      if (psrc) *reinterpret_cast<float4*>(prm + w * D + lane * PER) = pv;
+      if (b1t) {
+        *reinterpret_cast<float4*>(b1s + tid * 4) = b1v;
+        *reinterpret_cast<float4*>(b1s + a.H + tid * 4) = b1bv;
+      }
+      if (tid < D / 2) *reinterpret_cast<float4*>(ga0 + 4 * tid) = gav;
+    });
+    lds_barrier();
+    issue(0, 0);
+    issue(1, 1);
+    float z[T][MT][4];
+#pragma unroll
+    for (int j = 0; j < T; ++j)
+#pragma unroll
+      for (int mt = 0; mt < MT; ++mt)
+#pragma unroll
+        for (int e = 0; e < 4; ++e) z[j][mt][e] = xres[j][mt][e];
+    row_ln<D, T, MT, NW>(z, red, ga0, ga0 + D, a.eps0, w, g, fr, a.inv_n, a.npad);
+#pragma unroll
+    for (int j = 0; j < T; ++j) {
+      const int d = (w * T + j) * 16 + 4 * g;
+#pragma unroll
+      for (int mt = 0; mt < MT; ++mt) {
+        uint2 pk;
+        pk.x = pack_bf16x2(z[j][mt][0], z[j][mt][1]);
+        pk.y = pack_bf16x2(z[j][mt][2], z[j][mt][3]);
+        lds_st2(Xn + (mt * 16 + fr) * XS + (d ^ ffn_sw(fr)), pk);
+      }
+    }
+  } else {
 #pragma unroll
   for (int j = 0; j < T; ++j)
 #pragma unroll
     for (int mt = 0; mt < MT; ++mt) {
-      const int row = min(m0 + mt * 16 + fr, a.M - 1);
+      const int row = min(m0 + mt * 16 + fr, mlim - 1);
       xres[j][mt] = gld4(a.x + (long long)row * D + (w * T + j) * 16 + 4 * g);
     }
   f32x4 xv[NRW];
 #pragma unroll
   for (int i = 0; i < NRW; ++i) {
-    const int rr = w + i * NW, row = min(m0 + rr, a.M - 1);
+    const int rr = w + i * NW, row = min(m0 + rr, mlim - 1);
     xv[i] = gld4(a.x + (long long)row * D + lane * PER);
   }
   f32x4 g04 = gld4(a.g0 + lane * PER), b04 = gld4(a.b0 + lane * PER);
@@ -287,7 +341,7 @@
   for (int i = 0; i < NRW; ++i) {
     const int rr = w + i * NW;
     if (rr >= BM) break;
-    const bool live = m0 + rr < a.M;
+    const bool live = m0 + rr < mlim;
     const float v[4] = {live ? xv[i][0] : 0.f, live ? xv[i][1] : 0.f, live ? xv[i][2] : 0.f, live ? xv[i][3] : 0.f};
     const float mean = wave_sum_v(v[0] + v[1] + v[2] + v[3]) * a.inv_n;
     float q = 0.f;
@@ -303,6 +357,7 @@
   if (psrc) lds_st4(prm + w * D + lane * PER, pv);
   if (b1t) lds_st4(b1s + tid * 4, b1v);
   if (CHAIN && b1t) lds_st4(b1s + a.H + tid * 4, b1bv);
+  }
 
   f32x4 acc1[T][MT], acc2[T][MT];
 #pragma unroll
@@ -478,7 +533,7 @@
     FFN_TL(205);
     static_assert(MT <= K1, "stores of a column block fit in its steps");
     const int ncp = a.np / TROWS;
-    const bool full = m0 + BM <= a.M;
+    const bool full = m0 + BM <= mlim;
     uint2 yq[T][MT];
     for (int nc = 0; nc < ncp; ++nc) {
 #pragma unroll
@@ -548,7 +603,7 @@
           yq[t][mt].y = pack_bf16x2(v[2], v[3]);
           acc1[t][mt] = f32x4{0.f, 0.f, 0.f, 0.f};
           const int row = m0 + mt * 16 + (ln & 15);
-          if ((!full || nc == ncp - 1) && row < a.M)
+          if ((!full || nc == ncp - 1) && row < mlim)
             *reinterpret_cast<uint2*>(a.yp + (long long)row * a.np + nc * TROWS + w * (T * 16) + t * 16 + 4 * (ln >> 4)) =
                 yq[t][mt];
         }
@@ -566,7 +621,7 @@
 #pragma unroll
         for (int mt = 0; mt < MT; ++mt) {
           const int row = m0 + mt * 16 + fr;
-          if (row < a.M) *reinterpret_cast<f32x4*>(a.out + (long long)row * D + (w * T + j) * 16 + 4 * g) = ov[j][mt];
+          if (row < mlim) *reinterpret_cast<f32x4*>(a.out + (long long)row * D + (w * T + j) * 16 + 4 * g) = ov[j][mt];
         }
     }
     SBK_PROBE(asm volatile("s_waitcnt vmcnt(0)" ::: "memory");)
@@ -579,7 +634,7 @@
 #pragma unroll
     for (int mt = 0; mt < MT; ++mt) {
       const int row = m0 + mt * 16 + fr;
-      if (row < a.M)
+      if (row < mlim)
         *reinterpret_cast<float4*>(a.out + (long long)row * D + d) =
             make_float4(z[j][mt][0], z[j][mt][1], z[j][mt][2], z[j][mt][3]);
     }
@@ -592,7 +647,7 @@
 #pragma unroll
       for (int mt = 0; mt < MT; ++mt) {
         const int row = m0 + mt * 16 + fr;
-        if (row >= a.M) continue;
+        if (row >= mlim) continue;
         if (a.u_bf16) {
           uint2 pk;
           pk.x = pack_bf16x2(z[j][mt][0], z[j][mt][1]);
@@ -608,6 +663,16 @@
   FFN_TL(196);
 }
 
+template <int D, int ACT, bool PROJ, bool CHAIN>
+__global__ void __launch_bounds__(FFN_NT) ffn_kernel(FfnArgs a) {
+  ffn_body<D, ACT, PROJ, CHAIN, false>(a, nullptr);
+}
+
+template <int ACT>
+__global__ void __launch_bounds__(FFN_NT) conv_chain_kernel(FfnArgs a, ConvStageArgs c) {
+  ffn_body<256, ACT, true, true, true>(a, &c);
+}
+
 template <int D>
 size_t ffn_lds(int H, bool chain) {
   return ((size_t)2 * 256 * 64 + (size_t)FFN_BM * (D + FFN_PAD) + (size_t)2 * FFN_BM * (256 + FFN_PAD)) *
@@ -640,6 +705,40 @@
   const bool proj = a.np > 0, chain = a.g0b != nullptr;
   if (chain) return proj ? launch_ffn<256, true, true>(a, s) : launch_ffn<256, false, true>(a, s);
   return proj ? launch_ffn<256, true, false>(a, s) : launch_ffn<256, false, false>(a, s);
+}
+
+template <int ACT>
+int launch_conv_chain_act(const FfnArgs& a, const ConvStageArgs& c, unsigned grid, size_t lds, hipStream_t s) {
+  if (hipError_t e = sbk::lds_optin(reinterpret_cast<const void*>(&conv_chain_kernel<ACT>), lds)) return (int)e;
+  hipLaunchKernelGGL((conv_chain_kernel<ACT>), dim3(grid), dim3(FFN_NT), lds, s, a, c);
+  return 0;
+}
+
+int conv_chain_dispatch(const FfnArgs& a, const ConvStageArgs& c, hipStream_t s) {
+  const size_t lds = ffn_lds<256>(a.H, true);
+  static_assert(CS_LDS + 2 * 256 * 4 <= (2 * 256 * 64 + FFN_BM * (256 + FFN_PAD) * 3) * 2, "the conv stage lies under ring, Xn, Hs");
+  if (lds > 160 * 1024) return SBK_ERR_ARG;
+  const long long grid = (long long)c.B * ((c.T + FFN_BM - 1) / FFN_BM);
+  if (grid > 0x7fffffffLL) return SBK_ERR_ARG;
+  switch (a.act) {
+    case ACT_SWISH: return launch_conv_chain_act<ACT_SWISH>(a, c, (unsigned)grid, lds, s);
+    case ACT_LRELU: return launch_conv_chain_act<ACT_LRELU>(a, c, (unsigned)grid, lds, s);
+    case ACT_GELU: return launch_conv_chain_act<ACT_GELU>(a, c, (unsigned)grid, lds, s);
+    case ACT_NONE: return launch_conv_chain_act<ACT_NONE>(a, c, (unsigned)grid, lds, s);
+    default: return SBK_ERR_ARG;
+  }
+}
+
+__global__ void __launch_bounds__(256) conv_image_kernel(const bf16_t* __restrict__ w1p, const bf16_t* __restrict__ w2,
+                                                         bf16_t* __restrict__ img) {
+  const int n = (CS_P1T + CS_P3T) * 256 * 8;
+  for (int i = blockIdx.x * blockDim.x + threadIdx.x; i < n; i += gridDim.x * blockDim.x) {
+    const int s = i >> 11, rem = i & 2047, r = rem >> 3, jp = rem & 7;
+    const int j = jp ^ ((r >> 1) & 7);
+    const bf16_t* src = s < CS_P1T ? w1p + (long long)((r >> 5) * 64 + (s & 1) * 32 + (r & 31)) * CS_D + (s >> 1) * 64
+                                   : w2 + (long long)r * CS_D + (s - CS_P1T) * 64;
+    *reinterpret_cast<uint4*>(img + (long long)i * 8) = *reinterpret_cast<const uint4*>(src + 8 * j);
+  }
 }
 
 struct ImgSrc {
@@ -797,3 +896,66 @@
   return sbk_ffn_proj(x, M, D, d_eff, H, g0, b0, eps0, img, img_elems, b1, act, slope, b2, alpha, gp, bp, epsp, out, gn, bn,
                       epsn, u, u_bf16, 0, nullptr, stream);
 }
+
+SBK_API long long sbk_conv_image_elems(int D) { return D == CS_D ? (long long)(CS_P1T + CS_P3T) * CS_TILE : -1; }
+
+SBK_API int sbk_conv_image(const void* w1p, const void* w2, int D, void* img, void* stream) {
+  if (D != CS_D || !w1p || !w2 || !img) return SBK_ERR_ARG;
+  if ((reinterpret_cast<uintptr_t>(w1p) | reinterpret_cast<uintptr_t>(w2) | reinterpret_cast<uintptr_t>(img)) & 15)
+    return SBK_ERR_ARG;
+  hipLaunchKernelGGL(conv_image_kernel, dim3((CS_P1T + CS_P3T) * 8), dim3(256), 0, (hipStream_t)stream,
+                     reinterpret_cast<const bf16_t*>(w1p), reinterpret_cast<const bf16_t*>(w2),
+                     reinterpret_cast<bf16_t*>(img));
+  SBK_CHECK_LAUNCH();
+  return 0;
+}
+
+SBK_API int sbk_conv_ffn_chain(const float* x, const void* o, const void* wo, const float* bo, int B, int T, int D,
+                               int d_eff, const float* cln0_w, const float* cln0_b, float ceps0, const void* cimg,
+                               long long cimg_elems, const float* cb1p, const float* wc, const float* bc, int K,
+                               int causal, const float* cln1_w, const float* cln1_b, float ceps1, const float* cb2,
+                               const unsigned char* kpm, int H, int act, float slope, const float* g0, const float* b0,
+                               float eps0, const float* b1, const float* b2, float alpha, const float* gp,
+                               const float* bp, float epsp, const float* g0b, const float* b0b, float eps0b,
+                               const float* b1b, const float* b2b, float alphab, float* out, const float* gn,
+                               const float* bn, float epsn, const void* img, long long img_elems, int np, void* yp,
+                               void* stream) {
+  if (B <= 0 || T <= 0 || (long long)B * T > 0x7fffffffLL || D != CS_D || K < 1 || K > CS_KMAX || !x || !out ||
+      x == out || d_eff <= 0 || d_eff > D)
+    return SBK_ERR_ARG;
+  if (!o || !wo || !cln0_w || !cln0_b || !cimg || !cb1p || !wc || !cln1_w || !cln1_b) return SBK_ERR_ARG;
+  if (cimg_elems != sbk_conv_image_elems(D)) return SBK_ERR_ARG;
+  if (!g0b || !b0b || !b1b || !b2b || !gn || !bn || !yp || np <= 0) return SBK_ERR_ARG;
+  if ((reinterpret_cast<uintptr_t>(o) | reinterpret_cast<uintptr_t>(wo) | reinterpret_cast<uintptr_t>(bo) |
+       reinterpret_cast<uintptr_t>(cln0_w) | reinterpret_cast<uintptr_t>(cln0_b) | reinterpret_cast<uintptr_t>(cimg) |
+       reinterpret_cast<uintptr_t>(cb1p) | reinterpret_cast<uintptr_t>(cln1_w) | reinterpret_cast<uintptr_t>(cln1_b) |
+       reinterpret_cast<uintptr_t>(cb2) | reinterpret_cast<uintptr_t>(g0b) | reinterpret_cast<uintptr_t>(b0b) |
+       reinterpret_cast<uintptr_t>(b1b) | reinterpret_cast<uintptr_t>(b2b)) & 15)
+    return SBK_ERR_ARG;
+  const int M = B * T;
+  if (ffn_check(x, M, D, H, g0, b0, img, img_elems, 1, b1, act, b2, gp, bp, out, gn, bn, nullptr, np, yp))
+    return SBK_ERR_ARG;
+  FfnArgs a;
+  a.inv_n = 1.0f / (float)d_eff; a.npad = (float)(D - d_eff);
+  a.x = x; a.M = M; a.H = H;
+  a.g0 = g0; a.b0 = b0; a.eps0 = eps0;
+  a.img = reinterpret_cast<const bf16_t*>(img); a.b1 = b1; a.act = act; a.slope = slope;
+  a.b2 = b2; a.alpha = alpha;
+  a.gp = gp; a.bp = bp; a.epsp = epsp;
+  a.out = out;
+  a.gn = gn; a.bn = bn; a.epsn = epsn; a.u = nullptr; a.u_bf16 = 1;
+  a.np = np; a.yp = reinterpret_cast<bf16_t*>(yp);
+  a.g0b = g0b; a.b0b = b0b; a.eps0b = eps0b;
+  a.b1b = b1b; a.b2b = b2b; a.alphab = alphab;
+  ConvStageArgs c;
+  c.x = x; c.B = B; c.T = T; c.K = K; c.padL = causal ? K - 1 : (K - 1) / 2;
+  c.g0 = cln0_w; c.b0 = cln0_b; c.eps0 = ceps0;
+  c.img = reinterpret_cast<const bf16_t*>(cimg); c.b1 = cb1p; c.wc = wc; c.bc = bc;
+  c.g1 = cln1_w; c.b1n = cln1_b; c.eps1 = ceps1;
+  c.b2 = cb2; c.kpm = reinterpret_cast<const uint8_t*>(kpm);
+  c.o = reinterpret_cast<const bf16_t*>(o); c.wo = reinterpret_cast<const bf16_t*>(wo); c.bo = bo;
+  const int rc = conv_chain_dispatch(a, c, (hipStream_t)stream);
+  if (rc) return rc;
+  SBK_CHECK_LAUNCH();
+  return 0;
+}
diff --git a/speechbrain_amd/lobes/models/transformer/Conformer.py b/speechbrain_amd/lobes/models/transformer/Conformer.py
--- a/speechbrain_amd/lobes/models/transformer/Conformer.py
+++ b/speechbrain_amd/lobes/models/transformer/Conformer.py
@@ -16,6 +16,7 @@
 
 USE_CONV_MODULE_KERNEL = True
 USE_LAYER_CHAIN = True
+USE_CONV_CHAIN = True
 USE_PADDED_SHADOW = True
 PAD_D = 256
 
@@ -97,16 +98,19 @@
                 and self.bottleneck[0].bias is not None and isinstance(self.after_conv[1], Swish)
                 and getattr(self.after_conv[1], "beta", 1) == 1)
 
-    def run_fused(self, x2d, B, T, pad_mask_u8=None, pre=None):
+    def fused_params(self):
         w1p, b1p, w2 = self.kernel_weights(_bf16)
         ln = self.after_conv[0]
         lin = self.after_conv[2]
         wc = self._wc.get("taps", [self.conv.weight], lambda: self.conv.weight.detach().reshape(
             self.conv.weight.shape[0], -1).t().contiguous())
-        return _enc.conv_module(x2d, B, T, self.ln_params(), w1p, b1p, wc,
-                                self.conv.bias.detach() if self.conv.bias is not None else None, self.causal,
-                                (ln.weight.detach(), ln.bias.detach(), ln.eps), w2,
-                                lin.bias.detach() if lin.bias is not None else None, pad_mask_u8, pre=pre,
+        return (self.ln_params(), w1p, b1p, wc, self.conv.bias.detach() if self.conv.bias is not None else None,
+                self.causal, (ln.weight.detach(), ln.bias.detach(), ln.eps), w2,
+                lin.bias.detach() if lin.bias is not None else None)
+
+    def run_fused(self, x2d, B, T, pad_mask_u8=None, pre=None):
+        ln0, w1p, b1p, wc, bc, causal, ln1, w2, b2 = self.fused_params()
+        return _enc.conv_module(x2d, B, T, ln0, w1p, b1p, wc, bc, causal, ln1, w2, b2, pad_mask_u8, pre=pre,
                                 deff=self._deff)
 
     def train_run(self, x2d, B, T, dtype, pad_mask_u8=None, residual=None):
@@ -356,16 +360,23 @@
             _, attn, pre = layer.mha_layer.attend_heads(None, B, T, pos, kpm_u8, dtype, need_attn,
                                                         pk=pk_all[:, i * d:(i + 1) * d], qkv=qkv)
             attns.append(attn)
-            x = layer.convolution_module.run_fused(x, B, T, kpm_u8, pre=pre)
             f2 = layer.ffn_module2
+            cm = layer.convolution_module
             if i + 1 < len(L):
                 nl = L[i + 1]
                 a = f2[1].chain_block(ln(layer, f2[0]), 0.5, post_ln=ln(layer, layer.norm2.norm))
                 b = nl.ffn_module1[1].chain_block(ln(nl, nl.ffn_module1[0]), 0.5)
                 act, slope = f2[1].act_name()
-                x, qkv = _enc.ffn_chain(x, a, b, act, slope, ln(nl, nl.norm1.norm), nl.mha_layer.fused_in_proj(dtype),
-                                        deff=f2[1]._deff)
+                wp = nl.mha_layer.fused_in_proj(dtype)
+                if USE_CONV_CHAIN and _enc.conv_ffn_chain_supported(d, cm.conv.weight.shape[-1], a[1].shape[0],
+                                                                    wp.shape[0]):
+                    x, qkv = _enc.conv_ffn_chain(x, B, T, pre, cm.fused_params(), kpm_u8, a, b, act, slope,
+                                                 ln(nl, nl.norm1.norm), wp, deff=f2[1]._deff)
+                    continue
+                x = cm.run_fused(x, B, T, kpm_u8, pre=pre)
+                x, qkv = _enc.ffn_chain(x, a, b, act, slope, ln(nl, nl.norm1.norm), wp, deff=f2[1]._deff)
             else:
+                x = cm.run_fused(x, B, T, kpm_u8, pre=pre)
                 fn = self.norm.norm
                 _, y = f2[1].run_fused(x, ln(layer, f2[0]), 0.5, post_ln=ln(layer, layer.norm2.norm),
                                        next_ln=(fn.weight.detach(), fn.bias.detach(), fn.eps), next_dtype=_f32)
```

After: 406,400 audio-sec/sec (median of 6 runs). +5.8%, better.
